# NVIDIA/tacotron2

Hardware: AMD Instinct MI355X
Metric: mel-frames/sec (train fwd+bwd) LJSpeech hparams (higher is better)
Workload: dtype bf16; 1 GPU; BASELINE configs[1]: LJSpeech default hparams, batch_size=64/GPU, synthetic LJSpeech-shaped batches, full train step (fwd+loss+bwd+clip+Adam); global_batch=64, parallelism=dp1, optimizer=FusedAdam, compute=bf16 MFMA operands, f32 accumulate/state/master weights

## Files before the change

### include/tacotron2_amd.h

```cpp
#ifndef TACOTRON2_AMD_H
#define TACOTRON2_AMD_H

#include <stdint.h>

#ifdef __cplusplus
extern "C" {
#endif

#define T2AMD_ABI_VERSION 1
#define T2AMD_OK 0
#define T2AMD_ERR_ARG 1
#define T2AMD_ERR_LAUNCH 2

#define T2AMD_ATT_DIM 128
#define T2AMD_LOC_FILTERS 32
#define T2AMD_LOC_KERNEL 31
#define T2AMD_LOC_TAPS (2 * T2AMD_LOC_KERNEL)
#define T2AMD_ATT_SLICES 4

int t2amd_abi_version(void);
const char* t2amd_source_sha1(void);
const char* t2amd_last_error(void);
int t2amd_struct_sizes(int* out, int max_n);
int t2amd_set_validate_only(int on);
int t2amd_profile_enable(int tag, int max_launches);
int t2amd_profile_read(float* total_ms, int* count);
int t2amd_profile_event_overhead(float* ms);

typedef struct t2amd_gemm_desc {
    const float* A;
    const float* B;
    float* C;
    int M, N, K;
    long long lda, ldb, ldc;
    int a_kcontig;
    int b_kcontig;
    int batch;
    long long strideA, strideB, strideC;
    int splitk;
    long long strideSplitC;
    int accumulate;
    const float* bias;
    int act;
    const uint8_t* keep;
    long long ldkeep;
    float keep_scale;
    int convA_T, convA_C, convA_pad, convA_sign;
    int convB_T, convB_C, convB_pad;
    int precision;
} t2amd_gemm_desc;

int t2amd_gemm_tile_size(int M, int N, int precision, int nz, int a_kcontig, int b_kcontig);
int t2amd_gemm_f32(const t2amd_gemm_desc* d, void* stream);

int t2amd_splitk_reduce_f32(const float* partials, int nsplit, long long stride, float* out,
                            long long n, int accumulate, int perm_taps, int perm_ci, void* stream);
int t2amd_splitk_reduce2d_f32(const float* partials, int nsplit, long long stride, float* out, int rows, int cols,
                              long long ldo, int accumulate, void* stream);

typedef struct t2amd_gemm16_desc {
    const void* A;
    const void* B;
    float* C;
    int M, N, K;
    long long lda, ldb, ldc;
    int splitk;
    long long strideSplitC;
    int accumulate;
    const float* bias;
    int win_T, win_Tp;
} t2amd_gemm16_desc;
int t2amd_gemm16_tn(const t2amd_gemm16_desc* d, void* stream);
int t2amd_gemm16_kk(const t2amd_gemm16_desc* d, void* stream);
int t2amd_gemm16_kk_group(const t2amd_gemm16_desc* d, int count, void* stream);

int t2amd_cast_halo_bf16(const float* src, long long lds, void* dst, long long rows, int C, int T, int pad, void* stream);

int t2amd_pack_conv_bf16(const float* W, void* out, int Co, int Ci, int k, int Kp, int reversed, void* stream);

int t2amd_transpose_cast_bf16(const void* src, int src_is_bf16, long long lds, void* dst, long long ldd, int rows, int cols,
                              int rows_padded, void* stream);

int t2amd_bn_stats_f32(const float* x, long long ldx, int M, int N, double* ws, float* mean,
                       float* invstd, float* running_mean, float* running_var, float momentum,
                       float eps, void* stream);
int t2amd_bn_eval_invstd_f32(const float* running_var, float* invstd, int N, float eps, void* stream);
int t2amd_bn_act_fwd_f32(const float* x, long long ldx, float* y, long long ldy, int M, int N,
                         const float* mean, const float* invstd, const float* gamma,
                         const float* beta, int act, const uint8_t* keep, long long ldkeep,
                         float keep_scale, const int* lens, int row_valid_T, void* stream);
int t2amd_bn_act_fwd_img_f32(const float* x, long long ldx, float* y, long long ldy, int M, int N, const float* mean,
                             const float* invstd, const float* gamma, const float* beta, int act, const uint8_t* keep,
                             long long ldkeep, float keep_scale, void* y_img16, int T, int pad, void* stream);
int t2amd_bn_act_bwd_f32(float* dy, long long lddy, const float* y, long long ldy, const float* x,
                         long long ldx, int M, int N, const float* mean, const float* invstd,
                         const float* gamma, int act, const uint8_t* keep, long long ldkeep,
                         float keep_scale, double* ws, float* dgamma, float* dbeta, void* stream);
int t2amd_bn_act_bwd_img_f32(float* dy, long long lddy, const float* y, long long ldy, const float* x, long long ldx, int M, int N,
                             const float* mean, const float* invstd, const float* gamma, int act, const uint8_t* keep,
                             long long ldkeep, float keep_scale, double* ws, float* dgamma, float* dbeta, void* dx_img16, int T,
                             int pad, float* dbias, int keep_f32, void* stream);
int t2amd_colsum_f32(const float* x, long long ldx, int M, int N, double* ws, float* out,
                     int accumulate, void* stream);
int t2amd_colsum_bf16(const void* x16, long long ldx, int M, int N, double* ws, float* out, int accumulate, void* stream);

int t2amd_embedding_fwd_f32(const long long* ids, const float* table, float* out, long long rows,
                            int dim, int n_symbols, void* stream);
int t2amd_embedding_bwd_f32(const long long* ids, const float* dout, float* dtable, float* ws, long long rows,
                            int dim, int n_symbols, void* stream);
int t2amd_philox_keep_mask(uint8_t* out, long long n, float p, unsigned long long seed,
                           unsigned long long offset, void* stream);
int t2amd_fill_f32(float* p, long long n, float v, void* stream);
int t2amd_cast_bf16_f32(const float* src, void* dst, long long n, void* stream);
int t2amd_split_bf16x3_f32(const float* src, long long lds, void* dst, long long ldd, long long rows, int K, void* stream);
int t2amd_copy2d_f32(const float* src, long long lds, const float* src2, long long lds2, float* dst,
                     long long ldd, int rows, int cols, void* stream);
int t2amd_transpose_f32(const float* src, long long lds, float* dst, long long ldd, int rows,
                        int cols, int batch, long long sstride, long long dstride, void* stream);
int t2amd_frames_to_time_major_f32(const float* mels, float* x0, int B, int C, int To, void* stream);
int t2amd_split_projection_f32(const float* pg, float* mel_cl, float* gate, const int* out_lens,
                               int B, int C, int To, void* stream);
int t2amd_finalize_outputs_f32(float* mel_cl, const float* post_cl, float* mel, float* mel_post,
                               const int* out_lens, int B, int C, int To, void* stream);
int t2amd_grads_to_channel_last_f32(const float* dmel, const float* dmel_post, float* dmel_cl,
                                    float* dpost_cl, int B, int C, int To, void* stream);
int t2amd_gather_dout_f32(const float* dmel_cl, const float* dgate, float* dout, int B, int C,
                          int To, void* stream);
int t2amd_relu_dropout_bwd_f32(float* dy, const float* y, float scale, long long n, void* stream);

typedef struct t2amd_seg {
    const float* p;
    long long ld;
    int width;
} t2amd_seg;

typedef struct t2amd_lstm_step {
    t2amd_seg x[3];
    int nseg;
    const float* W;
    int Ktot, H, B;
    const float* gin;
    long long ld_gin;
    const float* bias;
    const float* c_prev;
    long long ld_cprev;
    float* gates_out;
    long long ld_gates;
    float* c_out;
    long long ld_c;
    float* h_out;
    long long ld_h;
    const uint8_t* keep;
    long long ld_keep;
    float keep_scale;
    const int* lens;
    int t;
    int tag;
    int bf16;
    void* h16_out;
    long long ld_h16;
} t2amd_lstm_step;

int t2amd_lstm_step_fwd_f32(const t2amd_lstm_step* a, void* stream);
int t2amd_lstm_step_fwd2_f32(const t2amd_lstm_step* a, const t2amd_lstm_step* b, void* stream);

int t2amd_lstm_step_small_f32(const t2amd_lstm_step* a, void* stream);
typedef struct t2amd_small_linear {
    const float* X;
    long long ldx;
    const float* W;
    long long ldw;
    const float* bias;
    float* Y;
    long long ldy;
    int B, N, K;
    int act;
    const uint8_t* keep;
    long long ldkeep;
    float keep_scale;
} t2amd_small_linear;
int t2amd_linear_small_f32(const t2amd_small_linear* a, void* stream);

typedef struct t2amd_skinny_gemm {
    t2amd_seg x[3];
    int nseg;
    const float* W;
    int Ktot, N, B;
    float* Y;
    long long ldy;
    int nsplit;
    long long split_stride;
    int tag;
    int bf16;
    const float* bias;
    int act;
    const uint8_t* keep;
    long long ld_keep;
    float keep_scale;
    void* Y16;
    long long ldy16;
    uint8_t* stop_active;
    int* stop_lengths;
    int* stop_done;
    int stop_col, stop_t, stop_max_steps;
    float stop_threshold;
} t2amd_skinny_gemm;

int t2amd_skinny_gemm_f32(const t2amd_skinny_gemm* a, void* stream);
int t2amd_skinny_gemm2_f32(const t2amd_skinny_gemm* a, const t2amd_skinny_gemm* b, void* stream);

typedef struct t2amd_addend {
    const float* p;
    long long ld;
    int nsplit;
    long long split_stride;
} t2amd_addend;

typedef struct t2amd_lstm_bwd {
    int B, H;
    t2amd_addend dh[3];
    const float* gates;
    long long ld_gates;
    const float* c_prev;
    long long ld_cprev;
    const float* c;
    long long ld_c;
    const uint8_t* keep;
    long long ld_keep;
    float keep_scale;
    float* dc;
    long long ld_dc;
    float* dgates;
    long long ld_dgates;
    const int* lens;
    int t;
    void* dgates16;
    long long ld_dgates16;
    int dgates16_x3;
} t2amd_lstm_bwd;

int t2amd_lstm_pointwise_bwd_f32(const t2amd_lstm_bwd* a, void* stream);
int t2amd_lstm_pointwise_bwd2_f32(const t2amd_lstm_bwd* a, const t2amd_lstm_bwd* b, void* stream);

int t2amd_fold_location_f32(const float* wdense, const float* wconv, float* U, void* stream);
int t2amd_unfold_location_grads_f32(const float* dU_acc, const float* dv_acc, int nb,
                                    const float* wdense, const float* wconv, float* dwdense,
                                    float* dwconv, float* dv, void* stream);

typedef struct t2amd_attn_fwd {
    int B, Ti, E, Hq;
    const float* h;
    long long ld_h;
    const float* Wq;
    const float* U;
    const float* v;
    const float* pm;
    const float* memory;
    const int* lens;
    const float* w_prev;
    long long ld_wprev;
    float* cum;
    float* cum_save;
    float* w_out;
    long long ld_wout;
    float* ctx_out;
    long long ld_ctx;
    float* q_out;
    long long ld_q;
    const uint8_t* active;
    float* ws;
    void* ctx16_out;
    long long ld_ctx16;
    int loc_split_bf16;
    const void* memory16;
    const void* Wq16;
    long long ws_floats;
    int ctx16_x3;
} t2amd_attn_fwd;

int t2amd_attention_step_fwd_f32(const t2amd_attn_fwd* a, void* stream);
// ... 370 lines not shown
```

### tacotron2_amd/csrc/elementwise.hip

```cpp
#include "common.h"

#define RB 64

template <int MODE>
__global__ void colreduce_partial_kernel(const float* __restrict__ x, long long ldx, int M, int N,
                                         double* __restrict__ ws) {
    const int col = blockIdx.x * 64 + (threadIdx.x & 63);
    const int rsub = threadIdx.x >> 6;
    const int rb = blockIdx.y;
    __shared__ double s1[4][64], s2[4][64];
    double a = 0.0, q = 0.0;
    if (col < N) {
        const long long step = (long long)RB * 4;
        long long r = (long long)rb * 4 + rsub;
        for (; r + 3 * step < M; r += 4 * step) {
            const float v0 = x[r * ldx + col], v1 = x[(r + step) * ldx + col];
            const float v2 = x[(r + 2 * step) * ldx + col], v3 = x[(r + 3 * step) * ldx + col];
            a += (double)v0; a += (double)v1; a += (double)v2; a += (double)v3;
            if (MODE == 0) {
                q += (double)v0 * (double)v0; q += (double)v1 * (double)v1;
                q += (double)v2 * (double)v2; q += (double)v3 * (double)v3;
            }
        }
        for (; r < M; r += step) {
// ... 769 lines not shown
            }
        }
    }
}

extern "C" int t2amd_philox_keep_mask(uint8_t* out, long long n, float p, unsigned long long seed,
                                      unsigned long long offset, void* stream) {
    T2_REQUIRE(out && n > 0 && p >= 0.f && p < 1.f, "philox: bad args");
    T2_REQUIRE(offset % 4 == 0, "philox: offset must be a multiple of 4");
    int blocks = t2_cdiv((n + 3) / 4, 256);
    if (blocks > 8192) blocks = 8192;
    T2_LAUNCH(philox_keep_kernel, dim3(blocks), dim3(256), 0, (hipStream_t)stream, out, n, p, seed, offset);
    T2_LAUNCH_CHECK();
    return T2AMD_OK;
}

__global__ void fill_kernel(float* p, long long n, float v) {
    for (long long i = blockIdx.x * (long long)blockDim.x + threadIdx.x; i < n; i += (long long)gridDim.x * blockDim.x)
        p[i] = v;
}
__global__ void cast_bf16_kernel(const float4* __restrict__ src, uint2* __restrict__ dst, long long n4) {
    for (long long i = blockIdx.x * (long long)blockDim.x + threadIdx.x; i < n4; i += (long long)gridDim.x * blockDim.x) {
        const float4 v = src[i];
        uint2 o;
        o.x = (unsigned)t2_f32_to_bf16(v.x) | ((unsigned)t2_f32_to_bf16(v.y) << 16);
        o.y = (unsigned)t2_f32_to_bf16(v.z) | ((unsigned)t2_f32_to_bf16(v.w) << 16);
        dst[i] = o;
    }
}

extern "C" int t2amd_cast_bf16_f32(const float* src, void* dst, long long n, void* stream) {
    T2_REQUIRE(src && dst && n > 0 && n % 4 == 0, "cast_bf16: n must be a positive multiple of 4");
    T2_REQUIRE(t2_aligned16(src) && (reinterpret_cast<uintptr_t>(dst) & 7u) == 0, "cast_bf16: alignment");
    int blocks = t2_cdiv(n / 4, 256);
    if (blocks > 4096) blocks = 4096;
    T2_LAUNCH(cast_bf16_kernel, dim3(blocks), dim3(256), 0, (hipStream_t)stream, reinterpret_cast<const float4*>(src),
              reinterpret_cast<uint2*>(dst), n / 4);
    T2_LAUNCH_CHECK();
    return T2AMD_OK;
}

__global__ void split_bf16x3_kernel(const float* __restrict__ src, long long lds_, unsigned short* __restrict__ dst, long long ldd,
                                    long long rows, int K4) {
    const long long total = rows * K4;
    for (long long i = blockIdx.x * (long long)blockDim.x + threadIdx.x; i < total; i += (long long)gridDim.x * blockDim.x) {
        const long long r = i / K4;
        const int k = (int)(i - r * K4) * 4;
        const float4 v = *reinterpret_cast<const float4*>(src + r * lds_ + k);
        unsigned short h[4], l[4];
        t2_split_bf16(v.x, h[0], l[0]); t2_split_bf16(v.y, h[1], l[1]);
        t2_split_bf16(v.z, h[2], l[2]); t2_split_bf16(v.w, h[3], l[3]);
        unsigned short* const d = dst + r * ldd * 2 + t2_x3_pos(k);
        *reinterpret_cast<uint2*>(d) = make_uint2((unsigned)h[0] | ((unsigned)h[1] << 16), (unsigned)h[2] | ((unsigned)h[3] << 16));
        *reinterpret_cast<uint2*>(d + 16) = make_uint2((unsigned)l[0] | ((unsigned)l[1] << 16), (unsigned)l[2] | ((unsigned)l[3] << 16));
    }
}
extern "C" int t2amd_split_bf16x3_f32(const float* src, long long lds, void* dst, long long ldd, long long rows, int K, void* stream) {
    T2_REQUIRE(src && dst && rows > 0 && K > 0 && K % 16 == 0, "split_bf16x3: K must be a positive multiple of 16");
    T2_REQUIRE(lds >= K && lds % 4 == 0 && ldd >= K && ldd % 16 == 0, "split_bf16x3: row strides (lds % 4 == 0, ldd % 16 == 0, both >= K)");
    T2_REQUIRE(t2_aligned16(src) && t2_aligned16(dst), "split_bf16x3: alignment");
    int blocks = t2_cdiv(rows * (K / 4), 256);
    if (blocks > 8192) blocks = 8192;
    T2_LAUNCH(split_bf16x3_kernel, dim3(blocks), dim3(256), 0, (hipStream_t)stream, src, lds, reinterpret_cast<unsigned short*>(dst), ldd,
              rows, K / 4);
    T2_LAUNCH_CHECK();
    return T2AMD_OK;
}

extern "C" int t2amd_fill_f32(float* p, long long n, float v, void* stream) {
    T2_REQUIRE(p && n > 0, "fill: bad args");
    int blocks = t2_cdiv(n, 256);
    if (blocks > 4096) blocks = 4096;
    T2_LAUNCH(fill_kernel, dim3(blocks), dim3(256), 0, (hipStream_t)stream, p, n, v);
    T2_LAUNCH_CHECK();
    return T2AMD_OK;
}

__global__ void copy2d_kernel(const float* __restrict__ src, long long lds_, const float* __restrict__ src2,
                              long long lds2, float* __restrict__ dst, long long ldd, int rows, int cols) {
    const long long total = (long long)rows * cols;
    for (long long i = blockIdx.x * (long long)blockDim.x + threadIdx.x; i < total;
         i += (long long)gridDim.x * blockDim.x) {
        const long long r = i / cols;
        const int c = (int)(i - r * cols);
        float v = src[r * lds_ + c];
        if (src2) v += src2[r * lds2 + c];
        dst[r * ldd + c] = v;
    }
}
extern "C" int t2amd_copy2d_f32(const float* src, long long lds_, const float* src2, long long lds2, float* dst,
                                long long ldd, int rows, int cols, void* stream) {
    T2_REQUIRE(src && dst && rows > 0 && cols > 0, "copy2d: bad args");
    int blocks = t2_cdiv((long long)rows * cols, 256);
    if (blocks > 4096) blocks = 4096;
    T2_LAUNCH(copy2d_kernel, dim3(blocks), dim3(256), 0, (hipStream_t)stream, src, lds_, src2, lds2, dst, ldd,
                       rows, cols);
    T2_LAUNCH_CHECK();
    return T2AMD_OK;
}

__global__ void transpose_kernel(const float* __restrict__ src, long long lds_, float* __restrict__ dst, long long ldd,
                                 int rows, int cols, long long sstride, long long dstride) {
    __shared__ float tile[32][33];
    const float* s = src + (long long)blockIdx.z * sstride;
    float* d = dst + (long long)blockIdx.z * dstride;
    const int c0 = blockIdx.x * 32, r0 = blockIdx.y * 32;
    const int tx = threadIdx.x & 31, ty = threadIdx.x >> 5;
    for (int j = ty; j < 32; j += 8) {
        const int r = r0 + j, c = c0 + tx;
        tile[j][tx] = (r < rows && c < cols) ? s[(long long)r * lds_ + c] : 0.f;
    }
    __syncthreads();
    for (int j = ty; j < 32; j += 8) {
        const int c = c0 + j, r = r0 + tx;
        if (c < cols && r < rows) d[(long long)c * ldd + r] = tile[tx][j];
    }
}
extern "C" int t2amd_transpose_f32(const float* src, long long lds_, float* dst, long long ldd, int rows, int cols,
                                   int batch, long long sstride, long long dstride, void* stream) {
    T2_REQUIRE(src && dst && rows > 0 && cols > 0 && batch > 0, "transpose: bad args");
    dim3 grid(t2_cdiv(cols, 32), t2_cdiv(rows, 32), batch);
    T2_REQUIRE(grid.y <= 65535 && grid.z <= 65535, "transpose: grid too large");
    T2_LAUNCH(transpose_kernel, grid, dim3(256), 0, (hipStream_t)stream, src, lds_, dst, ldd, rows, cols, sstride,
                       dstride);
    T2_LAUNCH_CHECK();
    return T2AMD_OK;
}

__global__ void frames_to_tm_kernel(const float* __restrict__ mels, float* __restrict__ x0, int B, int C, int To) {
    __shared__ float tile[32][33];
    const int b = blockIdx.z;
    const int t0 = blockIdx.x * 32, c0 = blockIdx.y * 32;
    const int tx = threadIdx.x & 31, ty = threadIdx.x >> 5;
    for (int j = ty; j < 32; j += 8) {
        const int c = c0 + j, t = t0 + tx;
        float v = 0.f;
        if (c < C && t < To && t >= 1) v = mels[((long long)b * C + c) * To + (t - 1)];
        tile[j][tx] = v;
    }
    __syncthreads();
    for (int j = ty; j < 32; j += 8) {
        const int t = t0 + j, c = c0 + tx;
        if (t < To && c < C) x0[((long long)t * B + b) * C + c] = tile[tx][j];
    }
}
extern "C" int t2amd_frames_to_time_major_f32(const float* mels, float* x0, int B, int C, int To, void* stream) {
    T2_REQUIRE(mels && x0 && B > 0 && C > 0 && To > 0, "frames_to_tm: bad args");
    dim3 grid(t2_cdiv(To, 32), t2_cdiv(C, 32), B);
    T2_LAUNCH(frames_to_tm_kernel, grid, dim3(256), 0, (hipStream_t)stream, mels, x0, B, C, To);
    T2_LAUNCH_CHECK();
    return T2AMD_OK;
}

__global__ void split_projection_kernel(const float* __restrict__ pg, float* __restrict__ mel_cl,
                                        float* __restrict__ gate, const int* __restrict__ out_lens, int B, int C,
                                        int To) {
    const long long total = (long long)To * B * (C + 1);
    for (long long i = blockIdx.x * (long long)blockDim.x + threadIdx.x; i < total;
         i += (long long)gridDim.x * blockDim.x) {
        const long long row = i / (C + 1);
        const int c = (int)(i - row * (C + 1));
        const int t = (int)(row / B), b = (int)(row - (long long)t * B);
        const float v = pg[i];
        if (c < C) {
            mel_cl[((long long)b * To + t) * C + c] = v;
        } else {
            const bool pad = out_lens && t >= out_lens[b];
            gate[(long long)b * To + t] = pad ? 1e3f : v;
        }
    }
}
extern "C" int t2amd_split_projection_f32(const float* pg, float* mel_cl, float* gate, const int* out_lens, int B,
                                          int C, int To, void* stream) {
    T2_REQUIRE(pg && mel_cl && gate && B > 0 && C > 0 && To > 0, "split_projection: bad args");
    int blocks = t2_cdiv((long long)To * B * (C + 1), 256);
    if (blocks > 8192) blocks = 8192;
    T2_LAUNCH(split_projection_kernel, dim3(blocks), dim3(256), 0, (hipStream_t)stream, pg, mel_cl, gate,
                       out_lens, B, C, To);
    T2_LAUNCH_CHECK();
    return T2AMD_OK;
}

__global__ void finalize_outputs_kernel(float* __restrict__ mel_cl, const float* __restrict__ post_cl,
                                        float* __restrict__ mel, float* __restrict__ mel_post,
                                        const int* __restrict__ out_lens, int B, int C, int To) {
    __shared__ float t1[32][33], t2[32][33];
    const int b = blockIdx.z;
    const int c0 = blockIdx.x * 32, t0 = blockIdx.y * 32;
    const int tx = threadIdx.x & 31, ty = threadIdx.x >> 5;
    const int len = out_lens ? out_lens[b] : To;
    for (int j = ty; j < 32; j += 8) {
        const int t = t0 + j, c = c0 + tx;
        float m = 0.f, q = 0.f;
        if (t < To && c < C) {
            const long long idx = ((long long)b * To + t) * C + c;
            if (t < len) {
                m = mel_cl[idx];
                q = post_cl ? m + post_cl[idx] : 0.f;
            } else {
                mel_cl[idx] = 0.f;
            }
        }
        t1[j][tx] = m;
        t2[j][tx] = q;
    }
    __syncthreads();
    for (int j = ty; j < 32; j += 8) {
        const int c = c0 + j, t = t0 + tx;
        if (c < C && t < To) {
            const long long o = ((long long)b * C + c) * To + t;
            mel[o] = t1[tx][j];
            if (mel_post) mel_post[o] = t2[tx][j];
        }
    }
}
extern "C" int t2amd_finalize_outputs_f32(float* mel_cl, const float* post_cl, float* mel, float* mel_post,
                                          const int* out_lens, int B, int C, int To, void* stream) {
    T2_REQUIRE(mel_cl && mel && B > 0 && C > 0 && To > 0, "finalize_outputs: bad args");
    T2_REQUIRE((post_cl != nullptr) == (mel_post != nullptr), "finalize_outputs: post_cl and mel_post go together");
    dim3 grid(t2_cdiv(C, 32), t2_cdiv(To, 32), B);
    T2_REQUIRE(grid.y <= 65535, "finalize_outputs: To too large");
    T2_LAUNCH(finalize_outputs_kernel, grid, dim3(256), 0, (hipStream_t)stream, mel_cl, post_cl, mel, mel_post,
                       out_lens, B, C, To);
    T2_LAUNCH_CHECK();
    return T2AMD_OK;
}

__global__ void grads_to_cl_kernel(const float* __restrict__ dmel, const float* __restrict__ dmel_post,
                                   float* __restrict__ dmel_cl, float* __restrict__ dpost_cl, int B, int C, int To) {
    __shared__ float t1[32][33], t2[32][33];
    const int b = blockIdx.z;
    const int t0 = blockIdx.x * 32, c0 = blockIdx.y * 32;
    const int tx = threadIdx.x & 31, ty = threadIdx.x >> 5;
    for (int j = ty; j < 32; j += 8) {
        const int c = c0 + j, t = t0 + tx;
        float a = 0.f, q = 0.f;
        if (c < C && t < To) {
            const long long idx = ((long long)b * C + c) * To + t;
            if (dmel) a = dmel[idx];
            if (dmel_post) q = dmel_post[idx];
        }
        t1[j][tx] = a;
        t2[j][tx] = q;
    }
    __syncthreads();
    for (int j = ty; j < 32; j += 8) {
        const int t = t0 + j, c = c0 + tx;
        if (t < To && c < C) {
            const long long o = ((long long)b * To + t) * C + c;
            dmel_cl[o] = t1[tx][j] + t2[tx][j];
            dpost_cl[o] = t2[tx][j];
        }
    }
}
extern "C" int t2amd_grads_to_channel_last_f32(const float* dmel, const float* dmel_post, float* dmel_cl,
                                               float* dpost_cl, int B, int C, int To, void* stream) {
    T2_REQUIRE(dmel_cl && dpost_cl && B > 0 && C > 0 && To > 0, "grads_to_cl: bad args");
    dim3 grid(t2_cdiv(To, 32), t2_cdiv(C, 32), B);
    T2_LAUNCH(grads_to_cl_kernel, grid, dim3(256), 0, (hipStream_t)stream, dmel, dmel_post, dmel_cl, dpost_cl, B,
                       C, To);
    T2_LAUNCH_CHECK();
    return T2AMD_OK;
}

__global__ void gather_dout_kernel(const float* __restrict__ dmel_cl, const float* __restrict__ dgate,
                                   float* __restrict__ dout, int B, int C, int To) {
    const long long total = (long long)To * B * (C + 1);
    for (long long i = blockIdx.x * (long long)blockDim.x + threadIdx.x; i < total;
         i += (long long)gridDim.x * blockDim.x) {
        const long long row = i / (C + 1);
        const int c = (int)(i - row * (C + 1));
        const int t = (int)(row / B), b = (int)(row - (long long)t * B);
        float v;
        if (c < C) v = dmel_cl[((long long)b * To + t) * C + c];
        else v = dgate ? dgate[(long long)b * To + t] : 0.f;
        dout[i] = v;
    }
}
extern "C" int t2amd_gather_dout_f32(const float* dmel_cl, const float* dgate, float* dout, int B, int C, int To,
                                     void* stream) {
    T2_REQUIRE(dmel_cl && dout && B > 0 && C > 0 && To > 0, "gather_dout: bad args");
    int blocks = t2_cdiv((long long)To * B * (C + 1), 256);
    if (blocks > 8192) blocks = 8192;
    T2_LAUNCH(gather_dout_kernel, dim3(blocks), dim3(256), 0, (hipStream_t)stream, dmel_cl, dgate, dout, B, C,
                       To);
    T2_LAUNCH_CHECK();
    return T2AMD_OK;
}

__global__ void relu_dropout_bwd_kernel(float* __restrict__ dy, const float* __restrict__ y, float scale, long long n) {
    for (long long i = blockIdx.x * (long long)blockDim.x + threadIdx.x; i < n; i += (long long)gridDim.x * blockDim.x)
        dy[i] = (y[i] > 0.f) ? dy[i] * scale : 0.f;
}
__global__ void relu_dropout_bwd_vec_kernel(float4* __restrict__ dy, const float4* __restrict__ y, float scale, long long n4) {
    for (long long i = blockIdx.x * (long long)blockDim.x + threadIdx.x; i < n4; i += (long long)gridDim.x * blockDim.x) {
        const float4 g = dy[i], v = y[i];
        dy[i] = make_float4((v.x > 0.f) ? g.x * scale : 0.f, (v.y > 0.f) ? g.y * scale : 0.f, (v.z > 0.f) ? g.z * scale : 0.f,
                            (v.w > 0.f) ? g.w * scale : 0.f);
    }
}
extern "C" int t2amd_relu_dropout_bwd_f32(float* dy, const float* y, float scale, long long n, void* stream) {
    T2_REQUIRE(dy && y && n > 0, "relu_dropout_bwd: bad args");
    if (!g_ew_scalar && n % 4 == 0 && t2_aligned16(dy) && t2_aligned16(y)) {
        int b4 = t2_cdiv(n / 4, 256);
        if (b4 > 8192) b4 = 8192;
        T2_LAUNCH(relu_dropout_bwd_vec_kernel, dim3(b4), dim3(256), 0, (hipStream_t)stream, reinterpret_cast<float4*>(dy),
                  reinterpret_cast<const float4*>(y), scale, n / 4);
        T2_LAUNCH_CHECK();
        return T2AMD_OK;
    }
    int blocks = t2_cdiv(n, 256);
    if (blocks > 8192) blocks = 8192;
    T2_LAUNCH(relu_dropout_bwd_kernel, dim3(blocks), dim3(256), 0, (hipStream_t)stream, dy, y, scale, n);
    T2_LAUNCH_CHECK();
    return T2AMD_OK;
}
```

### tacotron2_amd/csrc/gemm16.hip

```cpp
#include "common.h"
#include <stdlib.h>

typedef __bf16 g16_bf16x8 __attribute__((ext_vector_type(8)));
typedef __attribute__((address_space(3))) void* g16_lptr;
typedef __attribute__((address_space(1))) const void* g16_gptr;

#define G16_T 256
#define G16_BK 64
#define G16_IMG (G16_T * 128)
#define G16_NT 512

struct Gemm16Params {
    t2amd_gemm16_desc d;
    int ktiles_per_split;
};

struct G16Tile { int bx, by, bz; };
__device__ __forceinline__ G16Tile g16_tile_id() {
    const int nbx = gridDim.x, nby = gridDim.y;
    const int total = nbx * nby * (int)gridDim.z;
    const int L = blockIdx.x + nbx * (blockIdx.y + nby * blockIdx.z);
    const int xcd = L & 7, q = L >> 3;
    const int base = total >> 3, rem = total & 7;
    const int id = xcd * base + (xcd < rem ? xcd : rem) + q;
    const int per_z = nbx * nby;
    G16Tile t;
    t.bz = id / per_z;
    const int r = id - t.bz * per_z;
    const int G = 8;
    const int group = r / (G * nbx);
    const int first = group * G;
    const int gsz = (nby - first) < G ? (nby - first) : G;
    const int w = r - group * (G * nbx);
    t.by = first + w % gsz;
    t.bx = w / gsz;
    return t;
}

__global__ __launch_bounds__(G16_NT) void gemm16_tn_kernel(Gemm16Params p) {
    __shared__ __attribute__((aligned(16))) char smem[4 * G16_IMG];
    const t2amd_gemm16_desc& d = p.d;
    const int tid = threadIdx.x, lane = tid & 63;
    const int wave = __builtin_amdgcn_readfirstlane(tid >> 6);
    const int wm = wave >> 2, wn = wave & 3;
    const int l31 = lane & 31, lhi = lane >> 5;

    const G16Tile tile = g16_tile_id();
    const int split = tile.bz;
    const int row0 = tile.by * G16_T, col0 = tile.bx * G16_T;
    const int M = d.M, N = d.N;
    const int nkt_all = d.K / G16_BK;
    const int kt_beg = split * p.ktiles_per_split;
    int kt_end = kt_beg + p.ktiles_per_split;
    if (kt_end > nkt_all) kt_end = nkt_all;
    const int nk = kt_end > kt_beg ? kt_end - kt_beg : 0;

    const char* asrc[4];
    const char* bsrc[4];
    {
        const int rin = 8 * wave + (lane >> 3);
        const int chunk = (lane & 7) ^ ((rin >> 1) & 7);
#pragma unroll
        for (int i = 0; i < 4; ++i) {
            int ga = row0 + 64 * i + rin, gb = col0 + 64 * i + rin;
            ga = ga < M ? ga : M - 1;
            gb = gb < N ? gb : N - 1;
            asrc[i] = reinterpret_cast<const char*>(d.A) + ((long long)ga * d.lda + (long long)kt_beg * G16_BK) * 2 + chunk * 16;
            bsrc[i] = reinterpret_cast<const char*>(d.B) + ((long long)gb * d.ldb + (long long)kt_beg * G16_BK) * 2 + chunk * 16;
        }
    }
#define G16_ISSUE(STAGE)                                                                                         \
    {                                                                                                            \
        char* ad_ = smem + (STAGE) * G16_IMG + wave * 1024;                                                      \
        char* bd_ = smem + (2 + (STAGE)) * G16_IMG + wave * 1024;                                                \
        _Pragma("unroll") for (int i = 0; i < 4; ++i) {                                                          \
            __builtin_amdgcn_global_load_lds((g16_gptr)(asrc[i]), (g16_lptr)(ad_ + i * 8192), 16, 0, 0);         \
            __builtin_amdgcn_global_load_lds((g16_gptr)(bsrc[i]), (g16_lptr)(bd_ + i * 8192), 16, 0, 0);         \
            asrc[i] += 128; bsrc[i] += 128;                                                                      \
        }                                                                                                        \
    }

    unsigned aaddr[4][4], baddr[2][4];
    {
        const unsigned base = (unsigned)reinterpret_cast<size_t>((g16_lptr)(smem));
#pragma unroll
        for (int t = 0; t < 4; ++t) {
            const int r = wm * 128 + t * 32 + l31;
#pragma unroll
            for (int ks = 0; ks < 4; ++ks) aaddr[t][ks] = base + (unsigned)(r * 128 + (((2 * ks + lhi) ^ ((r >> 1) & 7)) << 4));
        }
#pragma unroll
        for (int t = 0; t < 2; ++t) {
            const int r = wn * 64 + t * 32 + l31;
#pragma unroll
            for (int ks = 0; ks < 4; ++ks)
                baddr[t][ks] = base + 2 * G16_IMG + (unsigned)(r * 128 + (((2 * ks + lhi) ^ ((r >> 1) & 7)) << 4));
        }
    }

    f32x16 acc[4][2];
#pragma unroll
    for (int i = 0; i < 4; ++i)
#pragma unroll
        for (int j = 0; j < 2; ++j)
#pragma unroll
            for (int r = 0; r < 16; ++r) acc[i][j][r] = 0.f;

    f32x4 fa[4], fb[2], ga[4], gb[2];
#define G16_READ(STAGE, KS, A_, B_)                                                                              \
    asm volatile(                                                                                                \
        "ds_read_b128 %0, %6 offset:%12\n\t"                                                                     \
        "ds_read_b128 %4, %10 offset:%12\n\t"                                                                    \
        "ds_read_b128 %1, %7 offset:%12\n\t"                                                                     \
        "ds_read_b128 %5, %11 offset:%12\n\t"                                                                    \
        "ds_read_b128 %2, %8 offset:%12\n\t"                                                                     \
        "ds_read_b128 %3, %9 offset:%12"                                                                         \
        : "=&v"(A_[0]), "=&v"(A_[1]), "=&v"(A_[2]), "=&v"(A_[3]), "=&v"(B_[0]), "=&v"(B_[1])                     \
        : "v"(aaddr[0][KS]), "v"(aaddr[1][KS]), "v"(aaddr[2][KS]), "v"(aaddr[3][KS]), "v"(baddr[0][KS]),          \
          "v"(baddr[1][KS]), "i"((STAGE) * G16_IMG)                                                              \
        : "memory");
#define G16_WAIT(A_, B_)                                                                                         \
    asm volatile("s_waitcnt lgkmcnt(0)"                                                                          \
                 : "+v"(A_[0]), "+v"(A_[1]), "+v"(A_[2]), "+v"(A_[3]), "+v"(B_[0]), "+v"(B_[1]) : : "memory");
#define G16_MFMA(A_, B_)                                                                                         \
    _Pragma("unroll") for (int i = 0; i < 4; ++i)                                                                \
        _Pragma("unroll") for (int j = 0; j < 2; ++j)                                                            \
            acc[i][j] = __builtin_amdgcn_mfma_f32_32x32x16_bf16(__builtin_bit_cast(g16_bf16x8, A_[i]),           \
                                                                __builtin_bit_cast(g16_bf16x8, B_[j]), acc[i][j], 0, 0, 0);
#define G16_TILE(STAGE)                                                                                          \
    {                                                                                                            \
        G16_READ(STAGE, 0, fa, fb) G16_WAIT(fa, fb)                                                              \
        G16_READ(STAGE, 1, ga, gb) __builtin_amdgcn_sched_barrier(0); G16_MFMA(fa, fb) __builtin_amdgcn_sched_barrier(0); G16_WAIT(ga, gb) \
        G16_READ(STAGE, 2, fa, fb) __builtin_amdgcn_sched_barrier(0); G16_MFMA(ga, gb) __builtin_amdgcn_sched_barrier(0); G16_WAIT(fa, fb) \
        G16_READ(STAGE, 3, ga, gb) __builtin_amdgcn_sched_barrier(0); G16_MFMA(fa, fb) __builtin_amdgcn_sched_barrier(0); G16_WAIT(ga, gb) \
        G16_MFMA(ga, gb)                                                                                         \
    }

    if (nk > 0) {
        G16_ISSUE(0)
        asm volatile("s_waitcnt vmcnt(0)" ::: "memory");
        __builtin_amdgcn_s_barrier();
        for (int kt = 0; kt + 1 < nk; kt += 2) {
            G16_ISSUE(1)
            G16_TILE(0)
            asm volatile("s_waitcnt vmcnt(0)" ::: "memory");
            __builtin_amdgcn_s_barrier();
            if (kt + 2 < nk) G16_ISSUE(0)
            G16_TILE(1)
            asm volatile("s_waitcnt vmcnt(0)" ::: "memory");
            __builtin_amdgcn_s_barrier();
        }
        if (nk & 1) G16_TILE(0)
    }
#undef G16_ISSUE
#undef G16_READ
#undef G16_WAIT
#undef G16_MFMA
#undef G16_TILE

    float* __restrict__ C = d.C + (long long)split * d.strideSplitC;
#pragma unroll
    for (int tm = 0; tm < 4; ++tm) {
#pragma unroll
        for (int tn = 0; tn < 2; ++tn) {
            const int gn = col0 + wn * 64 + tn * 32 + l31;
#pragma unroll
            for (int r = 0; r < 16; ++r) {
                const int gm = row0 + wm * 128 + tm * 32 + (r & 3) + 8 * (r >> 2) + 4 * lhi;
                long long crow = gm;
                bool live = gm < M;
                if (d.win_Tp > 0) {
                    const int b_ = gm / d.win_Tp, t_ = gm - b_ * d.win_Tp;
                    live = live && t_ < d.win_T;
                    crow = (long long)b_ * d.win_T + t_;
                }
                if (live && gn < N) {
                    float* cp = C + crow * d.ldc + gn;
                    float val = acc[tm][tn][r];
                    if (d.bias) val += d.bias[gn];
                    if (d.accumulate) val += *cp;
                    *cp = val;
                }
            }
        }
    }
}

extern "C" int t2amd_gemm16_tn(const t2amd_gemm16_desc* dp, void* stream) {
    T2_REQUIRE(dp != nullptr, "gemm16: null descriptor");
    Gemm16Params p;
    p.d = *dp;
    t2amd_gemm16_desc& d = p.d;
    T2_REQUIRE(d.A && d.B && d.C, "gemm16: null operand");
    T2_REQUIRE(d.M > 0 && d.N > 0 && d.K > 0 && d.K % G16_BK == 0, "gemm16: K must be a positive multiple of 64");
    T2_REQUIRE(t2_aligned16(d.A) && t2_aligned16(d.B) && d.lda % 8 == 0 && d.ldb % 8 == 0 && d.ldb >= d.K,
               "gemm16: operands must be 16-byte aligned with row strides that are multiples of 8 elements (B's >= K)");
    T2_REQUIRE(d.win_Tp == 0 || (d.win_T > 0 && d.win_T <= d.win_Tp && d.splitk == 1), "gemm16: bad window geometry");
    T2_REQUIRE(d.win_Tp > 0 || d.lda >= d.K, "gemm16: lda must be >= K unless the rows are windows");
    if (d.splitk < 1) d.splitk = 1;
    T2_REQUIRE(d.splitk == 1 || (!d.bias && !d.accumulate), "gemm16: split-K needs a plain epilogue");
    const int nkt = d.K / G16_BK;
    p.ktiles_per_split = t2_cdiv(nkt, d.splitk);
    dim3 grid(t2_cdiv(d.N, G16_T), t2_cdiv(d.M, G16_T), d.splitk);
    T2_REQUIRE(grid.y <= 65535 && grid.z <= 65535, "gemm16: grid too large");
    T2_LAUNCH(gemm16_tn_kernel, grid, dim3(G16_NT), 0, (hipStream_t)stream, p);
    T2_LAUNCH_CHECK();
    return T2AMD_OK;
}

typedef float g16_f32x2 __attribute__((ext_vector_type(2)));

#define G16_GROUP 4
struct Gemm16GroupParams {
    t2amd_gemm16_desc d[G16_GROUP];
    int coltile_end[G16_GROUP];
    int count;
};

__global__ __launch_bounds__(G16_NT) void gemm16_kk_kernel(Gemm16GroupParams p) {
    __shared__ __attribute__((aligned(16))) char smem[4 * G16_IMG];
    const int tid = threadIdx.x, lane = tid & 63;
    const int wave = __builtin_amdgcn_readfirstlane(tid >> 6);
    const int wm = wave >> 2, wn = wave & 3;
    const int l31 = lane & 31, lhi = lane >> 5;

    const G16Tile tile = g16_tile_id();
    const int split = tile.bz;
    int prob = 0;
#pragma unroll
    for (int j = 0; j + 1 < G16_GROUP; ++j)
        if (j + 1 < p.count && tile.bx >= p.coltile_end[j]) prob = j + 1;
    const int bx = tile.bx - (prob > 0 ? p.coltile_end[prob - 1] : 0);
    struct { const void* A; const void* B; float* C; int M, N, K; long long lda, ldb, ldc; long long strideSplitC; int accumulate;
             const float* bias; int splitk; } d;
    d.A = p.d[prob].A; d.B = p.d[prob].B; d.C = p.d[prob].C; d.M = p.d[prob].M; d.N = p.d[prob].N; d.K = p.d[prob].K;
    d.lda = p.d[prob].lda; d.ldb = p.d[prob].ldb; d.ldc = p.d[prob].ldc; d.strideSplitC = p.d[prob].strideSplitC;
    d.accumulate = p.d[prob].accumulate; d.bias = p.d[prob].bias; d.splitk = p.d[prob].splitk;
    const int row0 = tile.by * G16_T, col0 = bx * G16_T;
    const int M = d.M, N = d.N;
    const int nkt_all = (d.K + G16_BK - 1) / G16_BK;
    const int per_split = (nkt_all + d.splitk - 1) / d.splitk;
    const int kt_beg = split * per_split;
    int kt_end = kt_beg + per_split;
    if (kt_end > nkt_all) kt_end = nkt_all;
    const int nk = kt_end > kt_beg ? kt_end - kt_beg : 0;
    const int rem = d.K - (nkt_all - 1) * G16_BK;
    const int ztile = (kt_end == nkt_all && rem < G16_BK) ? nk - 1 : -1;

    const int rsub = 2 * wave + lhi;
    const long long arow = d.lda * 2, brow = d.ldb * 2;
    const char* asrc[4];
    const char* bsrc[4];
    {
        const int cl = l31 ^ ((rsub & 3) << 2);
        int ma = row0 + 8 * cl, nb = col0 + 8 * cl;
        ma = ma + 8 <= M ? ma : M - 8;
        nb = nb + 8 <= N ? nb : N - 8;
#pragma unroll
        for (int i = 0; i < 4; ++i) {
            const long long k = (long long)kt_beg * G16_BK + 16 * i + rsub;
            asrc[i] = reinterpret_cast<const char*>(d.A) + k * arow + (long long)ma * 2;
            bsrc[i] = reinterpret_cast<const char*>(d.B) + k * brow + (long long)nb * 2;
        }
    }
#define KK_ISSUE(STAGE, KT)                                                                                      \
    {                                                                                                            \
        char* ad_ = smem + (STAGE) * G16_IMG + wave * 1024;                                                      \
        char* bd_ = smem + (2 + (STAGE)) * G16_IMG + wave * 1024;                                                \
        if ((KT) != ztile) {                                                                                     \
            _Pragma("unroll") for (int i = 0; i < 4; ++i) {                                                      \
                __builtin_amdgcn_global_load_lds((g16_gptr)(asrc[i]), (g16_lptr)(ad_ + i * 8192), 16, 0, 0);     \
                __builtin_amdgcn_global_load_lds((g16_gptr)(bsrc[i]), (g16_lptr)(bd_ + i * 8192), 16, 0, 0);     \
                asrc[i] += 64 * arow; bsrc[i] += 64 * brow;                                                      \
            }                                                                                                    \
        } else {                                                                                                 \
            _Pragma("unroll") for (int i = 0; i < 4; ++i) {                                                      \
                const int over = 16 * i + rsub - (rem - 1);           \
                const char* a_ = over > 0 ? asrc[i] - over * arow : asrc[i];                                     \
                const char* b_ = over > 0 ? bsrc[i] - over * brow : bsrc[i];                                     \
                __builtin_amdgcn_global_load_lds((g16_gptr)(a_), (g16_lptr)(ad_ + i * 8192), 16, 0, 0);          \
                __builtin_amdgcn_global_load_lds((g16_gptr)(b_), (g16_lptr)(bd_ + i * 8192), 16, 0, 0);          \
            }                                                                                                    \
        }                                                                                                        \
    }
#define KK_LANDED(STAGE, KT)                                                                                     \
    asm volatile("s_waitcnt vmcnt(0)" ::: "memory");                                                             \
    if ((KT) == ztile) {                                                                                         \
        _Pragma("unroll") for (int i = 0; i < 4; ++i)                                                            \
            if (16 * i + rsub >= rem)                                                                            \
                *reinterpret_cast<f32x4*>(smem + (STAGE) * G16_IMG + i * 8192 + wave * 1024 + lane * 16) = f32x4{0.f, 0.f, 0.f, 0.f}; \
        asm volatile("s_waitcnt lgkmcnt(0)" ::: "memory");                                                       \
    }                                                                                                            \
    __builtin_amdgcn_s_barrier();

    unsigned aaddr[4], baddr[2];
    {
        const unsigned base = (unsigned)reinterpret_cast<size_t>((g16_lptr)(smem));
        const int g = lane >> 4, i = lane & 15;
        const int r = 8 * (g >> 1) + (i >> 2);
        const int sw = (i >> 2) << 2;
        const int sub = 2 * (g & 1) + ((i & 3) >> 1);
        const unsigned in = (unsigned)(r * 512 + (i & 1) * 8);
#pragma unroll
        for (int t = 0; t < 4; ++t) aaddr[t] = base + in + (unsigned)((((wm * 16 + 4 * t + sub) ^ sw)) << 4);
#pragma unroll
        for (int t = 0; t < 2; ++t) baddr[t] = base + 2 * G16_IMG + in + (unsigned)((((wn * 8 + 4 * t + sub) ^ sw)) << 4);
    }

    f32x16 acc[4][2];
#pragma unroll
    for (int i = 0; i < 4; ++i)
#pragma unroll
        for (int j = 0; j < 2; ++j)
#pragma unroll
            for (int r = 0; r < 16; ++r) acc[i][j][r] = 0.f;

    g16_f32x2 fa[4][2], fb[2][2], ga[4][2], gb[2][2];
#define KK_READ(STAGE, KS, A_, B_)                                                                               \
    asm volatile(                                                                                                \
        "ds_read_b64_tr_b16 %0, %12 offset:%18\n\t"                                                              \
        "ds_read_b64_tr_b16 %1, %12 offset:%19\n\t"                                                              \
        "ds_read_b64_tr_b16 %8, %16 offset:%18\n\t"                                                              \
        "ds_read_b64_tr_b16 %9, %16 offset:%19\n\t"                                                              \
        "ds_read_b64_tr_b16 %2, %13 offset:%18\n\t"                                                              \
        "ds_read_b64_tr_b16 %3, %13 offset:%19\n\t"                                                              \
        "ds_read_b64_tr_b16 %10, %17 offset:%18\n\t"                                                             \
        "ds_read_b64_tr_b16 %11, %17 offset:%19\n\t"                                                             \
        "ds_read_b64_tr_b16 %4, %14 offset:%18\n\t"                                                              \
        "ds_read_b64_tr_b16 %5, %14 offset:%19\n\t"                                                              \
        "ds_read_b64_tr_b16 %6, %15 offset:%18\n\t"                                                              \
        "ds_read_b64_tr_b16 %7, %15 offset:%19"                                                                  \
        : "=&v"(A_[0][0]), "=&v"(A_[0][1]), "=&v"(A_[1][0]), "=&v"(A_[1][1]), "=&v"(A_[2][0]), "=&v"(A_[2][1]),  \
          "=&v"(A_[3][0]), "=&v"(A_[3][1]), "=&v"(B_[0][0]), "=&v"(B_[0][1]), "=&v"(B_[1][0]), "=&v"(B_[1][1])   \
        : "v"(aaddr[0]), "v"(aaddr[1]), "v"(aaddr[2]), "v"(aaddr[3]), "v"(baddr[0]), "v"(baddr[1]),              \
          "i"((STAGE) * G16_IMG + (KS) * 8192), "i"((STAGE) * G16_IMG + (KS) * 8192 + 2048)                      \
        : "memory");
#define KK_WAIT(A_, B_)                                                                                          \
    asm volatile("s_waitcnt lgkmcnt(0)"                                                                          \
                 : "+v"(A_[0][0]), "+v"(A_[0][1]), "+v"(A_[1][0]), "+v"(A_[1][1]), "+v"(A_[2][0]), "+v"(A_[2][1]), \
                   "+v"(A_[3][0]), "+v"(A_[3][1]), "+v"(B_[0][0]), "+v"(B_[0][1]), "+v"(B_[1][0]), "+v"(B_[1][1]) : : "memory");
#define KK_OP(X_) __builtin_bit_cast(g16_bf16x8, __builtin_shufflevector(X_[0], X_[1], 0, 1, 2, 3))
#define KK_MFMA(A_, B_)                                                                                          \
    _Pragma("unroll") for (int i = 0; i < 4; ++i)                                                                \
        _Pragma("unroll") for (int j = 0; j < 2; ++j)                                                            \
            acc[i][j] = __builtin_amdgcn_mfma_f32_32x32x16_bf16(KK_OP(A_[i]), KK_OP(B_[j]), acc[i][j], 0, 0, 0);
#define KK_TILE(STAGE)                                                                                           \
    {                                                                                                            \
        KK_READ(STAGE, 0, fa, fb) KK_WAIT(fa, fb)                                                                \
        KK_READ(STAGE, 1, ga, gb) __builtin_amdgcn_sched_barrier(0); KK_MFMA(fa, fb) __builtin_amdgcn_sched_barrier(0); KK_WAIT(ga, gb) \
        KK_READ(STAGE, 2, fa, fb) __builtin_amdgcn_sched_barrier(0); KK_MFMA(ga, gb) __builtin_amdgcn_sched_barrier(0); KK_WAIT(fa, fb) \
        KK_READ(STAGE, 3, ga, gb) __builtin_amdgcn_sched_barrier(0); KK_MFMA(fa, fb) __builtin_amdgcn_sched_barrier(0); KK_WAIT(ga, gb) \
        KK_MFMA(ga, gb)                                                                                          \
    }

    if (nk > 0) {
        KK_ISSUE(0, 0)
        KK_LANDED(0, 0)
        for (int kt = 0; kt + 1 < nk; kt += 2) {
            KK_ISSUE(1, kt + 1)
            KK_TILE(0)
            KK_LANDED(1, kt + 1)
            if (kt + 2 < nk) KK_ISSUE(0, kt + 2)
            KK_TILE(1)
            KK_LANDED(0, kt + 2)
        }
        if (nk & 1) KK_TILE(0)
    }
#undef KK_ISSUE
#undef KK_LANDED
#undef KK_READ
#undef KK_WAIT
#undef KK_OP
#undef KK_MFMA
#undef KK_TILE

    float* __restrict__ C = d.C + (long long)split * d.strideSplitC;
#pragma unroll
    for (int tm = 0; tm < 4; ++tm) {
#pragma unroll
        for (int tn = 0; tn < 2; ++tn) {
            const int gn = col0 + wn * 64 + tn * 32 + l31;
#pragma unroll
            for (int r = 0; r < 16; ++r) {
                const int gm = row0 + wm * 128 + tm * 32 + (r & 3) + 8 * (r >> 2) + 4 * lhi;
                if (gm < M && gn < N) {
                    float* cp = C + (long long)gm * d.ldc + gn;
                    float val = acc[tm][tn][r];
                    if (d.bias) val += d.bias[gn];
                    if (d.accumulate) val += *cp;
                    *cp = val;
                }
            }
        }
    }
}

extern "C" int t2amd_gemm16_kk_group(const t2amd_gemm16_desc* dp, int count, void* stream) {
    T2_REQUIRE(dp != nullptr && count >= 1 && count <= G16_GROUP, "gemm16_kk: 1..4 descriptors");
    Gemm16GroupParams p;
    p.count = count;
    int coltiles = 0;
    for (int j = 0; j < G16_GROUP; ++j) {
        p.d[j] = dp[j < count ? j : count - 1];
        if (j >= count) { p.coltile_end[j] = coltiles; continue; }
        t2amd_gemm16_desc& d = p.d[j];
        T2_REQUIRE(d.A && d.B && d.C, "gemm16_kk: null operand");
        T2_REQUIRE(d.M >= 8 && d.N >= 8 && d.K > 0 && d.M % 8 == 0 && d.N % 8 == 0, "gemm16_kk: M and N must be positive multiples of 8, K positive");
        T2_REQUIRE(t2_aligned16(d.A) && t2_aligned16(d.B) && d.lda > 0 && d.ldb > 0 && d.lda % 8 == 0 && d.ldb % 8 == 0,
                   "gemm16_kk: operands must be 16-byte aligned with row strides that are multiples of 8 elements");
        T2_REQUIRE(d.win_Tp == 0 && d.win_T == 0, "gemm16_kk: no window epilogue (overlapping rows are expressed by lda / ldb < M / N)");
        if (d.splitk < 1) d.splitk = 1;
        T2_REQUIRE(d.splitk == 1 || (!d.bias && !d.accumulate), "gemm16_kk: split-K needs a plain epilogue");
        T2_REQUIRE(d.M == p.d[0].M && d.splitk == p.d[0].splitk, "gemm16_kk: the products of one launch share M and the split count");
        coltiles += t2_cdiv(d.N, G16_T);
        p.coltile_end[j] = coltiles;
    }
    dim3 grid(coltiles, t2_cdiv(p.d[0].M, G16_T), p.d[0].splitk);
    T2_REQUIRE(grid.y <= 65535 && grid.z <= 65535, "gemm16_kk: grid too large");
    T2_LAUNCH(gemm16_kk_kernel, grid, dim3(G16_NT), 0, (hipStream_t)stream, p);
    T2_LAUNCH_CHECK();
    return T2AMD_OK;
}

extern "C" int t2amd_gemm16_kk(const t2amd_gemm16_desc* dp, void* stream) { return t2amd_gemm16_kk_group(dp, 1, stream); }

template <bool SRC16>
__global__ __launch_bounds__(256) void transpose_cast16_kernel(const void* __restrict__ src, long long lds_, unsigned short* __restrict__ dst,
                                                               long long ldd, int rows, int cols, int rpad) {
    __shared__ unsigned short tile[64][66];
    const int r0 = blockIdx.x * 64, c0 = blockIdx.y * 64;
    const int tid = threadIdx.x;
    const bool vec_in = SRC16 ? (lds_ % 4 == 0 && (reinterpret_cast<size_t>(src) & 7) == 0) : (lds_ % 4 == 0 && (reinterpret_cast<size_t>(src) & 15) == 0);
#pragma unroll
    for (int pass = 0; pass < 4; ++pass) {
        const int i = pass * 16 + (tid >> 4), j = 4 * (tid & 15);
        const int r = r0 + i, c = c0 + j;
        unsigned short v[4] = {0, 0, 0, 0};
        if (r < rows) {
            if (vec_in && c + 3 < cols) {
                if (SRC16) {
                    const uint2 u = *reinterpret_cast<const uint2*>(reinterpret_cast<const unsigned short*>(src) + (long long)r * lds_ + c);
                    v[0] = (unsigned short)(u.x & 0xffffu); v[1] = (unsigned short)(u.x >> 16);
                    v[2] = (unsigned short)(u.y & 0xffffu); v[3] = (unsigned short)(u.y >> 16);
                } else {
                    const float4 f = *reinterpret_cast<const float4*>(reinterpret_cast<const float*>(src) + (long long)r * lds_ + c);
                    v[0] = t2_f32_to_bf16(f.x); v[1] = t2_f32_to_bf16(f.y); v[2] = t2_f32_to_bf16(f.z); v[3] = t2_f32_to_bf16(f.w);
                }
            } else {
#pragma unroll
                for (int e = 0; e < 4; ++e)
                    if (c + e < cols)
                        v[e] = SRC16 ? reinterpret_cast<const unsigned short*>(src)[(long long)r * lds_ + c + e]
                                     : t2_f32_to_bf16(reinterpret_cast<const float*>(src)[(long long)r * lds_ + c + e]);
            }
        }
#pragma unroll
        for (int e = 0; e < 4; ++e) tile[i][j + e] = v[e];
    }
    __syncthreads();
    const bool vec_out = ldd % 4 == 0 && (reinterpret_cast<size_t>(dst) & 7) == 0;
#pragma unroll
    for (int pass = 0; pass < 4; ++pass) {
        const int i = pass * 16 + (tid >> 4), j = 4 * (tid & 15);
        const int c = c0 + i, r = r0 + j;
        if (c >= cols || r >= rpad) continue;
        unsigned short* o = dst + (long long)c * ldd + r;
        if (vec_out && r + 3 < rpad) {
            uint2 u;
            u.x = (unsigned)tile[j][i] | ((unsigned)tile[j + 1][i] << 16);
            u.y = (unsigned)tile[j + 2][i] | ((unsigned)tile[j + 3][i] << 16);
            *reinterpret_cast<uint2*>(o) = u;
        } else {
#pragma unroll
            for (int e = 0; e < 4; ++e)
                if (r + e < rpad) o[e] = tile[j + e][i];
        }
    }
}

__global__ __launch_bounds__(256) void cast_halo16_kernel(const float* __restrict__ src, long long lds_, unsigned short* __restrict__ dst,
                                                          long long img_rows, long long nb, int C4, int T, int Tp, int pad) {
    const long long i = (long long)blockIdx.x * 256 + threadIdx.x;
    if (i >= img_rows * C4) return;
    const long long R = i / C4;
    const int c4 = (int)(i - R * C4);
    const long long b = R / Tp;
    const int t = (int)(R - b * Tp) - pad;
    uint2 o = make_uint2(0u, 0u);
    if (b < nb && t >= 0 && t < T) {
        const float4 v = *reinterpret_cast<const float4*>(src + (b * T + t) * lds_ + c4 * 4);
        o.x = (unsigned)t2_f32_to_bf16(v.x) | ((unsigned)t2_f32_to_bf16(v.y) << 16);
        o.y = (unsigned)t2_f32_to_bf16(v.z) | ((unsigned)t2_f32_to_bf16(v.w) << 16);
    }
    *reinterpret_cast<uint2*>(dst + (R * (long long)(C4 * 4)) + c4 * 4) = o;
}

__global__ __launch_bounds__(256) void pack_conv16_kernel(const float* __restrict__ W, unsigned short* __restrict__ out, int Co, int Ci,
                                                          int k, int Kp, int reversed) {
    const int rows = reversed ? Ci : Co, inner = reversed ? Co : Ci;
    const long long n = (long long)rows * Kp;
    for (long long i = (long long)blockIdx.x * 256 + threadIdx.x; i < n; i += (long long)gridDim.x * 256) {
        const int r = (int)(i / Kp), c = (int)(i - (long long)r * Kp);
        unsigned short v = 0;
        if (c < k * inner) {
            const int tap = c / inner, j = c - tap * inner;
            const int co = reversed ? j : r, ci = reversed ? r : j, t = reversed ? k - 1 - tap : tap;
            v = t2_f32_to_bf16(W[((long long)co * Ci + ci) * k + t]);
        }
        out[i] = v;
    }
}

extern "C" int t2amd_pack_conv_bf16(const float* W, void* out, int Co, int Ci, int k, int Kp, int reversed, void* stream) {
    T2_REQUIRE(W && out && Co > 0 && Ci > 0 && k > 0 && Kp >= k * (reversed ? Co : Ci), "pack_conv: bad arguments");
    const long long n = (long long)(reversed ? Ci : Co) * Kp;
    int blocks = t2_cdiv(n, 256);
    if (blocks > 8192) blocks = 8192;
    T2_LAUNCH(pack_conv16_kernel, dim3(blocks), dim3(256), 0, (hipStream_t)stream, W, (unsigned short*)out, Co, Ci, k, Kp, reversed);
    T2_LAUNCH_CHECK();
    return T2AMD_OK;
}

extern "C" int t2amd_cast_halo_bf16(const float* src, long long lds_, void* dst, long long rows, int C, int T, int pad, void* stream) {
    T2_REQUIRE(src && dst && rows > 0 && C > 0 && C % 4 == 0 && T > 0 && rows % T == 0 && pad >= 0 && lds_ % 4 == 0 &&
                   t2_aligned16(src) && t2_aligned16(dst),
               "cast_halo: rows must be whole utterances of T, C a multiple of 4, 16-byte aligned operands");
    const long long nb = rows / T, img_rows = nb * (T + 2 * pad) + 2 * pad;
    const long long n = img_rows * (C / 4);
    T2_REQUIRE((n + 255) / 256 < (1ll << 31), "cast_halo: too large");
    T2_LAUNCH(cast_halo16_kernel, dim3((unsigned)((n + 255) / 256)), dim3(256), 0, (hipStream_t)stream, src, lds_, (unsigned short*)dst,
              img_rows, nb, C / 4, T, T + 2 * pad, pad);
    T2_LAUNCH_CHECK();
    return T2AMD_OK;
}

extern "C" int t2amd_transpose_cast_bf16(const void* src, int src_is_bf16, long long lds_, void* dst, long long ldd, int rows, int cols,
                                         int rows_padded, void* stream) {
    T2_REQUIRE(src && dst && rows > 0 && cols > 0 && rows_padded >= rows && ldd >= rows_padded, "transpose_cast: bad arguments");
    dim3 grid(t2_cdiv(rows_padded, 64), t2_cdiv(cols, 64));
    T2_REQUIRE(grid.y <= 65535, "transpose_cast: too many columns");
    if (src_is_bf16)
        T2_LAUNCH((transpose_cast16_kernel<true>), grid, dim3(256), 0, (hipStream_t)stream, src, lds_, (unsigned short*)dst, ldd, rows, cols, rows_padded);
    else
        T2_LAUNCH((transpose_cast16_kernel<false>), grid, dim3(256), 0, (hipStream_t)stream, src, lds_, (unsigned short*)dst, ldd, rows, cols, rows_padded);
    T2_LAUNCH_CHECK();
    return T2AMD_OK;
}
```

### tacotron2_amd/engine.py

```python
import os

import math
import torch

from . import native as nv
from .native import NativeError

BN_EPS = 1e-5
BN_MOMENTUM = 0.1


def check_hparams(hp):
    if hp.n_frames_per_step != 1:
        raise ValueError("n_frames_per_step != 1 is not supported (nor by the reference, hparams.py:56)")
    K = hp.attention_location_kernel_size
    if not (1 <= hp.attention_dim <= nv.ATT_DIM and 1 <= hp.attention_location_n_filters <= nv.LOC_FILTERS
            and 1 <= K <= nv.LOC_KERNEL and K % 2 == 1):
        raise ValueError("the attention kernels hold attention_dim <= %d, <= %d location filters and an odd location "
                         "kernel <= %d (smaller geometries run zero-embedded in the compiled one; an even kernel size "
                         "does not run in the reference either: ConvNorm pads (k-1)//2, model.py:18-20)"
                         % (nv.ATT_DIM, nv.LOC_FILTERS, nv.LOC_KERNEL))
    for name in ('encoder_embedding_dim', 'attention_rnn_dim', 'decoder_rnn_dim', 'prenet_dim'):
        if getattr(hp, name) % 64 != 0:
            raise ValueError("%s must be a multiple of 64 for the MFMA recurrent kernels" % name)
    if (hp.encoder_embedding_dim // 2) % 64 != 0:
        raise ValueError("encoder_embedding_dim/2 must be a multiple of 64")
    if hp.symbols_embedding_dim != hp.encoder_embedding_dim:
        raise ValueError("symbols_embedding_dim must equal encoder_embedding_dim")
    for name in ('encoder_embedding_dim', 'postnet_embedding_dim', 'n_mel_channels'):
        if getattr(hp, name) % 16 != 0:
            raise ValueError("%s must be a multiple of 16 (implicit-GEMM convolution tiles)" % name)
    if hp.encoder_kernel_size % 2 != 1 or hp.postnet_kernel_size % 2 != 1:
        raise ValueError("convolution kernel sizes must be odd")


class MaskSource(object):

    def __init__(self, injected, device, run=None):
        self.injected = injected or {}
        self.device = device
        self.run = run
        self.seed = None
        self.offset = 0

    def get(self, name, index, shape, p):
        src = self.injected.get(name)
        if src is not None:
            m = src[index] if index is not None else src
            if tuple(m.shape) != tuple(shape) or m.dtype != torch.uint8 or not m.is_contiguous():
                raise NativeError("injected mask %s[%s] must be contiguous uint8 of shape %s, got %s %s"
                                  % (name, index, tuple(shape), tuple(m.shape), m.dtype))
            return m
        if self.seed is None:
            self.seed = int(torch.randint(0, 2 ** 62, (1,)).item())
        out = self.run.empty8(*shape) if self.run is not None else torch.empty(shape, dtype=torch.uint8, device=self.device)
        nv.philox_keep_mask(out, p, self.seed, self.offset)
        self.offset += (out.numel() + 3) // 4 * 4
        return out


def _choose_splitk(M, N, K, batch=1, precision=0, a_km=False, b_kn=False):
    t256 = ((M + 255) // 256) * ((N + 255) // 256) * batch
    if precision >= 1 and M >= 512 and N >= 512 and nv.gemm_tile_size(M, N, precision, 1 << 20, a_km, b_kn) == 256:
        if t256 >= 192:
            return 1
        best, best_score = 0, -1.0
        for s in range(1, 33):
            if s > 1 and K // s < 512:
                break
            if t256 * s < 192:
                continue
            w = t256 * s / 256.0
            score = w / math.ceil(w) * min(1.0, w / 0.85) - 0.02 * (s - 1)
            if score > best_score:
                best, best_score = s, score
        if best:
            return best
    tiles = ((M + 127) // 128) * ((N + 127) // 128) * batch
    if tiles >= 512:
        return 1
    s = (768 + tiles - 1) // tiles
    s = min(s, 64, max(1, K // 256))
    return max(1, s)


def _choose_splitk16(M, N, K):
    t256 = ((M + 255) // 256) * ((N + 255) // 256)
    nkt = (K + 63) // 64
    best, best_t = 1, None
    for s in range(1, 65):
        if s > 1 and nkt // s < 8:
            break
        rounds = math.ceil(t256 * s / 256.0)
        t = rounds * (math.ceil(nkt / s) * 1.9 + 4.0)
        if s > 1:
            t += (s + 1) * M * N * 4 / 5.0e6 + 3.0
        if best_t is None or t < best_t - 1e-9:
            best, best_t = s, t
    return best


WGRAD16 = os.environ.get('T2AMD_WGRAD16', '1') != '0'


WGRAD_KK = os.environ.get('T2AMD_WGRAD_KK', '1') != '0'


def _kk_to(run, out, A16, B16, K, M, N, lda=None, ldb=None, perm=None):
    sk = _choose_splitk16(M, N, K)
    if sk == 1 and perm is None:
        nv.gemm16_kk(out, A16, B16, K, M=M, N=N, lda=lda, ldb=ldb)
        return
    part = run.empty(sk, M * N)
    nv.gemm16_kk(part[0].view(M, N), A16, B16, K, M=M, N=N, lda=lda, ldb=ldb, splitk=sk, partials=part)
    if perm is not None:
        nv.splitk_reduce(part, sk, out, perm_taps=perm[0], perm_ci=perm[1])
    else:
        nv.splitk_reduce2d(part, sk, out)


def _lstm_wgrad_kk(run, dG2, B, parts, outs):
    rowsD, G4 = dG2.shape
    widths = [src.shape[1] for src, _ in parts]
    offs = [0]
    for w in widths:
        offs.append(offs[-1] + w)
    jobs = []
    for dW, i0, i1 in outs:
        base = offs[i0]
        for i in range(i0, i1):
            src, shifted = parts[i]
            if src.dtype != torch.bfloat16:
                src = run.cast16(src)
            blk = dW[:, offs[i] - base:offs[i + 1] - base]
            if shifted and rowsD <= B:
                blk.zero_()
            elif shifted:
                jobs.append((blk, dG2[B:], src, rowsD - B, widths[i]))
            else:
                jobs.append((blk, dG2, src, rowsD, widths[i]))
    if not jobs:
        return
    sk = _choose_splitk16(G4, sum((j[4] + 255) // 256 * 256 for j in jobs), rowsD)
    if sk == 1:
        nv.gemm16_kk_group([dict(Cm=blk, A16=A, B16=Bm, K=K, M=G4, N=w) for blk, A, Bm, K, w in jobs])
        return
    parts_ = [run.empty(sk, G4 * w) for _, _, _, _, w in jobs]
    nv.gemm16_kk_group([dict(Cm=pt[0].view(G4, w), A16=A, B16=Bm, K=K, M=G4, N=w, splitk=sk, partials=pt)
                        for (blk, A, Bm, K, w), pt in zip(jobs, parts_)])
    for (blk, _, _, _, _), pt in zip(jobs, parts_):
        nv.splitk_reduce2d(pt, sk, blk)


def _lstm_wgrad16(run, dG2, B, parts, outs):
    rowsD, G4 = dG2.shape
    if WGRAD_KK and G4 % 8 == 0 and all(src.shape[1] % 8 == 0 for src, _ in parts):
        return _lstm_wgrad_kk(run, dG2, B, parts, outs)
    Kp = ((rowsD + B + 63) // 64) * 64
    GT = run.empty16(G4, Kp)
    nv.transpose_cast_bf16(dG2, GT)
    widths = [src.shape[1] for src, _ in parts]
    XT = run.empty16(sum(widths), Kp)
    n0, offs = 0, []
    for (src, shifted), w in zip(parts, widths):
        blk = XT[n0:n0 + w]
        if shifted:
            blk[:, :B].zero_()
            if rowsD > B:
                nv.transpose_cast_bf16(src[:rowsD - B], blk[:, B:])
            else:
                blk[:, B:].zero_()
        else:
            nv.transpose_cast_bf16(src, blk)
        offs.append(n0)
        n0 += w
    offs.append(n0)
    for dW, i0, i1 in outs:
        Bop = XT[offs[i0]:offs[i1]]
        M, N = dW.shape
        sk = _choose_splitk16(M, N, Kp)
        if sk == 1:
            nv.gemm16_tn(dW, GT, Bop)
        else:
            part = run.empty(sk, M * N)
            nv.gemm16_tn(dW, GT, Bop, splitk=sk, partials=part)
            nv.splitk_reduce(part, sk, dW)


class _Ctx(object):
    arena = None

    def release(self):
        a, self.arena = self.arena, None
        _arena_release(a)

    def __del__(self):
        try:
            self.release()
        except Exception:
            pass


class _EvalCtx(object):
    training = False


FAST_GRAD_GEMM = True


def _dgrad_split():
    raw = os.environ.get('T2AMD_DGRAD_SPLIT', '2')
    try:
        ns = int(raw)
    except ValueError:
        ns = -1
    if not 1 <= ns <= 8:
        raise NativeError("T2AMD_DGRAD_SPLIT must be an integer in 1..8, got %r" % (raw,))
    return ns


DGRAD_SPLIT = _dgrad_split()


def _enc_dgrad_split():
    raw = os.environ.get('T2AMD_ENC_DGRAD_SPLIT', '4')
    if raw not in ('1', '2', '4'):
        raise NativeError("T2AMD_ENC_DGRAD_SPLIT must be 1, 2 or 4, got %r" % (raw,))
    return int(raw)


ENC_DGRAD_SPLIT = _enc_dgrad_split()

BN_BWD_IMAGE = os.environ.get('T2AMD_BN_BWD_IMAGE', '1') != '0'
BN_FWD_IMAGE = os.environ.get('T2AMD_BN_FWD_IMAGE', '1') != '0'
BIAS_GRAD16 = os.environ.get('T2AMD_BIAS_GRAD16', '1') != '0'
GATE_GRADS_BF16_ONLY = os.environ.get('T2AMD_GATE_GRADS_BF16_ONLY', '1') != '0'
DXD_RING = int(os.environ.get('T2AMD_DXD_RING', '3'))


def _rg(run, *a, **k):
    return run.gemm(*a, fast=run.gradp, **k)


def _ng(run, *a, **k):
    return nv.gemm(*a, fast=run.gradp, **k)


def _fg(run, *a, exact=False, **k):
    return nv.gemm(*a, fast=(0 if (exact and run.x3) else run.fwdp), **k)


_PACK_GEN = [0]


def bump_weight_generation():
    _PACK_GEN[0] += 1


# ... 597 lines not shown
               "runs on the launch chain from here on" % ne)
        if log is not None:
            log(msg)
        else:
            import sys
            print(msg, file=sys.stderr, flush=True)
    if n > 0:
        TRAIN_FWD_PERSISTENT = False
        nv.set_attn_fwd_fused(0)
        nv.set_attn_bwd_fused(0)
        nv.set_bptt_cell_fold(0)
        msg = ("tacotron2_amd: %d in-launch attention hand-off(s) timed out (the workgroups of an utterance were not "
               "co-resident within 50 ms -- is the GPU shared or partitioned?); that step was poisoned with NaN and is "
               "skipped; the separate-launch forms are selected from here on" % n)
        if TRAIN_FWD_REPROMOTE_AFTER > 0:
            msg += " (and re-selected after %d clean steps)" % _DEMOTION['need']
        if log is not None:
            log(msg)
        else:
            import sys
            print(msg, file=sys.stderr, flush=True)
    return n + ne


def _cached_bias_sum(run, tag, b1, b2):
    return run.cached(tag, [b1, b2], lambda: _bias_sum(run, b1, b2))


_ATT_Q = 'decoder.attention_layer.query_layer.linear_layer.weight'
_ATT_M = 'decoder.attention_layer.memory_layer.linear_layer.weight'
_ATT_V = 'decoder.attention_layer.v.linear_layer.weight'
_ATT_D = 'decoder.attention_layer.location_layer.location_dense.linear_layer.weight'
_ATT_C = 'decoder.attention_layer.location_layer.location_conv.conv.weight'


def _embed_attention(run, P):
    Wq, Wm, Wv, Wd, Wc = (P[n] for n in (_ATT_Q, _ATT_M, _ATT_V, _ATT_D, _ATT_C))
    A, F, K = Wq.shape[0], Wc.shape[0], Wc.shape[2]
    AD, FD, KD = nv.ATT_DIM, nv.LOC_FILTERS, nv.LOC_KERNEL
    if (A, F, K) == (AD, FD, KD):
        return P, ()

    def embed():
        o = (KD - K) // 2
        q = run.zeros(AD, Wq.shape[1]); q[:A] = Wq
        m = run.zeros(AD, Wm.shape[1]); m[:A] = Wm
        v = run.zeros(1, AD); v[:, :A] = Wv
        d = run.zeros(AD, FD); d[:A, :F] = Wd
        c = run.zeros(FD, 2, KD); c[:F, :, o:o + K] = Wc
        return q, m, v, d, c
    emb = run.cached('attention.embedded', [Wq, Wm, Wv, Wd, Wc], embed)
    P = dict(P)
    P.update(zip((_ATT_Q, _ATT_M, _ATT_V, _ATT_D, _ATT_C), emb))
    return P, (_ATT_Q, _ATT_M, _ATT_V, _ATT_D, _ATT_C)


def _crop_attention_grad(name, grad, shape):
    if name == _ATT_C:
        o = (nv.LOC_KERNEL - shape[2]) // 2
        return grad[:shape[0], :, o:o + shape[2]]
    return grad[:shape[0], :shape[1]]


def _fold_U(run, Wdense, Wconv):
    U = run.empty(nv.ATT_DIM * nv.LOC_TAPS)
    nv.fold_location(Wdense, Wconv, U)
    return U


def _packed_projection(run, P, Cm, Hd, E):
    Wp = P['decoder.linear_projection.linear_layer.weight']
    Wg = P['decoder.gate_layer.linear_layer.weight']
    bp = P['decoder.linear_projection.linear_layer.bias']
    bg = P['decoder.gate_layer.linear_layer.bias']

    def pack():
        Wpg = run.empty(Cm + 1, Hd + E)
        nv.copy2d(Wpg[:Cm], Wp)
        nv.copy2d(Wpg[Cm:], Wg)
        bpg = run.empty(Cm + 1)
        nv.copy2d(bpg[:Cm].view(1, Cm), bp.view(1, Cm))
        nv.copy2d(bpg[Cm:].view(1, 1), bg.view(1, 1))
        return Wpg, bpg
    return run.cached('Wpg', [Wp, Wg, bp, bg], pack)


def _forward(model, P, bufs, text, in_lens, mels, max_len, out_lens, training):
    hp = model.hparams
    dev = text.device
    if not text.is_cuda and not nv.validate_only():
        raise NativeError("tacotron2_amd: the engine runs on the MI355X only (got %s tensors). "
                          "There is no CPU path; the CPU oracle lives in oracle/ for tests." % dev)
    nv.load()
    c = _Ctx()
    c.arena = _arena_acquire(dev)
    run = _Run(dev, getattr(model, 'precision', 'fp32'), _weight_cache(model), c.arena)
    _guard_weights(model, run, P)
    P, _ = _embed_attention(run, P)
    ms = MaskSource(model.dropout_masks, dev, run)
    B = text.shape[0]
    Ti = int(max_len)
    To = mels.shape[2]
    E = hp.encoder_embedding_dim
    Ha, Hd, Pd = hp.attention_rnn_dim, hp.decoder_rnn_dim, hp.prenet_dim
    Cm = hp.n_mel_channels
    He = E // 2
    A = nv.ATT_DIM
    if text.shape[1] != Ti:
        text = text[:, :Ti]
    text = text.contiguous()
    mels = mels.contiguous().float()
    lens32 = in_lens.to(torch.int32).contiguous()
    olens32 = out_lens.to(torch.int32).contiguous() if (model.mask_padding and out_lens is not None) else None
    c.B, c.Ti, c.To, c.text, c.lens32, c.olens32 = B, Ti, To, text, lens32, olens32
    c.training = training

    rowsE = B * Ti
    emb = run.empty(rowsE, E)
    nv.embedding_fwd(text, P['embedding.weight'], emb)
    nconv = hp.encoder_n_convolutions
    enc_masks = [ms.get('enc', i, (B, Ti, E), 0.5) for i in range(nconv)] if training else None
    x3, c.enc_saved = _conv_stack_fwd(run, P, bufs, 'encoder.convolutions', nconv, emb, Ti,
                                      [1] * nconv, enc_masks, training, exact=True)
    memory = run.empty(B, Ti, E)
    c.enc_lstm = []
    for d, sfx in enumerate(('', '_reverse')):
        Wih = P['encoder.lstm.weight_ih_l0' + sfx]
        Whh = P['encoder.lstm.weight_hh_l0' + sfx]
        bsum = _cached_bias_sum(run, 'enc_bias' + sfx, P['encoder.lstm.bias_ih_l0' + sfx], P['encoder.lstm.bias_hh_l0' + sfx])
        GX = run.empty(rowsE, 4 * He)
        _fg(run, GX, x3, Wih, bias=bsum)
        Cst = run.empty(Ti, B, He)
        desc = nv.LstmSeq()
        desc.B, desc.T, desc.H, desc.reverse = B, Ti, He, d
        desc.Whh = nv.ptr(Whh)
        desc.GX = nv.ptr(GX)
        out_view = memory.view(rowsE, E)[:, d * He:(d + 1) * He]
        desc.out, desc.ld_out = nv.ptr(out_view), E
        desc.C = nv.ptr(Cst)
        desc.lens = nv.ptr(lens32, torch.int32)
        c.enc_lstm.append(dict(GX=GX, C=Cst, Whh=Whh, Wih=Wih, desc=desc, bsum=bsum))

    def regen_gx():
        for L_ in c.enc_lstm:
            _fg(run, L_['GX'], x3, L_['Wih'], bias=L_['bsum'])
    model.last_encoder_path = _encoder_lstm_fwd(
        model, text.device, c.enc_lstm[0]['desc'], c.enc_lstm[1]['desc'], regen_gx,
        reads=[L_[k_] for L_ in c.enc_lstm for k_ in ('Whh', 'GX')] + [lens32],
        writes=[memory] + [L_['C'] for L_ in c.enc_lstm], poison=memory if training else None, run=run)
    c.x3, c.memory = x3, memory

    rowsD = To * B
    x0 = run.empty(To, B, Cm)
    nv.frames_to_time_major(mels, x0)
    W1 = P['decoder.prenet.layers.0.linear_layer.weight']
    W2 = P['decoder.prenet.layers.1.linear_layer.weight']
    k0 = ms.get('prenet', 0, (To, B, Pd), 0.5)
    k1 = ms.get('prenet', 1, (To, B, Pd), 0.5)
    p1 = run.empty(rowsD, Pd)
    p2 = run.empty(rowsD, Pd)
    _fg(run, p1, x0.view(rowsD, Cm), W1, act=1, keep=k0.view(rowsD, Pd), keep_scale=2.0, exact=True)
    _fg(run, p2, p1, W2, act=1, keep=k1.view(rowsD, Pd), keep_scale=2.0, exact=True)
    Wmem = P['decoder.attention_layer.memory_layer.linear_layer.weight']
    pm = run.empty(B, Ti, A)
    _fg(run, pm.view(rowsE, A), memory.view(rowsE, E), Wmem)

    Wih_a, Whh_a = P['decoder.attention_rnn.weight_ih'], P['decoder.attention_rnn.weight_hh']
    Wih_d, Whh_d = P['decoder.decoder_rnn.weight_ih'], P['decoder.decoder_rnn.weight_hh']
    bias_a = _cached_bias_sum(run, 'bias_a', P['decoder.attention_rnn.bias_ih'], P['decoder.attention_rnn.bias_hh'])
    bias_d = _cached_bias_sum(run, 'bias_d', P['decoder.decoder_rnn.bias_ih'], P['decoder.decoder_rnn.bias_hh'])

    def pack_a_rec():
        W = run.empty(4 * Ha, E + Ha)
        nv.copy2d(W[:, :E], Wih_a[:, Pd:Pd + E])
        nv.copy2d(W[:, E:], Whh_a)
        return W

    def pack_d_cat():
        W = run.empty(4 * Hd, Ha + E + Hd)
        nv.copy2d(W[:, :Ha + E], Wih_d)
        nv.copy2d(W[:, Ha + E:], Whh_d)
        return W

    Wa_rec = run.cached('Wa_rec', [Wih_a, Whh_a], pack_a_rec)
    Wd_cat = run.cached('Wd_cat', [Wih_d, Whh_d], pack_d_cat)
    Wq = P['decoder.attention_layer.query_layer.linear_layer.weight'].contiguous()
    Wdense = P['decoder.attention_layer.location_layer.location_dense.linear_layer.weight']
    Wconv = P['decoder.attention_layer.location_layer.location_conv.conv.weight']
    U = run.cached('U', [Wdense, Wconv], lambda: _fold_U(run, Wdense, Wconv))
    vvec = P['decoder.attention_layer.v.linear_layer.weight'].view(-1)

    GA = run.empty(To, B, 4 * Ha)

    def project_ga():
        if run.bf16 and WGRAD16 and Pd % 64 == 0 and (Pd + E) % 8 == 0 and not nv.validate_only():
            Wih_a16 = run.cached('Wih_a16', [Wih_a], lambda: run.cast16(Wih_a))
            nv.gemm16_tn(GA.view(rowsD, 4 * Ha), run.cast16(p2), Wih_a16[:, :Pd], bias=bias_a)
        else:
            _fg(run, GA.view(rowsD, 4 * Ha), p2, Wih_a[:, :Pd], bias=bias_a)
    project_ga()

    att_p, dec_p = hp.p_attention_dropout, hp.p_decoder_dropout
    keep_att = ms.get('att', None, (To, B, Ha), att_p) if training else None
    keep_dec = ms.get('dec', None, (To, B, Hd), dec_p) if training else None

    d = nv.DecTrain()
    d.B, d.Ti, d.To, d.E, d.Ha, d.Hd = B, Ti, To, E, Ha, Hd
    slabs = dict(HA=run.empty(To, B, Ha), CA=run.empty(To, B, Ha), GD=run.empty(To, B, 4 * Hd),
                 HD=run.empty(To, B, Hd), CD=run.empty(To, B, Hd), CTX=run.empty(To, B, E),
                 Q=run.empty(To, B, A), ALIGN=run.out_empty(B, To, Ti), CUM=run.empty(To, B, Ti),
                 cum_work=run.empty(B, Ti),
                 attn_ws=run.empty(nv.attn_fwd_ws_floats(B, Ti) + nv.attn_bwd_ws_floats(B, Ti)))
    d.Wa_rec, d.Wd_cat, d.bias_d = nv.ptr(Wa_rec), nv.ptr(Wd_cat), nv.ptr(bias_d)
    d.Wq, d.U, d.v = nv.ptr(Wq), nv.ptr(U), nv.ptr(vvec)
    d.GA, d.memory, d.pm = nv.ptr(GA), nv.ptr(memory), nv.ptr(pm)
    d.lens = nv.ptr(lens32, torch.int32)
    d.keep_att = nv.ptr(keep_att, torch.uint8)
    d.keep_dec = nv.ptr(keep_dec, torch.uint8)
    d.scale_att, d.scale_dec = nv.scale_for(att_p), nv.scale_for(dec_p)
    for k_, v_ in slabs.items():
        setattr(d, k_, nv.ptr(v_))
    if run.bf16:
        c.bf16 = dict(Wa_rec16=run.cached('Wa_rec16', [Wih_a, Whh_a], lambda: run.cast16(Wa_rec)),
                      Wd_cat16=run.cached('Wd_cat16', [Wih_d, Whh_d], lambda: run.cast16(Wd_cat)),
                      HA16=run.empty16(To, B, Ha),
                      HD16=run.empty16(To, B, Hd), CTX16=run.empty16(To, B, E), memory16=run.cast16(memory),
                      Wq16=run.cached('Wq16', [Wq], lambda: run.cast16(Wq)))
        d.bf16 = 1
        for k_, v_ in c.bf16.items():
            setattr(d, k_, nv.ptr(v_, torch.bfloat16))
    elif run.x3:
        c.bf16 = dict(Wa_rec16=run.cached('Wa_rec16x3', [Wih_a, Whh_a], lambda: run.split16(Wa_rec)),
                      Wd_cat16=run.cached('Wd_cat16x3', [Wih_d, Whh_d], lambda: run.split16(Wd_cat)),
                      HA16=run.empty16(To, B, 2 * Ha), HD16=run.empty16(To, B, 2 * Hd), CTX16=run.empty16(To, B, 2 * E))
        d.bf16 = 3
        for k_, v_ in c.bf16.items():
            setattr(d, k_, nv.ptr(v_, torch.bfloat16))
    op16 = run.bf16 or run.x3
    model.last_train_decoder_path = _decoder_train_fwd(
        model, run, d, poison=slabs['CTX'] if training else None,
        reads=[Wa_rec, Wd_cat, bias_d, Wq, U, vvec, memory, pm, lens32, keep_att, keep_dec]
        + ([c.bf16[k_] for k_ in ('Wa_rec16', 'Wd_cat16')] if op16 else []) + ([c.bf16[k_] for k_ in ('memory16', 'Wq16')] if run.bf16 else []),
        writes=[GA] + list(slabs.values()) + ([c.bf16[k_] for k_ in ('HA16', 'HD16', 'CTX16')] if op16 else []),
        regen_ga=project_ga)

    Wpg, bpg = _packed_projection(run, P, Cm, Hd, E)
    PG = run.empty(rowsD, Cm + 1)
    _fg(run, PG, slabs['HD'].view(rowsD, Hd), Wpg[:, :Hd])
    _fg(run, PG, slabs['CTX'].view(rowsD, E), Wpg[:, Hd:], accumulate=True, bias=bpg)
    mel_cl = run.empty(B, To, Cm)
    gate = run.out_empty(B, To)
    nv.split_projection(PG, mel_cl, gate, olens32)

    npost = hp.postnet_n_convolutions
    rowsP = B * To
    post_chans = [hp.postnet_embedding_dim] * (npost - 1) + [Cm]
    post_masks = [ms.get('post', i, (B, To, post_chans[i]), 0.5) for i in range(npost)] if training else None
    post_cl, c.post_saved = _conv_stack_fwd(run, P, bufs, 'postnet.convolutions', npost,
                                            mel_cl.view(rowsP, Cm), To, [2] * (npost - 1) + [0],
                                            post_masks, training)
    mel = run.out_empty(B, Cm, To)
    mel_post = run.out_empty(B, Cm, To)
    nv.finalize_outputs(mel_cl, post_cl.view(B, To, Cm), mel, mel_post, olens32)

    c.run = run
    c.dec = d
    c.keep = dict(att=keep_att, dec=keep_dec, k0=k0, k1=k1)
    c.slabs = slabs
    c.tensors = dict(x0=x0, p1=p1, p2=p2, pm=pm, GA=GA, Wa_rec=Wa_rec, Wd_cat=Wd_cat, bias_d=bias_d,
                     Wq=Wq, U=U, Wpg=Wpg, mel_cl=mel_cl, vvec=vvec, lens32=lens32)
    return (mel, mel_post, gate, slabs['ALIGN']), c


def _backward(model, P, c, d_mel, d_post, d_gate, d_align):
    hp = model.hparams
    run = c.run
    g = {}
    B, Ti, To = c.B, c.Ti, c.To
    E = hp.encoder_embedding_dim
    Ha, Hd, Pd = hp.attention_rnn_dim, hp.decoder_rnn_dim, hp.prenet_dim
    Cm = hp.n_mel_channels
    He = E // 2
    A = nv.ATT_DIM
    rowsD, rowsE, rowsP = To * B, B * Ti, B * To
    S, T = c.slabs, c.tensors

    def cont(t):
        return t.contiguous() if t is not None else None

    sync = getattr(model, '_grad_sync', None)
    if sync is not None:
        sync.start(run.dev)

    def G(name, *shape):
        return sync.out(name, shape) if sync is not None else run.out_empty(*shape)

    own_shape = {n: tuple(P[n].shape) for n in (_ATT_Q, _ATT_M, _ATT_V, _ATT_D, _ATT_C)}
    P, embedded = _embed_attention(run, P)
    if embedded:
        G_own, staged = G, {}

        def G(name, *shape):
            if name in embedded:
                staged[name] = run.empty(*shape)
                return staged[name]
            return G_own(name, *shape)

    dmel_cl = run.empty(B, To, Cm)
    dpost_cl = run.empty(B, To, Cm)
    nv.grads_to_channel_last(cont(d_mel), cont(d_post), dmel_cl, dpost_cl)
    _conv_stack_bwd(run, P, g, 'postnet.convolutions', c.post_saved, dpost_cl.view(rowsP, Cm), To,
                    first_dx=dmel_cl.view(rowsP, Cm), first_dx_accumulate=True, G=G)
    if sync is not None:
        sync.bucket_ready('postnet')
    dout = run.empty(rowsD, Cm + 1)
    nv.gather_dout(dmel_cl, cont(d_gate), dout)

    Wpg = T['Wpg']
    DHC = run.empty(rowsD, Hd + E)
    _ng(run, DHC, dout, Wpg, b_kn=True)
    dWpg_h = run.empty(Cm + 1, Hd)
    dWpg_c = run.empty(Cm + 1, E)
    _rg(run, dWpg_h, dout, S['HD'].view(rowsD, Hd), a_km=True, b_kn=True)
    _rg(run, dWpg_c, dout, S['CTX'].view(rowsD, E), a_km=True, b_kn=True)
    dWp = G('decoder.linear_projection.linear_layer.weight', Cm, Hd + E)
    dWg = G('decoder.gate_layer.linear_layer.weight', 1, Hd + E)
    nv.copy2d(dWp[:, :Hd], dWpg_h[:Cm]); nv.copy2d(dWp[:, Hd:], dWpg_c[:Cm])
    nv.copy2d(dWg[:, :Hd], dWpg_h[Cm:]); nv.copy2d(dWg[:, Hd:], dWpg_c[Cm:])
    dbpg = run.empty(Cm + 1)
    run.colsum(dout, dbpg)
    dbp = G('decoder.linear_projection.linear_layer.bias', Cm)
    dbg = G('decoder.gate_layer.linear_layer.bias', 1)
    nv.copy2d(dbp.view(1, Cm), dbpg[:Cm].view(1, Cm))
    nv.copy2d(dbg.view(1, 1), dbpg[Cm:].view(1, 1))
    g['decoder.linear_projection.linear_layer.weight'] = dWp
    g['decoder.gate_layer.linear_layer.weight'] = dWg
    g['decoder.linear_projection.linear_layer.bias'] = dbp
    g['decoder.gate_layer.linear_layer.bias'] = dbg

    Wq = P['decoder.attention_layer.query_layer.linear_layer.weight']
    Wih_a, Whh_a = P['decoder.attention_rnn.weight_ih'], P['decoder.attention_rnn.weight_hh']
    Wih_d, Whh_d = P['decoder.decoder_rnn.weight_ih'], P['decoder.decoder_rnn.weight_hh']

    def transposed(src, rows, cols):
        Wt = run.empty(rows, cols)
        nv.transpose(Wt, src)
        return Wt

    Wa_recT = run.cached('Wa_recT', [Wih_a, Whh_a], lambda: transposed(T['Wa_rec'], E + Ha, 4 * Ha))
    Wd_catT = run.cached('Wd_catT', [Wih_d, Whh_d], lambda: transposed(T['Wd_cat'], Ha + E + Hd, 4 * Hd))
    ns = DGRAD_SPLIT
    bw = nv.DecTrainBwd()
    bw.f = c.dec
    bw.Wa_recT, bw.Wd_catT = nv.ptr(Wa_recT), nv.ptr(Wd_catT)
    bw.DHC = nv.ptr(DHC)
    bw.d_align = nv.ptr(cont(d_align))
    bw.nsplit = ns
    ring = DXD_RING if (DXD_RING >= 3 and nv.decoder_streams() == 1) else 0
    drop32 = GATE_GRADS_BF16_ONLY and BIAS_GRAD16 and run.bf16 and WGRAD16 and B % 8 == 0 and not nv.validate_only()
    out = dict(DGA=None if drop32 else run.empty(To, B, 4 * Ha), DGD=None if drop32 else run.empty(To, B, 4 * Hd), DCTX=run.empty(To, B, E),
               DQ=run.empty(To, B, A), d_pm=run.empty(B, Ti, A), dU_acc=run.empty(B, A, nv.LOC_TAPS),
               dv_acc=run.empty(B, A), dXd=run.empty(ring or To, ns, B, Ha + E + Hd), dXa=run.empty(ns, B, E + Ha),
               dc_a=run.empty(B, Ha), dc_d=run.empty(B, Hd), dwin_part=run.empty(nv.ATT_SLICES, B, 2, Ti),
               dcum_acc=run.empty(B, Ti), dq_h=run.empty(nv.ATT_SLICES, B, Ha))
    for k_, v_ in out.items():
        setattr(bw, k_, nv.ptr(v_))
    bw.dXd_ring = ring
    if run.bf16:
        slab16 = WGRAD16 and B % 8 == 0 and not nv.validate_only()
        nst = To if slab16 else 1
        b16 = dict(Wa_recT16=run.cached('Wa_recT16', [Wih_a, Whh_a], lambda: run.cast16(Wa_recT)),
                   Wd_catT16=run.cached('Wd_catT16', [Wih_d, Whh_d], lambda: run.cast16(Wd_catT)),
                   DGA16=run.empty16(nst, B, 4 * Ha), DGD16=run.empty16(nst, B, 4 * Hd))
        for k_, v_ in b16.items():
            setattr(bw, k_, nv.ptr(v_, torch.bfloat16))
        if slab16:
            bw.dg16_step_a, bw.dg16_step_d = B * 4 * Ha, B * 4 * Hd
    elif run.x3:
        b16 = dict(Wa_recT16=run.cached('Wa_recT16x3', [Wih_a, Whh_a], lambda: run.split16(Wa_recT)),
                   Wd_catT16=run.cached('Wd_catT16x3', [Wih_d, Whh_d], lambda: run.split16(Wd_catT)),
                   DGA16=run.empty16(1, B, 8 * Ha), DGD16=run.empty16(1, B, 8 * Hd))
        for k_, v_ in b16.items():
            setattr(bw, k_, nv.ptr(v_, torch.bfloat16))
    op16 = run.bf16 or run.x3
    model.last_train_decoder_bwd_path = _decoder_train_bwd(model, run, bw, out['dv_acc'],
                              reads=[Wa_recT, Wd_catT, DHC, cont(d_align), T['Wq'], T['U'], T['vvec'], T['pm'], c.memory,
                                     T['lens32'], T['GA'], c.keep['att'], c.keep['dec']]
                              + [S[k_] for k_ in ('HA', 'CA', 'GD', 'HD', 'CD', 'CTX', 'Q', 'ALIGN', 'CUM')]
                              + ([b16['Wa_recT16'], b16['Wd_catT16']] if op16 else [])
                              + ([c.bf16['memory16'], c.bf16['Wq16']] if run.bf16 else []),
                              writes=[v_ for v_ in out.values() if v_ is not None] + [S['attn_ws']] + ([b16['DGA16'], b16['DGD16']] if op16 else []))
    DGA, DGD, DCTX, DQ, d_pm = (out[k_] for k_ in ('DGA', 'DGD', 'DCTX', 'DQ', 'd_pm'))
    DGA2, DGD2 = (None, None) if drop32 else (DGA.view(rowsD, 4 * Ha), DGD.view(rowsD, 4 * Hd))

    Wdense = P['decoder.attention_layer.location_layer.location_dense.linear_layer.weight']
    Wconv = P['decoder.attention_layer.location_layer.location_conv.conv.weight']
    dWdense = G('decoder.attention_layer.location_layer.location_dense.linear_layer.weight', A, nv.LOC_FILTERS)
    dWconv = G('decoder.attention_layer.location_layer.location_conv.conv.weight', nv.LOC_FILTERS, 2, nv.LOC_KERNEL)
    dv = G('decoder.attention_layer.v.linear_layer.weight', 1, A)
    nv.unfold_location_grads(out['dU_acc'], out['dv_acc'], B, Wdense, Wconv, dWdense, dWconv, dv)
    g['decoder.attention_layer.location_layer.location_dense.linear_layer.weight'] = dWdense
    g['decoder.attention_layer.location_layer.location_conv.conv.weight'] = dWconv
    g['decoder.attention_layer.v.linear_layer.weight'] = dv
    dWq = G('decoder.attention_layer.query_layer.linear_layer.weight', A, Ha)
    _rg(run, dWq, DQ.view(rowsD, A), S['HA'].view(rowsD, Ha), a_km=True, b_kn=True)
    g['decoder.attention_layer.query_layer.linear_layer.weight'] = dWq

    dWih_a = G('decoder.attention_rnn.weight_ih', 4 * Ha, Pd + E)
    dWhh_a = G('decoder.attention_rnn.weight_hh', 4 * Ha, Ha)
    use16 = run.bf16 and WGRAD16 and B % 8 == 0 and not nv.validate_only()
    Z = c.bf16 if use16 else None
    if use16:
        _lstm_wgrad16(run, b16['DGA16'].view(rowsD, 4 * Ha), B, [(T['p2'], False), (Z['CTX16'].view(rowsD, E), True), (Z['HA16'].view(rowsD, Ha), True)],
                      [(dWih_a, 0, 2), (dWhh_a, 2, 3)])
    elif To > 1:
        tmp = run.empty(4 * Ha, Pd)
        _rg(run, tmp, DGA2, T['p2'], a_km=True, b_kn=True)
        nv.copy2d(dWih_a[:, :Pd], tmp)
        sh = (To - 1) * B
        tmp2 = run.empty(4 * Ha, E)
        _rg(run, tmp2, DGA2[B:], S['CTX'].view(rowsD, E)[:sh], a_km=True, b_kn=True)
        nv.copy2d(dWih_a[:, Pd:], tmp2)
        _rg(run, dWhh_a, DGA2[B:], S['HA'].view(rowsD, Ha)[:sh], a_km=True, b_kn=True)
    else:
        tmp = run.empty(4 * Ha, Pd)
        _rg(run, tmp, DGA2, T['p2'], a_km=True, b_kn=True)
        nv.copy2d(dWih_a[:, :Pd], tmp)
        nv.fill(dWhh_a, 0.0)
        z = run.zeros(4 * Ha, E)
        nv.copy2d(dWih_a[:, Pd:], z)
    db_a = G('decoder.attention_rnn.bias_ih', 4 * Ha)
    bias16 = use16 and BIAS_GRAD16
    if bias16:
        nv.colsum16(b16['DGA16'].view(rowsD, 4 * Ha), run.ws(4 * Ha), db_a)
    else:
        run.colsum(DGA2, db_a)
    db_a2 = G('decoder.attention_rnn.bias_hh', 4 * Ha)
    nv.copy2d(db_a2.view(1, -1), db_a.view(1, -1))
    g['decoder.attention_rnn.weight_ih'] = dWih_a
    g['decoder.attention_rnn.weight_hh'] = dWhh_a
    g['decoder.attention_rnn.bias_ih'] = db_a
    g['decoder.attention_rnn.bias_hh'] = db_a2

    dWih_d = G('decoder.decoder_rnn.weight_ih', 4 * Hd, Ha + E)
    dWhh_d = G('decoder.decoder_rnn.weight_hh', 4 * Hd, Hd)
    if use16:
        _lstm_wgrad16(run, b16['DGD16'].view(rowsD, 4 * Hd), B, [(Z['HA16'].view(rowsD, Ha), False), (Z['CTX16'].view(rowsD, E), False),
                                     (Z['HD16'].view(rowsD, Hd), True)], [(dWih_d, 0, 2), (dWhh_d, 2, 3)])
    else:
        tmp3 = run.empty(4 * Hd, Ha)
        _rg(run, tmp3, DGD2, S['HA'].view(rowsD, Ha), a_km=True, b_kn=True)
        nv.copy2d(dWih_d[:, :Ha], tmp3)
        tmp4 = run.empty(4 * Hd, E)
        _rg(run, tmp4, DGD2, S['CTX'].view(rowsD, E), a_km=True, b_kn=True)
        nv.copy2d(dWih_d[:, Ha:], tmp4)
        if To > 1:
            sh = (To - 1) * B
            _rg(run, dWhh_d, DGD2[B:], S['HD'].view(rowsD, Hd)[:sh], a_km=True, b_kn=True)
        else:
            nv.fill(dWhh_d, 0.0)
    db_d = G('decoder.decoder_rnn.bias_ih', 4 * Hd)
    if bias16:
        nv.colsum16(b16['DGD16'].view(rowsD, 4 * Hd), run.ws(4 * Hd), db_d)
    else:
        run.colsum(DGD2, db_d)
    db_d2 = G('decoder.decoder_rnn.bias_hh', 4 * Hd)
    nv.copy2d(db_d2.view(1, -1), db_d.view(1, -1))
    g['decoder.decoder_rnn.weight_ih'] = dWih_d
    g['decoder.decoder_rnn.weight_hh'] = dWhh_d
    g['decoder.decoder_rnn.bias_ih'] = db_d
    g['decoder.decoder_rnn.bias_hh'] = db_d2

    W2 = P['decoder.prenet.layers.1.linear_layer.weight']
    dp2 = run.empty(rowsD, Pd)
    if use16 and b16['DGA16'].shape[0] == To and (4 * Ha) % 64 == 0:
        WpT16 = run.cached('Wih_a_pT16', [Wih_a], lambda: Wih_a[:, :Pd].t().contiguous().to(torch.bfloat16))
        nv.gemm16_tn(dp2, b16['DGA16'].view(rowsD, 4 * Ha), WpT16)
    else:
        _ng(run, dp2, DGA2, Wih_a[:, :Pd], b_kn=True)
    nv.relu_dropout_bwd(dp2, T['p2'], 2.0)
    dW2 = G('decoder.prenet.layers.1.linear_layer.weight', Pd, Pd)
    _rg(run, dW2, dp2, T['p1'], a_km=True, b_kn=True)
    dp1 = run.empty(rowsD, Pd)
    _ng(run, dp1, dp2, W2, b_kn=True)
    nv.relu_dropout_bwd(dp1, T['p1'], 2.0)
    dW1 = G('decoder.prenet.layers.0.linear_layer.weight', Pd, Cm)
    _rg(run, dW1, dp1, T['x0'].view(rowsD, Cm), a_km=True, b_kn=True)
    g['decoder.prenet.layers.0.linear_layer.weight'] = dW1
    g['decoder.prenet.layers.1.linear_layer.weight'] = dW2

    Wmem = P['decoder.attention_layer.memory_layer.linear_layer.weight']
    dmem = run.empty(B, Ti, E)
    _ng(run, dmem[0], S['ALIGN'][0], DCTX[:, 0, :], a_km=True, b_kn=True, batch=B,
            strides=(To * Ti, E, Ti * E))
    _ng(run, dmem.view(rowsE, E), d_pm.view(rowsE, A), Wmem, b_kn=True, accumulate=True)
    dWmem = G('decoder.attention_layer.memory_layer.linear_layer.weight', A, E)
    _rg(run, dWmem, d_pm.view(rowsE, A), c.memory.view(rowsE, E), a_km=True, b_kn=True)
    g['decoder.attention_layer.memory_layer.linear_layer.weight'] = dWmem

    if embedded:
        for name, big in staged.items():
            g[name] = G_own(name, *own_shape[name])
            g[name].copy_(_crop_attention_grad(name, big, own_shape[name]))
    if sync is not None:
        sync.bucket_ready('decoder')
    dx3 = run.empty(rowsE, E)
    bdesc, DGs, keepalive = [], [], []
    for d, sfx in enumerate(('', '_reverse')):
        L = c.enc_lstm[d]
        WhhT = run.cached('enc_WhhT' + sfx, [L['Whh']], lambda L=L: transposed(L['Whh'], He, 4 * He))
        DG = run.empty(rowsE, 4 * He)
        desc = nv.LstmSeq()
        desc.B, desc.T, desc.H, desc.reverse = B, Ti, He, d
        desc.WhhT = nv.ptr(WhhT)
        desc.GX = nv.ptr(L['GX'])
        desc.C = nv.ptr(L['C'])
        desc.lens = nv.ptr(c.lens32, torch.int32)
        dout_view = dmem.view(rowsE, E)[:, d * He:(d + 1) * He]
        desc.dout, desc.ld_dout = nv.ptr(dout_view), E
        desc.DG = nv.ptr(DG)
        dX = run.empty(ENC_DGRAD_SPLIT, B, He)
        dc = run.empty(B, He)
        desc.dX, desc.dc, desc.dx_splits = nv.ptr(dX), nv.ptr(dc), ENC_DGRAD_SPLIT
        bdesc.append(desc)
        DGs.append(DG)
        keepalive.append((WhhT, dX, dc))
    model.last_encoder_bwd_path = _encoder_lstm_bwd(
        model, run, bdesc[0], bdesc[1], poison=DGs[0],
        reads=[k_[0] for k_ in keepalive] + [L_[k_] for L_ in c.enc_lstm for k_ in ('GX', 'C')] + [c.lens32, dmem],
        writes=DGs + [k_[i_] for k_ in keepalive for i_ in (1, 2)])
    for d, sfx in enumerate(('', '_reverse')):
        L, DG = c.enc_lstm[d], DGs[d]
        dWih = G('encoder.lstm.weight_ih_l0' + sfx, 4 * He, E)
        _rg(run, dWih, DG, c.x3, a_km=True, b_kn=True)
        dWhh = G('encoder.lstm.weight_hh_l0' + sfx, 4 * He, He)
        hview = c.memory.view(rowsE, E)[:, d * He:(d + 1) * He]
        _rg(run, dWhh, DG, hview, a_km=True, b_kn=True, convB=(Ti, He, 1 if d == 0 else -1))
        db = G('encoder.lstm.bias_ih_l0' + sfx, 4 * He)
        run.colsum(DG, db)
        db2 = G('encoder.lstm.bias_hh_l0' + sfx, 4 * He)
        nv.copy2d(db2.view(1, -1), db.view(1, -1))
        g['encoder.lstm.weight_ih_l0' + sfx] = dWih
        g['encoder.lstm.weight_hh_l0' + sfx] = dWhh
        g['encoder.lstm.bias_ih_l0' + sfx] = db
        g['encoder.lstm.bias_hh_l0' + sfx] = db2
        _ng(run, dx3, DG, L['Wih'], b_kn=True, accumulate=(d == 1))
    demb = run.empty(rowsE, E)
    _conv_stack_bwd(run, P, g, 'encoder.convolutions', c.enc_saved, dx3, Ti, first_dx=demb, G=G)
    dtable = G('embedding.weight', *P['embedding.weight'].shape)
    nv.embedding_bwd(c.text, demb, dtable)
    g['embedding.weight'] = dtable
    if sync is not None:
        sync.bucket_ready('encoder')
        sync.finish()
    return g


GC_FREEZE = os.environ.get('T2AMD_GC_FREEZE', '0') == '1'
_gc_state = {'train_forwards': 0, 'frozen': False}


def settle_gc(force=False, quiet=False):
    if _gc_state['frozen'] and not force:
        return False
    import gc
    gc.collect()
# ... 481 lines not shown
```

### tacotron2_amd/native.py

```python
import ctypes as C
import os

import torch

_HERE = os.path.dirname(os.path.abspath(__file__))
LIB_PATH = os.environ.get("T2AMD_LIB", os.path.join(_HERE, "lib", "libtacotron2_amd.so"))

TORCH_OPS_PATH = os.path.join(_HERE, "lib", "libtacotron2_amd_torch.so")

ATT_DIM = 128
LOC_FILTERS = 32
LOC_KERNEL = 31
LOC_TAPS = 62
ATT_SLICES = 4

_f32p = C.c_void_p
_i64 = C.c_longlong


class GemmDesc(C.Structure):
    _fields_ = [
        ("A", _f32p), ("B", _f32p), ("C", _f32p),
        ("M", C.c_int), ("N", C.c_int), ("K", C.c_int),
        ("lda", _i64), ("ldb", _i64), ("ldc", _i64),
        ("a_kcontig", C.c_int), ("b_kcontig", C.c_int),
        ("batch", C.c_int),
        ("strideA", _i64), ("strideB", _i64), ("strideC", _i64),
        ("splitk", C.c_int), ("strideSplitC", _i64),
        ("accumulate", C.c_int),
        ("bias", _f32p), ("act", C.c_int),
        ("keep", C.c_void_p), ("ldkeep", _i64), ("keep_scale", C.c_float),
        ("convA_T", C.c_int), ("convA_C", C.c_int), ("convA_pad", C.c_int), ("convA_sign", C.c_int),
        ("convB_T", C.c_int), ("convB_C", C.c_int), ("convB_pad", C.c_int),
        ("precision", C.c_int),
    ]


class Gemm16Desc(C.Structure):
    _fields_ = [
        ("A", C.c_void_p), ("B", C.c_void_p), ("C", _f32p),
        ("M", C.c_int), ("N", C.c_int), ("K", C.c_int),
        ("lda", _i64), ("ldb", _i64), ("ldc", _i64),
        ("splitk", C.c_int), ("strideSplitC", _i64), ("accumulate", C.c_int), ("bias", _f32p),
        ("win_T", C.c_int), ("win_Tp", C.c_int),
    ]


class Seg(C.Structure):
    _fields_ = [("p", _f32p), ("ld", _i64), ("width", C.c_int)]


class LstmStep(C.Structure):
    _fields_ = [
        ("x", Seg * 3), ("nseg", C.c_int),
        ("W", _f32p), ("Ktot", C.c_int), ("H", C.c_int), ("B", C.c_int),
        ("gin", _f32p), ("ld_gin", _i64),
        ("bias", _f32p),
        ("c_prev", _f32p), ("ld_cprev", _i64),
        ("gates_out", _f32p), ("ld_gates", _i64),
        ("c_out", _f32p), ("ld_c", _i64),
        ("h_out", _f32p), ("ld_h", _i64),
        ("keep", C.c_void_p), ("ld_keep", _i64), ("keep_scale", C.c_float),
        ("lens", C.c_void_p), ("t", C.c_int), ("tag", C.c_int),
        ("bf16", C.c_int), ("h16_out", C.c_void_p), ("ld_h16", _i64),
    ]


class SkinnyGemm(C.Structure):
    _fields_ = [
        ("x", Seg * 3), ("nseg", C.c_int),
        ("W", _f32p), ("Ktot", C.c_int), ("N", C.c_int), ("B", C.c_int),
        ("Y", _f32p), ("ldy", _i64), ("nsplit", C.c_int), ("split_stride", _i64), ("tag", C.c_int),
        ("bf16", C.c_int),
        ("bias", _f32p), ("act", C.c_int), ("keep", C.c_void_p), ("ld_keep", _i64), ("keep_scale", C.c_float),
        ("Y16", C.c_void_p), ("ldy16", _i64),
        ("stop_active", C.c_void_p), ("stop_lengths", C.c_void_p), ("stop_done", C.c_void_p),
        ("stop_col", C.c_int), ("stop_t", C.c_int), ("stop_max_steps", C.c_int), ("stop_threshold", C.c_float),
    ]


class Addend(C.Structure):
    _fields_ = [("p", _f32p), ("ld", _i64), ("nsplit", C.c_int), ("split_stride", _i64)]


class LstmBwd(C.Structure):
    _fields_ = [
        ("B", C.c_int), ("H", C.c_int),
        ("dh", Addend * 3),
        ("gates", _f32p), ("ld_gates", _i64),
        ("c_prev", _f32p), ("ld_cprev", _i64),
        ("c", _f32p), ("ld_c", _i64),
        ("keep", C.c_void_p), ("ld_keep", _i64), ("keep_scale", C.c_float),
        ("dc", _f32p), ("ld_dc", _i64),
        ("dgates", _f32p), ("ld_dgates", _i64),
        ("lens", C.c_void_p), ("t", C.c_int),
        ("dgates16", C.c_void_p), ("ld_dgates16", _i64),
        ("dgates16_x3", C.c_int),
    ]


class AttnFwd(C.Structure):
    _fields_ = [
        ("B", C.c_int), ("Ti", C.c_int), ("E", C.c_int), ("Hq", C.c_int),
        ("h", _f32p), ("ld_h", _i64),
        ("Wq", _f32p), ("U", _f32p), ("v", _f32p), ("pm", _f32p), ("memory", _f32p),
        ("lens", C.c_void_p),
        ("w_prev", _f32p), ("ld_wprev", _i64),
        ("cum", _f32p), ("cum_save", _f32p),
        ("w_out", _f32p), ("ld_wout", _i64),
        ("ctx_out", _f32p), ("ld_ctx", _i64),
        ("q_out", _f32p), ("ld_q", _i64),
        ("active", C.c_void_p),
        ("ws", _f32p),
        ("ctx16_out", C.c_void_p), ("ld_ctx16", _i64),
        ("loc_split_bf16", C.c_int),
        ("memory16", C.c_void_p),
        ("Wq16", C.c_void_p),
        ("ws_floats", _i64),
        ("ctx16_x3", C.c_int),
    ]


class AttnBwd(C.Structure):
    _fields_ = [
        ("B", C.c_int), ("Ti", C.c_int), ("E", C.c_int), ("Hq", C.c_int),
        ("dctx", Addend * 3),
        ("dctx_total", _f32p), ("ld_dctx_total", _i64),
        ("d_w_extra", _f32p), ("ld_dwextra", _i64),
        ("q", _f32p), ("ld_q", _i64),
        ("Wq", _f32p), ("U", _f32p), ("v", _f32p), ("pm", _f32p), ("memory", _f32p),
        ("lens", C.c_void_p),
        ("w", _f32p), ("ld_w", _i64),
        ("w_prev", _f32p), ("ld_wprev", _i64),
        ("cum_before", _f32p),
        ("dwin_part", _f32p), ("dcum_acc", _f32p),
        ("d_pm", _f32p), ("dU_acc", _f32p), ("dv_acc", _f32p),
        ("dq_out", _f32p), ("ld_dq", _i64),
        ("dh_out", _f32p), ("ld_dh", _i64), ("dh_split_stride", _i64),
        ("ws", _f32p),
        ("bf16", C.c_int),
        ("memory16", C.c_void_p),
        ("cell_q", C.POINTER(LstmBwd)), ("cell_x", C.POINTER(LstmBwd)),
        ("ws_floats", _i64),
        ("Wq16", C.c_void_p),
    ]


class DecTrain(C.Structure):
    _fields_ = [
        ("B", C.c_int), ("Ti", C.c_int), ("To", C.c_int), ("E", C.c_int), ("Ha", C.c_int), ("Hd", C.c_int),
        ("Wa_rec", _f32p), ("Wd_cat", _f32p), ("bias_d", _f32p), ("Wq", _f32p), ("U", _f32p), ("v", _f32p),
        ("GA", _f32p), ("memory", _f32p), ("pm", _f32p), ("lens", C.c_void_p),
        ("keep_att", C.c_void_p), ("keep_dec", C.c_void_p),
        ("scale_att", C.c_float), ("scale_dec", C.c_float),
        ("HA", _f32p), ("CA", _f32p), ("GD", _f32p), ("HD", _f32p), ("CD", _f32p), ("CTX", _f32p),
        ("Q", _f32p), ("ALIGN", _f32p), ("CUM", _f32p), ("cum_work", _f32p), ("attn_ws", _f32p),
        ("bf16", C.c_int), ("Wa_rec16", C.c_void_p), ("Wd_cat16", C.c_void_p),
        ("HA16", C.c_void_p), ("HD16", C.c_void_p), ("CTX16", C.c_void_p),
        ("memory16", C.c_void_p), ("Wq16", C.c_void_p),
    ]


class DecTrainBwd(C.Structure):
    _fields_ = [
        ("f", DecTrain),
        ("Wa_recT", _f32p), ("Wd_catT", _f32p), ("DHC", _f32p), ("d_align", _f32p),
        ("nsplit", C.c_int),
        ("DGA", _f32p), ("DGD", _f32p), ("DCTX", _f32p), ("DQ", _f32p), ("d_pm", _f32p),
        ("dU_acc", _f32p), ("dv_acc", _f32p),
        ("dXd", _f32p), ("dXa", _f32p), ("dc_a", _f32p), ("dc_d", _f32p),
        ("dwin_part", _f32p), ("dcum_acc", _f32p), ("dq_h", _f32p),
        ("Wa_recT16", C.c_void_p), ("Wd_catT16", C.c_void_p), ("DGA16", C.c_void_p), ("DGD16", C.c_void_p),
        ("dg16_step_a", _i64), ("dg16_step_d", _i64),
        ("dXd_ring", C.c_int),
    ]


class LstmSeq(C.Structure):
    _fields_ = [
        ("B", C.c_int), ("T", C.c_int), ("H", C.c_int), ("reverse", C.c_int),
        ("Whh", _f32p), ("WhhT", _f32p), ("GX", _f32p),
        ("out", _f32p), ("ld_out", _i64),
        ("C", _f32p), ("lens", C.c_void_p),
        ("dout", _f32p), ("ld_dout", _i64),
        ("DG", _f32p), ("dX", _f32p), ("dc", _f32p),
        ("dx_splits", C.c_int),
    ]


class SmallLinear(C.Structure):
    _fields_ = [
        ("X", _f32p), ("ldx", _i64), ("W", _f32p), ("ldw", _i64), ("bias", _f32p),
        ("Y", _f32p), ("ldy", _i64),
        ("B", C.c_int), ("N", C.c_int), ("K", C.c_int), ("act", C.c_int),
        ("keep", C.c_void_p), ("ldkeep", _i64), ("keep_scale", C.c_float),
    ]


class DecInfer(C.Structure):
    _fields_ = [
        ("B", C.c_int), ("Ti", C.c_int), ("E", C.c_int), ("Ha", C.c_int), ("Hd", C.c_int),
        ("P", C.c_int), ("C", C.c_int),
        ("t0", C.c_int), ("n_steps", C.c_int), ("max_steps", C.c_int),
        ("gate_threshold", C.c_float),
        ("W1", _f32p), ("W2", _f32p), ("Wa_cat", _f32p), ("bias_a", _f32p), ("Wd_cat", _f32p),
        ("bias_d", _f32p), ("Wq", _f32p), ("U", _f32p), ("v", _f32p), ("Wpg", _f32p), ("bias_pg", _f32p),
        ("memory", _f32p), ("pm", _f32p), ("lens", C.c_void_p), ("keep_prenet", C.c_void_p),
        ("h_a", _f32p), ("c_a", _f32p), ("c_d", _f32p), ("hc", _f32p), ("cum", _f32p),
        ("x_prenet", _f32p), ("gates", _f32p), ("zero_frame", _f32p), ("attn_ws", _f32p),
        ("PG", _f32p), ("ALIGN", _f32p), ("out_lengths", C.c_void_p), ("active", C.c_void_p),
        ("done_count", C.c_void_p),
        ("bf16", C.c_int), ("Wa_cat16", C.c_void_p), ("Wd_cat16", C.c_void_p),
        ("x_prenet16", C.c_void_p), ("h_a16", C.c_void_p), ("hc16", C.c_void_p),
        ("Wf", _f32p), ("bias_f", _f32p), ("memory16", C.c_void_p), ("Wq16", C.c_void_p),
        ("Wf16", C.c_void_p), ("Wpg16", C.c_void_p), ("W2_16", C.c_void_p), ("x_prenet1_16", C.c_void_p),
        ("attn_ws_floats", _i64),
    ]


class DecPersist(C.Structure):
    _fields_ = [
        ("Ti", C.c_int), ("E", C.c_int), ("H", C.c_int), ("P", C.c_int), ("C", C.c_int),
        ("max_steps", C.c_int), ("gate_threshold", C.c_float),
        ("Wa16", C.c_void_p), ("Wd16", C.c_void_p), ("bias_a", _f32p), ("bias_d", _f32p),
        ("Wq", _f32p), ("U", _f32p), ("v", _f32p), ("Wf", _f32p), ("bias_f", _f32p), ("W2", _f32p),
        ("memory", _f32p), ("pm", _f32p), ("keep_prenet", C.c_void_p),
        ("PG", _f32p), ("ALIGN", _f32p), ("out_length", C.c_void_p), ("status", C.c_void_p),
        ("steps_done", C.c_void_p), ("mailbox", C.c_void_p), ("trace", _f32p), ("timing", C.c_void_p),
        ("weights_f32", C.c_int),
    ]


PERSIST_TIMEOUT = 7
MAX_TENSORS = 64


class TensorList(C.Structure):
    _fields_ = [("param", C.c_void_p * MAX_TENSORS), ("grad", C.c_void_p * MAX_TENSORS),
                ("exp_avg", C.c_void_p * MAX_TENSORS), ("exp_avg_sq", C.c_void_p * MAX_TENSORS),
                ("numel", C.c_longlong * MAX_TENSORS), ("first_block", C.c_int * MAX_TENSORS), ("count", C.c_int)]


class AdamHyper(C.Structure):
    _fields_ = [("step_size", C.c_float), ("bc2_sqrt", C.c_float), ("one_minus_beta1", C.c_float),
                ("beta2", C.c_float), ("one_minus_beta2", C.c_float), ("eps", C.c_float), ("weight_decay", C.c_float)]


_STRUCTS = [GemmDesc, Seg, LstmStep, SkinnyGemm, Addend, LstmBwd, AttnFwd, AttnBwd, DecTrain,
            DecTrainBwd, LstmSeq, DecInfer, SmallLinear, TensorList, AdamHyper, DecPersist, Gemm16Desc]

SYMBOLS = [
    "t2amd_abi_version", "t2amd_source_sha1", "t2amd_last_error", "t2amd_struct_sizes", "t2amd_set_validate_only", "t2amd_profile_enable", "t2amd_profile_read", "t2amd_profile_event_overhead",
    "t2amd_gemm_f32", "t2amd_gemm_tile_size", "t2amd_splitk_reduce_f32", "t2amd_splitk_reduce2d_f32", "t2amd_gemm16_tn", "t2amd_gemm16_kk", "t2amd_gemm16_kk_group", "t2amd_transpose_cast_bf16", "t2amd_cast_halo_bf16", "t2amd_pack_conv_bf16",
    "t2amd_bn_stats_f32", "t2amd_bn_eval_invstd_f32", "t2amd_bn_act_fwd_f32", "t2amd_bn_act_bwd_f32", "t2amd_bn_act_bwd_img_f32", "t2amd_colsum_bf16", "t2amd_bn_act_fwd_img_f32",
    "t2amd_colsum_f32",
    "t2amd_embedding_fwd_f32", "t2amd_embedding_bwd_f32", "t2amd_philox_keep_mask", "t2amd_fill_f32",
    "t2amd_copy2d_f32", "t2amd_cast_bf16_f32", "t2amd_split_bf16x3_f32", "t2amd_transpose_f32", "t2amd_frames_to_time_major_f32",
    "t2amd_split_projection_f32", "t2amd_finalize_outputs_f32", "t2amd_grads_to_channel_last_f32",
    "t2amd_gather_dout_f32", "t2amd_relu_dropout_bwd_f32",
    "t2amd_lstm_step_fwd_f32", "t2amd_skinny_gemm_f32", "t2amd_lstm_pointwise_bwd_f32",
    "t2amd_lstm_step_fwd2_f32", "t2amd_skinny_gemm2_f32", "t2amd_lstm_pointwise_bwd2_f32",
    "t2amd_fold_location_f32", "t2amd_unfold_location_grads_f32",
    "t2amd_attention_step_fwd_f32", "t2amd_attention_step_bwd_f32",
    "t2amd_decoder_train_fwd_loop_f32", "t2amd_decoder_train_bwd_loop_f32",
    "t2amd_decoder_train_fwd_persistent_flag_bytes", "t2amd_decoder_train_fwd_persistent_supported", "t2amd_decoder_train_fwd_persistent_f32",
    "t2amd_lstm_seq_fwd_f32", "t2amd_lstm_seq_bwd_f32", "t2amd_decoder_infer_steps_f32",
    "t2amd_set_decoder_streams", "t2amd_set_bptt_cell_fold", "t2amd_get_bptt_cell_fold", "t2amd_attn_bwd_ws_floats",
    "t2amd_set_small_batch_max", "t2amd_get_small_batch_max", "t2amd_dec_infer_uses_tiles",
    "t2amd_set_attn_bwd_granules", "t2amd_attn_handoff_timeouts", "t2amd_set_attn_bwd_fused", "t2amd_attn_fwd_ws_floats", "t2amd_set_attn_fwd_fused", "t2amd_lstm_step_small_f32", "t2amd_linear_small_f32",
    "t2amd_lstm_seq_fwd2_f32", "t2amd_lstm_seq_bwd2_f32",
    "t2amd_lstm_seq_persistent_mailbox_bytes", "t2amd_lstm_seq_persistent_supported", "t2amd_lstm_seq_fwd2_persistent_f32",
    "t2amd_lstm_seq_batch_persistent_flag_bytes", "t2amd_lstm_seq_batch_persistent_supported", "t2amd_lstm_seq_fwd2_batch_persistent_f32", "t2amd_encoder_handoff_timeouts",
    "t2amd_lstm_seq_bwd2_batch_persistent_supported", "t2amd_lstm_seq_bwd2_batch_persistent_f32",
    "t2amd_reflect_pad_f32", "t2amd_reflect_index", "t2amd_stft_magnitude_f32", "t2amd_mel_log_compress_f32",
    "t2amd_gl_packed_rows", "t2amd_gl_overlap_add_f32", "t2amd_gl_project_f32", "t2amd_gl_rect_f32", "t2amd_stft_polar_f32",
    "t2amd_mel_decompress_f32",
    "t2amd_wg_layer_f32", "t2amd_wg_tail_f32", "t2amd_wg_denoise_f32", "t2amd_wg_head_f32", "t2amd_wg_nll_chunk", "t2amd_wg_nll_f32",
    "t2amd_wg_layer_train_f32", "t2amd_wg_head_save_f32", "t2amd_wg_head_bwd_rows", "t2amd_wg_head_bwd_f32",
    "t2amd_wg_partial_sum_f32", "t2amd_wg_gate_bwd_f32",
    "t2amd_wg_weight_norm_short", "t2amd_wg_weight_norm_f32", "t2amd_wg_weight_norm_bwd_f32",
    "t2amd_optim_chunk", "t2amd_grad_norm_f32", "t2amd_adam_step_f32",
    "t2amd_decoder_persist_mailbox_bytes", "t2amd_decoder_persist_supported", "t2amd_decoder_infer_persistent_f32",
    "t2amd_loss_workspace_doubles", "t2amd_tacotron2_loss_fwd_f32", "t2amd_tacotron2_loss_bwd_f32",
    "t2amd_hg_conv_f32", "t2amd_hg_upsample_f32", "t2amd_hg_post_f32", "t2amd_hg_pack_mel_f32",
]

_P, _I, _L, _F, _UL = C.c_void_p, C.c_int, C.c_longlong, C.c_float, C.c_ulonglong


def _argtypes():
    pt = C.POINTER
    return {
        "t2amd_gemm_f32": [pt(GemmDesc), _P],
        "t2amd_gemm_tile_size": [_I, _I, _I, _I, _I, _I],
        "t2amd_splitk_reduce_f32": [_P, _I, _L, _P, _L, _I, _I, _I, _P],
        "t2amd_splitk_reduce2d_f32": [_P, _I, _L, _P, _I, _I, _L, _I, _P],
        "t2amd_gemm16_tn": [pt(Gemm16Desc), _P],
        "t2amd_gemm16_kk": [pt(Gemm16Desc), _P],
        "t2amd_gemm16_kk_group": [pt(Gemm16Desc), _I, _P],
        "t2amd_transpose_cast_bf16": [_P, _I, _L, _P, _L, _I, _I, _I, _P],
        "t2amd_cast_halo_bf16": [_P, _L, _P, _L, _I, _I, _I, _P],
        "t2amd_pack_conv_bf16": [_P, _P, _I, _I, _I, _I, _I, _P],
        "t2amd_bn_stats_f32": [_P, _L, _I, _I, _P, _P, _P, _P, _P, _F, _F, _P],
        "t2amd_bn_eval_invstd_f32": [_P, _P, _I, _F, _P],
        "t2amd_bn_act_fwd_f32": [_P, _L, _P, _L, _I, _I, _P, _P, _P, _P, _I, _P, _L, _F, _P, _I, _P],
        "t2amd_bn_act_fwd_img_f32": [_P, _L, _P, _L, _I, _I, _P, _P, _P, _P, _I, _P, _L, _F, _P, _I, _I, _P],
        "t2amd_bn_act_bwd_f32": [_P, _L, _P, _L, _P, _L, _I, _I, _P, _P, _P, _I, _P, _L, _F, _P, _P, _P, _P],
        "t2amd_bn_act_bwd_img_f32": [_P, _L, _P, _L, _P, _L, _I, _I, _P, _P, _P, _I, _P, _L, _F, _P, _P, _P, _P, _I, _I, _P, _I, _P],
        "t2amd_colsum_f32": [_P, _L, _I, _I, _P, _P, _I, _P],
        "t2amd_colsum_bf16": [_P, _L, _I, _I, _P, _P, _I, _P],
        "t2amd_embedding_fwd_f32": [_P, _P, _P, _L, _I, _I, _P],
        "t2amd_embedding_bwd_f32": [_P, _P, _P, _P, _L, _I, _I, _P],
        "t2amd_philox_keep_mask": [_P, _L, _F, _UL, _UL, _P],
        "t2amd_fill_f32": [_P, _L, _F, _P],
        "t2amd_cast_bf16_f32": [_P, _P, _L, _P],
        "t2amd_split_bf16x3_f32": [_P, _L, _P, _L, _L, _I, _P],
        "t2amd_copy2d_f32": [_P, _L, _P, _L, _P, _L, _I, _I, _P],
        "t2amd_transpose_f32": [_P, _L, _P, _L, _I, _I, _I, _L, _L, _P],
        "t2amd_frames_to_time_major_f32": [_P, _P, _I, _I, _I, _P],
        "t2amd_split_projection_f32": [_P, _P, _P, _P, _I, _I, _I, _P],
        "t2amd_finalize_outputs_f32": [_P, _P, _P, _P, _P, _I, _I, _I, _P],
        "t2amd_grads_to_channel_last_f32": [_P, _P, _P, _P, _I, _I, _I, _P],
        "t2amd_gather_dout_f32": [_P, _P, _P, _I, _I, _I, _P],
        "t2amd_relu_dropout_bwd_f32": [_P, _P, _F, _L, _P],
        "t2amd_lstm_step_fwd_f32": [pt(LstmStep), _P],
        "t2amd_skinny_gemm_f32": [pt(SkinnyGemm), _P],
        "t2amd_lstm_pointwise_bwd_f32": [pt(LstmBwd), _P],
        "t2amd_lstm_step_fwd2_f32": [pt(LstmStep), pt(LstmStep), _P],
        "t2amd_skinny_gemm2_f32": [pt(SkinnyGemm), pt(SkinnyGemm), _P],
        "t2amd_lstm_pointwise_bwd2_f32": [pt(LstmBwd), pt(LstmBwd), _P],
        "t2amd_fold_location_f32": [_P, _P, _P, _P],
        "t2amd_unfold_location_grads_f32": [_P, _P, _I, _P, _P, _P, _P, _P, _P],
        "t2amd_attention_step_fwd_f32": [pt(AttnFwd), _P],
        "t2amd_attention_step_bwd_f32": [pt(AttnBwd), _P],
        "t2amd_decoder_train_fwd_loop_f32": [pt(DecTrain), _P],
        "t2amd_decoder_train_fwd_persistent_flag_bytes": [_I, _I],
        "t2amd_decoder_train_fwd_persistent_supported": [pt(DecTrain), _I],
        "t2amd_decoder_train_fwd_persistent_f32": [pt(DecTrain), _P, _P, _P, _P],
        "t2amd_decoder_train_bwd_loop_f32": [pt(DecTrainBwd), _P],
        "t2amd_lstm_seq_fwd_f32": [pt(LstmSeq), _P],
        "t2amd_lstm_seq_bwd_f32": [pt(LstmSeq), _P],
        "t2amd_lstm_seq_fwd2_f32": [pt(LstmSeq), pt(LstmSeq), _P],
        "t2amd_lstm_seq_bwd2_f32": [pt(LstmSeq), pt(LstmSeq), _P],
        "t2amd_lstm_seq_persistent_mailbox_bytes": [_I, _I],
        "t2amd_lstm_seq_persistent_supported": [pt(LstmSeq)],
        "t2amd_lstm_seq_fwd2_persistent_f32": [pt(LstmSeq), pt(LstmSeq), _P, _P, _P],
        "t2amd_lstm_seq_batch_persistent_flag_bytes": [_I, _I, _I],
        "t2amd_lstm_seq_batch_persistent_supported": [pt(LstmSeq), _I, _I],
        "t2amd_lstm_seq_fwd2_batch_persistent_f32": [pt(LstmSeq), pt(LstmSeq), _P, _P, _P, _P],
        "t2amd_lstm_seq_bwd2_batch_persistent_supported": [pt(LstmSeq), _I, _I],
        "t2amd_lstm_seq_bwd2_batch_persistent_f32": [pt(LstmSeq), pt(LstmSeq), _P, _P, _P, _P],
        "t2amd_encoder_handoff_timeouts": [_I],
        "t2amd_decoder_infer_steps_f32": [pt(DecInfer), _P],
        "t2amd_struct_sizes": [pt(C.c_int), _I],
        "t2amd_set_validate_only": [_I],
        "t2amd_set_decoder_streams": [_I],
        "t2amd_set_bptt_cell_fold": [_I],
        "t2amd_get_bptt_cell_fold": [],
        "t2amd_set_small_batch_max": [_I],
        "t2amd_get_small_batch_max": [_I],
        "t2amd_dec_infer_uses_tiles": [_I, _I, _I, _I, _I, _I],
        "t2amd_attn_bwd_ws_floats": [_I, _I],
        "t2amd_set_attn_bwd_granules": [_I],
        "t2amd_attn_handoff_timeouts": [_I],
        "t2amd_set_attn_bwd_fused": [_I],
        "t2amd_attn_fwd_ws_floats": [_I, _I],
        "t2amd_set_attn_fwd_fused": [_I],
        "t2amd_lstm_step_small_f32": [pt(LstmStep), _P],
        "t2amd_linear_small_f32": [pt(SmallLinear), _P],
        "t2amd_profile_enable": [_I, _I],
        "t2amd_profile_read": [pt(C.c_float), pt(C.c_int)],
        "t2amd_profile_event_overhead": [pt(C.c_float)],
        "t2amd_reflect_pad_f32": [_P, _L, _P, _L, _I, _I, _I, _I, _P],
        "t2amd_stft_magnitude_f32": [_P, _L, _P, _L, _L, _I, _I, _P],
        "t2amd_mel_log_compress_f32": [_P, _L, _P, _I, _I, _I, _F, _P],
        "t2amd_gl_overlap_add_f32": [_P, _L, _P, _P, _P, _I, _L, _I, _I, _F, _P, _L, _L, _I, _P],
        "t2amd_gl_project_f32": [_P, _L, _P, _L, _P, _P, _I, _L, _I, _I, _I, _I, _P, _L, _P],
        "t2amd_gl_rect_f32": [_P, _P, _L, _P, _P, _I, _L, _I, _I, _I, _I, _P, _L, _P, _L, _P],
        "t2amd_stft_polar_f32": [_P, _L, _I, _I, _I, _P, _P, _P],
        "t2amd_mel_decompress_f32": [_P, _I, _I, _I, _P, _P, _P, _L, _P],
        "t2amd_wg_layer_f32": [_P, _L, _P, _P, _I, _I, _I, _I, _I, _I, _P, _L, _P, _L, _P, _L, _I, _P, _L, _I, _P, _I, _P],
        "t2amd_wg_tail_f32": [_P, _L, _I, _P, _P, _I, _P, _P, _L, _P, _L, _L, _I, _F, _P, _P, _P, _L, _P, _L, _P, _P, _L,
                              _I, _P],
        "t2amd_wg_denoise_f32": [_P, _P, _I, _I, _L, _F, _P],
        "t2amd_wg_head_f32": [_P, _L, _I, _P, _P, _I, _P, _L, _L, _P, _L, _P, _L, _P, _L, _L, _I, _I, _P, _P, _P, _P, _L, _P,
                              _P, _L, _I, _I, _L, _P],
        "t2amd_wg_nll_chunk": [],
        "t2amd_wg_nll_f32": [_P, _L, _L, _I, _P, _L, _L, _I, _P, _I, _L, _P, _L, _P, _P],
        "t2amd_wg_layer_train_f32": [_P, _L, _P, _P, _I, _I, _I, _I, _I, _I, _P, _L, _P, _L, _P, _L, _I, _P, _L, _I, _P, _P, _L,
                                     _P, _L, _I, _P],
        "t2amd_wg_head_save_f32": [_P, _L, _I, _P, _P, _I, _P, _L, _L, _P, _L, _P, _L, _P, _L, _L, _I, _I, _P, _P, _P, _P, _L,
                                   _P, _P, _L, _I, _I, _L, _P, _L, _P],
        "t2amd_wg_head_bwd_rows": [],
        "t2amd_wg_head_bwd_f32": [_P, _L, _I, _P, _I, _P, _L, _L, _P, _L, _P, _L, _P, _L, _P, _L, _P, _L, _P, _P, _I, _P, _L,
                                  _P, _L, _P, _P, _L, _I, _I, _L, _F, _F, _P],
        "t2amd_wg_partial_sum_f32": [_P, _L, _L, _P, _P],
        "t2amd_wg_gate_bwd_f32": [_P, _L, _P, _L, _P, _L, _I, _P, _L, _P, _L, _P],
        "t2amd_wg_weight_norm_short": [],
        "t2amd_wg_weight_norm_f32": [_P, _I, _L, _P, _P, _P, _P, _P],
        "t2amd_wg_weight_norm_bwd_f32": [_P, _I, _L, _P, _P, _P, _P, _P, _P, _F, _P],
        "t2amd_optim_chunk": [],
        "t2amd_grad_norm_f32": [pt(TensorList), _F, _P, _P, _P],
        "t2amd_adam_step_f32": [pt(TensorList), pt(AdamHyper), _P, _P],
        "t2amd_decoder_persist_mailbox_bytes": [_I, _I, _I, _I],
        "t2amd_decoder_persist_supported": [pt(DecPersist)],
        "t2amd_decoder_infer_persistent_f32": [pt(DecPersist), _P],
        "t2amd_loss_workspace_doubles": [],
        "t2amd_tacotron2_loss_fwd_f32": [_P, _P, _P, _L, _P, _P, _L, _P, _P, _P],
        "t2amd_tacotron2_loss_bwd_f32": [_P, _P, _P, _L, _P, _P, _L, _P, _P, _P, _P, _P],
        "t2amd_hg_conv_f32": [_P, _L, _L, _L, _I, _P, _L, _P, _I, _I, _I, _I, _F, _P, _L, _L, _P, _L, _L, _F, _I, _P, _L, _I,
                              _I, _P],
        "t2amd_hg_upsample_f32": [_P, _L, _L, _L, _I, _P, _L, _P, _I, _I, _I, _I, _F, _P, _L, _L, _P, _L, _I, _I, _P],
        "t2amd_hg_post_f32": [_P, _L, _L, _L, _I, _P, _L, _P, _F, _P, _P, _L, _I, _P, _L, _L, _P],
        "t2amd_hg_pack_mel_f32": [_P, _L, _I, _I, _L, _P, _P, _L, _P, _I, _L, _P],
    }


_lib = None


class NativeError(RuntimeError):
    pass


def load():
    global _lib
    if _lib is not None:
        return _lib
    if not os.path.exists(LIB_PATH):
        raise NativeError(
            "tacotron2_amd: %s not found. The MI355X engine has no fallback path; build it with "
            "`python -m tacotron2_amd.build` (needs hipcc)." % LIB_PATH)
    lib = C.CDLL(LIB_PATH)
    for name in SYMBOLS:
        if not hasattr(lib, name):
            raise NativeError("tacotron2_amd: symbol %s missing from %s" % (name, LIB_PATH))
    for name, at in _argtypes().items():
        fn = getattr(lib, name)
        fn.argtypes = at
        fn.restype = C.c_int
    lib.t2amd_last_error.restype = C.c_char_p
    lib.t2amd_reflect_index.argtypes = [_L, _L]
    lib.t2amd_reflect_index.restype = C.c_longlong
    lib.t2amd_gl_packed_rows.argtypes = [_P, _I, _I, _I]
    lib.t2amd_gl_packed_rows.restype = C.c_longlong
    lib.t2amd_abi_version.restype = C.c_int
    lib.t2amd_attn_bwd_ws_floats.restype = C.c_longlong
    lib.t2amd_attn_fwd_ws_floats.restype = C.c_longlong
    lib.t2amd_decoder_persist_mailbox_bytes.restype = C.c_longlong
    lib.t2amd_lstm_seq_persistent_mailbox_bytes.restype = C.c_longlong
    lib.t2amd_lstm_seq_batch_persistent_flag_bytes.restype = C.c_longlong
    lib.t2amd_decoder_train_fwd_persistent_flag_bytes.restype = C.c_longlong
    if lib.t2amd_abi_version() != 1:
        raise NativeError("tacotron2_amd: ABI version mismatch")
    lib.t2amd_source_sha1.restype = C.c_char_p
    lib.t2amd_source_sha1.argtypes = []
    built = (lib.t2amd_source_sha1() or b"").decode()
    if os.path.isdir(os.path.join(_HERE, "csrc")) and os.environ.get("T2AMD_ALLOW_STALE_LIB", "0") != "1":
        from . import build as _build
        try:
            want = _build.source_sha1()
        except OSError as e:
            want = None
            if os.environ.get("T2AMD_REQUIRE_SOURCE_HASH", "0") == "1":
                raise NativeError("tacotron2_amd: cannot hash the kernel sources beside %s (%s)" % (LIB_PATH, e))
            import sys
            print("tacotron2_amd: warning: the kernel sources beside %s could not be hashed (%s); the library (built from %s) "
                  "is loaded WITHOUT the stale-library check (T2AMD_REQUIRE_SOURCE_HASH=1 makes this an error)"
                  % (LIB_PATH, e, built or "<unstamped sources>"), file=sys.stderr, flush=True)
        if want is not None and built != want:
            raise NativeError("tacotron2_amd: %s was built from other sources (binary %s, sources %s): run "
                              "`python -m tacotron2_amd.build` (or set T2AMD_ALLOW_STALE_LIB=1 to use it anyway)"
                              % (LIB_PATH, built or "<unstamped>", want))
    sizes = (C.c_int * 32)()
    n = lib.t2amd_struct_sizes(sizes, 32)
    if n != len(_STRUCTS):
# ... 80 lines not shown

def decoder_streams():
    return _decoder_streams


def set_bptt_cell_fold(on):
    _check(load().t2amd_set_bptt_cell_fold(1 if on else 0), "t2amd_set_bptt_cell_fold")


def get_bptt_cell_fold():
    return int(load().t2amd_get_bptt_cell_fold())


def set_small_batch_max(n):
    _check(load().t2amd_set_small_batch_max(int(n)), "t2amd_set_small_batch_max")


def small_batch_max(bf16=0):
    return int(load().t2amd_get_small_batch_max(int(bf16)))


def dec_infer_uses_tiles(B, bf16, E, Ha, Hd, P):
    return bool(load().t2amd_dec_infer_uses_tiles(int(B), int(bf16), int(E), int(Ha), int(Hd), int(P)))


def small_batch_max_setting():
    a, b = small_batch_max(0), small_batch_max(1)
    return -1 if a != b else a


def set_validate_only(on):
    global _validate_only
    load().t2amd_set_validate_only(1 if on else 0)
    _validate_only = bool(on)


def validate_only():
    return _validate_only


def profile_enable(tag, max_launches):
    _check(load().t2amd_profile_enable(tag, max_launches), "t2amd_profile_enable")


def profile_event_overhead():
    ms = C.c_float(0)
    _check(load().t2amd_profile_event_overhead(C.byref(ms)), "t2amd_profile_event_overhead")
    return ms.value


def profile_read():
    ms, n = C.c_float(0), C.c_int(0)
    _check(load().t2amd_profile_read(C.byref(ms), C.byref(n)), "t2amd_profile_read")
    return ms.value, n.value


def _check(rc, what):
    if rc != 0:
        msg = _lib.t2amd_last_error()
        raise NativeError("%s failed (code %d): %s" % (what, rc, msg.decode() if msg else "?"))


def _stream():
    if _validate_only:
        return None
    return C.c_void_p(torch.cuda.current_stream().cuda_stream)


def ptr(t, dtype=torch.float32):
    if t is None:
        return None
    if not t.is_cuda and not _validate_only:
        raise NativeError("tacotron2_amd: expected a device (HIP) tensor, got a %s tensor; the engine "
                          "has no CPU path" % t.device)
    if dtype is not None and t.dtype != dtype:
        raise NativeError("tacotron2_amd: expected %s, got %s" % (dtype, t.dtype))
    return C.c_void_p(t.data_ptr())


def _mat(t, dtype=torch.float32):
    if t.dim() != 2 or (t.shape[1] > 1 and t.stride(1) != 1):
        raise NativeError("expected a 2-D tensor with contiguous rows, got shape %s stride %s"
                          % (tuple(t.shape), t.stride()))
    ld = t.stride(0) if t.shape[0] > 1 else max(t.stride(0), t.shape[1])
    return ptr(t, dtype), ld, t.shape[0], t.shape[1]


def _fullc(t):
    if not t.is_contiguous():
        raise NativeError("expected a contiguous tensor, got shape %s stride %s" % (tuple(t.shape), t.stride()))
    return t


def scale_for(p):
    return float(torch.tensor(1.0, dtype=torch.float32) / torch.tensor(1.0 - p, dtype=torch.float32))


def gemm_tile_size(M, N, precision, nz=1, a_km=False, b_kn=False):
    return int(load().t2amd_gemm_tile_size(int(M), int(N), int(precision), int(nz), 0 if a_km else 1, 0 if b_kn else 1))


def gemm(Cm, A, B, a_km=False, b_kn=False, accumulate=False, bias=None, act=0, keep=None,
         keep_scale=1.0, convA=None, convB=None, batch=1, strides=(0, 0, 0), splitk=1, partials=None,
         fast=False):
    lib = load()
    d = GemmDesc()
    pa, lda, r0, c0 = _mat(A)
    pb, ldb, r1, c1 = _mat(B)
    pc, ldc, M, N = _mat(Cm)
    Ka, Ma = (r0, c0) if a_km else (c0, r0)
    Kb, Nb = (r1, c1) if b_kn else (c1, r1)
    if convA is not None:
        if a_km or Ka != convA[1] or Kb % convA[1] != 0:
            raise NativeError("gemm: convA needs A=[rows,C] and K(B) a multiple of C")
        K = Kb
    else:
        K = Ka
    if convB is not None:
        if not b_kn or Nb != convB[1] or N % convB[1] != 0:
            raise NativeError("gemm: convB needs B=[rows,C] (b_kn) and N(C) a multiple of C")
        Nb = N
    if Ma != M or Nb != N or Kb != K:
        raise NativeError("gemm: shape mismatch C=%s A=%s B=%s (a_km=%s b_kn=%s K=%d)"
                          % (tuple(Cm.shape), tuple(A.shape), tuple(B.shape), a_km, b_kn, K))
    d.A, d.B, d.C = pa, pb, pc
    d.M, d.N, d.K = M, N, K
    d.lda, d.ldb, d.ldc = lda, ldb, ldc
    d.a_kcontig = 0 if a_km else 1
    d.b_kcontig = 0 if b_kn else 1
    d.batch = batch
    d.strideA, d.strideB, d.strideC = strides
    d.splitk = splitk
    d.precision = int(fast)
    d.accumulate = 1 if accumulate else 0
    d.bias = ptr(bias)
    d.act = act
    if keep is not None:
        if keep.dim() != 2 or tuple(keep.shape) != (M, N) or keep.stride(1) != 1:
            raise NativeError("gemm: keep mask must be a [M,N] uint8 view, got %s" % (tuple(keep.shape),))
        d.keep, d.ldkeep, d.keep_scale = ptr(keep, torch.uint8), keep.stride(0), keep_scale
    if convA is not None:
        d.convA_T, d.convA_C, d.convA_pad, d.convA_sign = convA
    if convB is not None:
        d.convB_T, d.convB_C, d.convB_pad = convB
    if splitk > 1:
        if partials is None or partials.numel() < splitk * M * N or not partials.is_contiguous():
            raise NativeError("gemm: split-K needs a contiguous partials buffer")
        d.C = ptr(partials)
        d.ldc = N
        d.strideSplitC = M * N
    _check(lib.t2amd_gemm_f32(C.byref(d), _stream()), "t2amd_gemm_f32")


def gemm16_tn(Cm, A16, B16, K=None, splitk=1, partials=None, accumulate=False, bias=None):
    lib = load()
    d = Gemm16Desc()
    pa, lda, M, Ka = _mat(A16, torch.bfloat16)
    pb, ldb, N, Kb = _mat(B16, torch.bfloat16)
    K = Ka if K is None else K
    if K > Ka or K > Kb or Cm.shape[0] != M or Cm.shape[1] != N:
        raise NativeError("gemm16_tn: shape mismatch A=%s B=%s C=%s K=%d" % (tuple(A16.shape), tuple(B16.shape), tuple(Cm.shape), K))
    d.A, d.B, d.M, d.N, d.K, d.lda, d.ldb = pa, pb, M, N, K, lda, ldb
    d.splitk = splitk
    if splitk > 1:
        if partials is None or partials.numel() < splitk * M * N:
            raise NativeError("gemm16_tn: split-K needs a (splitk, M*N) partials buffer")
        d.C, d.ldc, d.strideSplitC = ptr(partials), N, M * N
    else:
        d.C, d.ldc = _mat(Cm)[:2]
    d.accumulate = 1 if accumulate else 0
    d.bias = ptr(bias)
    _check(lib.t2amd_gemm16_tn(C.byref(d), _stream()), "t2amd_gemm16_tn")


def conv16(Cm, img16, W16, B, T, pad, bias=None, accumulate=False):
    lib = load()
    d = Gemm16Desc()
    Ci = img16.shape[1]
    Tp = T + 2 * pad
    pw, ldw, Co, K = _mat(W16, torch.bfloat16)
    klen = (2 * pad + 1) * Ci
    if img16.shape[0] < B * Tp + 2 * pad or K < klen or K - klen > 2 * pad * Ci or Cm.shape[0] != B * T or Cm.shape[1] != Co:
        raise NativeError("conv16: shape mismatch img=%s W=%s C=%s" % (tuple(img16.shape), tuple(W16.shape), tuple(Cm.shape)))
    d.A, d.lda = ptr(_fullc(img16), torch.bfloat16), Ci
    d.B, d.ldb = pw, ldw
    d.C, d.ldc = _mat(Cm)[:2]
    d.M, d.N, d.K = (B - 1) * Tp + T, Co, K
    d.splitk, d.accumulate, d.bias = 1, 1 if accumulate else 0, ptr(bias)
    d.win_T, d.win_Tp = T, Tp
    _check(lib.t2amd_gemm16_tn(C.byref(d), _stream()), "t2amd_gemm16_tn")


def _kk_desc(Cm, A16, B16, K, M=None, N=None, lda=None, ldb=None, splitk=1, partials=None, accumulate=False, bias=None):
    d = Gemm16Desc()
    pa, lda0, ra, wa = _mat(A16, torch.bfloat16)
    pb, ldb0, rb, wb = _mat(B16, torch.bfloat16)
    M = wa if M is None else M
    N = wb if N is None else N
    lda = lda0 if lda is None else lda
    ldb = ldb0 if ldb is None else ldb
    span_a = (ra - 1) * lda0 + wa
    span_b = (rb - 1) * ldb0 + wb
    if K < 1 or (K - 1) * lda + M > span_a or (K - 1) * ldb + N > span_b or Cm.shape[0] != M or Cm.shape[1] != N:
        raise NativeError("gemm16_kk: shape mismatch A=%s B=%s C=%s M=%d N=%d K=%d lda=%d ldb=%d"
                          % (tuple(A16.shape), tuple(B16.shape), tuple(Cm.shape), M, N, K, lda, ldb))
    d.A, d.B, d.M, d.N, d.K, d.lda, d.ldb = pa, pb, M, N, K, lda, ldb
    d.splitk = splitk
    if splitk > 1:
        if partials is None or partials.numel() < splitk * M * N:
            raise NativeError("gemm16_kk: split-K needs a (splitk, M*N) partials buffer")
        d.C, d.ldc, d.strideSplitC = ptr(partials), N, M * N
    else:
        d.C, d.ldc = _mat(Cm)[:2]
    d.accumulate = 1 if accumulate else 0
    d.bias = ptr(bias)
    return d


def gemm16_kk(Cm, A16, B16, K, M=None, N=None, lda=None, ldb=None, splitk=1, partials=None, accumulate=False, bias=None):
    d = _kk_desc(Cm, A16, B16, K, M, N, lda, ldb, splitk, partials, accumulate, bias)
    _check(load().t2amd_gemm16_kk(C.byref(d), _stream()), "t2amd_gemm16_kk")


def gemm16_kk_group(problems):
    if not 1 <= len(problems) <= 4:
        raise NativeError("gemm16_kk_group: 1..4 problems, got %d" % len(problems))
    arr = (Gemm16Desc * len(problems))(*[_kk_desc(**kw) for kw in problems])
    reads = [kw[k_] for kw in problems for k_ in ('A16', 'B16')]
    writes = [kw['partials'] if kw.get('partials') is not None else kw['Cm'] for kw in problems]
    if not _via_ops("wgrad_gemm16", [arr], reads, writes):
        _check(load().t2amd_gemm16_kk_group(arr, len(problems), _stream()), "t2amd_gemm16_kk_group")


def pack_conv_bf16(W, reversed=False):
    Co, Ci, k = W.shape
    rows, inner = (Ci, Co) if reversed else (Co, Ci)
    Kp = (k * inner + 63) // 64 * 64
    out = torch.empty(rows, Kp, dtype=torch.bfloat16, device=W.device)
    _check(load().t2amd_pack_conv_bf16(ptr(_fullc(W)), ptr(out, torch.bfloat16), Co, Ci, k, Kp, 1 if reversed else 0, _stream()),
           "t2amd_pack_conv_bf16")
    return out


def cast_halo_bf16(src, dst, T, pad):
    ps, lds, rows, Cc = _mat(src)
    if dst.dtype != torch.bfloat16 or dst.shape[1] != Cc or dst.shape[0] < (rows // T) * (T + 2 * pad) + 2 * pad:
        raise NativeError("cast_halo_bf16: shape mismatch src=%s dst=%s" % (tuple(src.shape), tuple(dst.shape)))
    _check(load().t2amd_cast_halo_bf16(ps, _i64(lds), ptr(_fullc(dst), torch.bfloat16), _i64(rows), Cc, T, pad, _stream()),
           "t2amd_cast_halo_bf16")


def transpose_cast_bf16(src, dst, rows_padded=None):
    lib = load()
    is16 = src.dtype == torch.bfloat16
    ps, lds, rows, cols = _mat(src, torch.bfloat16 if is16 else torch.float32)
    pd, ldd, c2, rp = _mat(dst, torch.bfloat16)
    rows_padded = rp if rows_padded is None else rows_padded
    if c2 != cols or rows_padded < rows or rows_padded > rp:
        raise NativeError("transpose_cast_bf16: shape mismatch src=%s dst=%s" % (tuple(src.shape), tuple(dst.shape)))
    _check(lib.t2amd_transpose_cast_bf16(ps, 1 if is16 else 0, _i64(lds), pd, _i64(ldd), rows, cols, rows_padded, _stream()),
           "t2amd_transpose_cast_bf16")


def splitk_reduce(partials, nsplit, out, accumulate=False, perm_taps=0, perm_ci=0):
    lib = load()
    n = out.numel()
    _fullc(out)
    _check(lib.t2amd_splitk_reduce_f32(ptr(partials), nsplit, _i64(n), ptr(out), _i64(n),
                                       1 if accumulate else 0, perm_taps, perm_ci, _stream()),
           "t2amd_splitk_reduce_f32")


def splitk_reduce2d(partials, nsplit, out, accumulate=False):
    po, ldo, rows, cols = _mat(out)
    _check(load().t2amd_splitk_reduce2d_f32(ptr(partials), nsplit, _i64(rows * cols), po, rows, cols, _i64(ldo),
                                            1 if accumulate else 0, _stream()), "t2amd_splitk_reduce2d_f32")


def bn_stats(x, ws, mean, invstd, running_mean=None, running_var=None, momentum=0.1, eps=1e-5):
    lib = load()
    px, ldx, M, N = _mat(x)
    _check(lib.t2amd_bn_stats_f32(px, _i64(ldx), M, N, ptr(ws, torch.float64), ptr(mean), ptr(invstd),
                                  ptr(running_mean), ptr(running_var), C.c_float(momentum), C.c_float(eps),
                                  _stream()), "t2amd_bn_stats_f32")


def bn_eval_invstd(running_var, invstd, eps=1e-5):
    lib = load()
    _check(lib.t2amd_bn_eval_invstd_f32(ptr(running_var), ptr(invstd), running_var.numel(), C.c_float(eps),
                                        _stream()), "t2amd_bn_eval_invstd_f32")


def bn_act_fwd(x, y, mean, invstd, gamma, beta, act, keep=None, keep_scale=1.0, lens=None, T=0):
    lib = load()
    px, ldx, M, N = _mat(x)
    py, ldy, M2, N2 = _mat(y)
    assert (M, N) == (M2, N2)
    pk, ldk = (None, 0)
    if keep is not None:
        assert tuple(keep.shape) == (M, N) and keep.stride(1) == 1
        pk, ldk = ptr(keep, torch.uint8), keep.stride(0)
    _check(lib.t2amd_bn_act_fwd_f32(px, _i64(ldx), py, _i64(ldy), M, N, ptr(mean), ptr(invstd), ptr(gamma),
                                    ptr(beta), act, pk, _i64(ldk), C.c_float(keep_scale),
                                    ptr(lens, torch.int32), T, _stream()), "t2amd_bn_act_fwd_f32")


def bn_act_fwd_img(x, y, mean, invstd, gamma, beta, act, keep, keep_scale, y_img, T, pad):
    lib = load()
    px, ldx, M, N = _mat(x)
    py, ldy, M2, N2 = _mat(y)
    assert (M, N) == (M2, N2)
    pk, ldk = (None, 0)
    if keep is not None:
        assert tuple(keep.shape) == (M, N) and keep.stride(1) == 1
        pk, ldk = ptr(keep, torch.uint8), keep.stride(0)
    assert y_img.is_contiguous() and y_img.dtype == torch.bfloat16 and tuple(y_img.shape) == ((M // T) * (T + 2 * pad) + 2 * pad, N)
    _check(lib.t2amd_bn_act_fwd_img_f32(px, _i64(ldx), py, _i64(ldy), M, N, ptr(mean), ptr(invstd), ptr(gamma), ptr(beta), act, pk,
                                        _i64(ldk), C.c_float(keep_scale), ptr(y_img, torch.bfloat16), int(T), int(pad), _stream()),
           "t2amd_bn_act_fwd_img_f32")


def bn_act_bwd(dy, y, x, mean, invstd, gamma, act, keep, keep_scale, ws, dgamma, dbeta):
    lib = load()
    pd, ldd, M, N = _mat(dy)
    py, ldy, _, _ = _mat(y)
    px, ldx, _, _ = _mat(x)
    pk, ldk = (None, 0)
    if keep is not None:
        assert tuple(keep.shape) == (M, N) and keep.stride(1) == 1
        pk, ldk = ptr(keep, torch.uint8), keep.stride(0)
    _check(lib.t2amd_bn_act_bwd_f32(pd, _i64(ldd), py, _i64(ldy), px, _i64(ldx), M, N, ptr(mean), ptr(invstd),
                                    ptr(gamma), act, pk, _i64(ldk), C.c_float(keep_scale),
                                    ptr(ws, torch.float64), ptr(dgamma), ptr(dbeta), _stream()),
           "t2amd_bn_act_bwd_f32")


def bn_act_bwd_img(dy, y, x, mean, invstd, gamma, act, keep, keep_scale, ws, dgamma, dbeta, dx_img, T, pad, dbias, keep_f32=False):
    lib = load()
    pd, ldd, M, N = _mat(dy)
    py, ldy, _, _ = _mat(y)
    px, ldx, _, _ = _mat(x)
    pk, ldk = (None, 0)
    if keep is not None:
        assert tuple(keep.shape) == (M, N) and keep.stride(1) == 1
        pk, ldk = ptr(keep, torch.uint8), keep.stride(0)
    assert dx_img.is_contiguous() and dx_img.dtype == torch.bfloat16 and tuple(dx_img.shape) == ((M // T) * (T + 2 * pad) + 2 * pad, N)
    assert dbias.numel() == N
    _check(lib.t2amd_bn_act_bwd_img_f32(pd, _i64(ldd), py, _i64(ldy), px, _i64(ldx), M, N, ptr(mean), ptr(invstd),
                                        ptr(gamma), act, pk, _i64(ldk), C.c_float(keep_scale),
                                        ptr(ws, torch.float64), ptr(dgamma), ptr(dbeta), ptr(dx_img, torch.bfloat16), int(T), int(pad),
                                        ptr(dbias), 1 if keep_f32 else 0, _stream()),
           "t2amd_bn_act_bwd_img_f32")


def colsum(x, ws, out, accumulate=False):
    lib = load()
    px, ldx, M, N = _mat(x)
    assert out.numel() == N
    _check(lib.t2amd_colsum_f32(px, _i64(ldx), M, N, ptr(ws, torch.float64), ptr(out), 1 if accumulate else 0,
                                _stream()), "t2amd_colsum_f32")


def colsum16(x16, ws, out, accumulate=False):
    lib = load()
    assert x16.dtype == torch.bfloat16 and x16.dim() == 2 and x16.stride(1) == 1 and out.numel() == x16.shape[1]
    _check(lib.t2amd_colsum_bf16(ptr(x16, torch.bfloat16), _i64(x16.stride(0)), x16.shape[0], x16.shape[1], ptr(ws, torch.float64),
                                 ptr(out), 1 if accumulate else 0, _stream()), "t2amd_colsum_bf16")


def embedding_fwd(ids, table, out):
    lib = load()
    rows = ids.numel()
    _check(lib.t2amd_embedding_fwd_f32(ptr(_fullc(ids), torch.int64), ptr(_fullc(table)), ptr(_fullc(out)),
                                       _i64(rows), table.shape[1], table.shape[0], _stream()),
           "t2amd_embedding_fwd_f32")


def embedding_bwd(ids, dout, dtable, ws=None):
    lib = load()
    rows = ids.numel()
    _check(lib.t2amd_embedding_bwd_f32(ptr(_fullc(ids), torch.int64), ptr(_fullc(dout)), ptr(_fullc(dtable)),
                                       None, _i64(rows), dtable.shape[1], dtable.shape[0], _stream()),
           "t2amd_embedding_bwd_f32")


def philox_keep_mask(out, p, seed, offset=0):
    lib = load()
    _check(lib.t2amd_philox_keep_mask(ptr(_fullc(out), torch.uint8), _i64(out.numel()), C.c_float(p),
                                      C.c_ulonglong(seed), C.c_ulonglong(offset), _stream()),
           "t2amd_philox_keep_mask")


def fill(t, v):
    lib = load()
    _check(lib.t2amd_fill_f32(ptr(_fullc(t)), _i64(t.numel()), C.c_float(v), _stream()), "t2amd_fill_f32")


def copy2d(dst, src, src2=None):
    lib = load()
    pd, ldd, R, Cc = _mat(dst)
    ps, lds, R1, C1 = _mat(src)
    assert (R, Cc) == (R1, C1), (dst.shape, src.shape)
    p2, ld2 = (None, 0)
    if src2 is not None:
        p2, ld2, R2, C2 = _mat(src2)
        assert (R, Cc) == (R2, C2)
    _check(lib.t2amd_copy2d_f32(ps, _i64(lds), p2, _i64(ld2), pd, _i64(ldd), R, Cc, _stream()), "t2amd_copy2d_f32")


def transpose(dst, src, batch=1, sstride=0, dstride=0):
    lib = load()
    ps, lds, R, Cc = _mat(src)
    pd, ldd, R1, C1 = _mat(dst)
    assert (R1, C1) == (Cc, R), (dst.shape, src.shape)
    _check(lib.t2amd_transpose_f32(ps, _i64(lds), pd, _i64(ldd), R, Cc, batch, _i64(sstride), _i64(dstride),
                                   _stream()), "t2amd_transpose_f32")


def frames_to_time_major(mels, x0):
    lib = load()
    B, Cm, To = mels.shape
    assert tuple(x0.shape) == (To, B, Cm)
    _check(lib.t2amd_frames_to_time_major_f32(ptr(_fullc(mels)), ptr(_fullc(x0)), B, Cm, To, _stream()),
           "t2amd_frames_to_time_major_f32")


def split_projection(pg, mel_cl, gate, out_lens):
    lib = load()
    B, To, Cm = mel_cl.shape
    assert pg.numel() == To * B * (Cm + 1)
    _check(lib.t2amd_split_projection_f32(ptr(_fullc(pg)), ptr(_fullc(mel_cl)), ptr(_fullc(gate)),
                                          ptr(out_lens, torch.int32), B, Cm, To, _stream()),
           "t2amd_split_projection_f32")


def finalize_outputs(mel_cl, post_cl, mel, mel_post, out_lens):
    lib = load()
    B, To, Cm = mel_cl.shape
    _check(lib.t2amd_finalize_outputs_f32(ptr(_fullc(mel_cl)), ptr(post_cl), ptr(_fullc(mel)), ptr(mel_post),
                                          ptr(out_lens, torch.int32), B, Cm, To, _stream()),
           "t2amd_finalize_outputs_f32")


def grads_to_channel_last(dmel, dmel_post, dmel_cl, dpost_cl):
    lib = load()
    B, To, Cm = dmel_cl.shape
    _check(lib.t2amd_grads_to_channel_last_f32(ptr(dmel), ptr(dmel_post), ptr(_fullc(dmel_cl)),
                                               ptr(_fullc(dpost_cl)), B, Cm, To, _stream()),
           "t2amd_grads_to_channel_last_f32")


def gather_dout(dmel_cl, dgate, dout):
    lib = load()
    B, To, Cm = dmel_cl.shape
    _check(lib.t2amd_gather_dout_f32(ptr(_fullc(dmel_cl)), ptr(dgate), ptr(_fullc(dout)), B, Cm, To, _stream()),
           "t2amd_gather_dout_f32")


def relu_dropout_bwd(dy, y, scale):
    lib = load()
    assert dy.shape == y.shape
    _check(lib.t2amd_relu_dropout_bwd_f32(ptr(_fullc(dy)), ptr(_fullc(y)), C.c_float(scale), _i64(dy.numel()),
                                          _stream()), "t2amd_relu_dropout_bwd_f32")


def _seg(t, width, dtype=torch.float32, x3=False):
    s = Seg()
    if t is None:
        s.p, s.ld, s.width = None, width, width
    else:
        p, ld, _, cols = _mat(t, dtype)
        if x3:
            if cols != 2 * width or ld % 2:
                raise NativeError("split-bf16 segment: expected %d columns (2 per k), got %d (ld %d)" % (2 * width, cols, ld))
            ld //= 2
        else:
            assert cols == width
        s.p, s.ld, s.width = p, ld, width
    return s


def lstm_step_fwd(xs, widths, W, H, B, gates_out, c_out, h_out, gin=None, bias=None, c_prev=None,
                  keep=None, keep_scale=1.0, lens=None, t=0, small=False, bf16=False, h16_out=None):
    lib = load()
    a = LstmStep()
    a.nseg = len(xs)
    x3 = bf16 == 3 and bf16 is not True
    odt = torch.bfloat16 if bf16 else torch.float32
    for i, (x, w) in enumerate(zip(xs, widths)):
        a.x[i] = _seg(x, w, odt, x3)
    a.W = ptr(_fullc(W), odt)
    a.bf16 = 3 if x3 else (1 if bf16 else 0)
    if h16_out is not None:
        a.h16_out, a.ld_h16 = _mat(h16_out, torch.bfloat16)[:2]
        if x3:
            a.ld_h16 //= 2
    a.Ktot, a.H, a.B = sum(widths), H, B
    if gin is not None:
        a.gin, a.ld_gin = _mat(gin)[:2]
    a.bias = ptr(bias)
    if c_prev is not None:
        a.c_prev, a.ld_cprev = _mat(c_prev)[:2]
    a.gates_out, a.ld_gates = _mat(gates_out)[:2]
    a.c_out, a.ld_c = _mat(c_out)[:2]
    a.h_out, a.ld_h = _mat(h_out)[:2]
    if keep is not None:
        a.keep, a.ld_keep, a.keep_scale = ptr(keep, torch.uint8), keep.stride(0), keep_scale
    a.lens = ptr(lens, torch.int32)
    a.t = t
    if small:
        _check(lib.t2amd_lstm_step_small_f32(C.byref(a), _stream()), "t2amd_lstm_step_small_f32")
    else:
        _check(lib.t2amd_lstm_step_fwd_f32(C.byref(a), _stream()), "t2amd_lstm_step_fwd_f32")


def linear_small(X, W, Y, bias=None, act=0, keep=None, keep_scale=1.0):
    lib = load()
    a = SmallLinear()
    a.X, a.ldx, Bx, K = _mat(X)
    a.W, a.ldw, N, Kw = _mat(W)
    a.Y, a.ldy, By, Ny = _mat(Y)
    if K != Kw or N != Ny or Bx != By:
        raise NativeError("linear_small: shape mismatch")
    a.B, a.N, a.K, a.act = Bx, N, K, act
    a.bias = ptr(bias)
    if keep is not None:
        a.keep, a.ldkeep, a.keep_scale = ptr(keep, torch.uint8), keep.stride(0), keep_scale
    _check(lib.t2amd_linear_small_f32(C.byref(a), _stream()), "t2amd_linear_small_f32")


def skinny_gemm(xs, widths, W, N, B, Y, nsplit=1, bf16=False, bias=None, act=0, keep=None, keep_scale=1.0):
    lib = load()
    a = SkinnyGemm()
    a.nseg = len(xs)
    x3 = bf16 == 3 and bf16 is not True
    odt = torch.bfloat16 if bf16 else torch.float32
    for i, (x, w) in enumerate(zip(xs, widths)):
        a.x[i] = _seg(x, w, odt, x3)
    a.W = ptr(_fullc(W), odt)
    a.bf16 = 3 if x3 else (1 if bf16 else 0)
    a.Ktot, a.N, a.B = sum(widths), N, B
    _fullc(Y)
    a.Y, a.ldy, a.nsplit, a.split_stride = ptr(Y), N, nsplit, B * N
    if bias is not None:
        a.bias = ptr(_fullc(bias))
    a.act = int(act)
    if keep is not None:
        a.keep, a.ld_keep, a.keep_scale = ptr(_fullc(keep), torch.uint8), keep.stride(0), keep_scale
    _check(lib.t2amd_skinny_gemm_f32(C.byref(a), _stream()), "t2amd_skinny_gemm_f32")


def _addend(t, nsplit=1, split_stride=0):
    a = Addend()
    if t is None:
        a.p, a.ld, a.nsplit, a.split_stride = None, 0, 1, 0
    else:
        p, ld, _, _ = _mat(t)
        a.p, a.ld, a.nsplit, a.split_stride = p, ld, nsplit, split_stride
    return a


def lstm_bwd_desc(B, H, dh_list, gates, c_prev, c, keep, keep_scale, dc, dgates, lens=None, t=0, dgates16=None, x3=False):
    a = LstmBwd()
    a.B, a.H = B, H
    for i in range(3):
        d = dh_list[i] if i < len(dh_list) else None
        a.dh[i] = _addend(*d) if isinstance(d, tuple) else _addend(d)
    a.gates, a.ld_gates = _mat(gates)[:2]
    if c_prev is not None:
        a.c_prev, a.ld_cprev = _mat(c_prev)[:2]
    a.c, a.ld_c = _mat(c)[:2]
    if keep is not None:
        a.keep, a.ld_keep, a.keep_scale = ptr(keep, torch.uint8), keep.stride(0), keep_scale
    a.dc, a.ld_dc = _mat(dc)[:2]
    a.dgates, a.ld_dgates = _mat(dgates)[:2]
    a.lens = ptr(lens, torch.int32)
    a.t = t
    if dgates16 is not None:
        a.dgates16, a.ld_dgates16 = ptr(dgates16, torch.bfloat16), dgates16.stride(0)
        if x3:
            a.ld_dgates16, a.dgates16_x3 = dgates16.stride(0) // 2, 1
    return a


def lstm_pointwise_bwd2(a, b=None):
    _check(load().t2amd_lstm_pointwise_bwd2_f32(C.byref(a), C.byref(b) if b is not None else None, _stream()),
           "t2amd_lstm_pointwise_bwd2_f32")


def lstm_pointwise_bwd(B, H, dh_list, gates, c_prev, c, keep, keep_scale, dc, dgates, lens=None, t=0):
    lib = load()
    a = LstmBwd()
    a.B, a.H = B, H
    for i in range(3):
        a.dh[i] = _addend(dh_list[i] if i < len(dh_list) else None)
    a.gates, a.ld_gates = _mat(gates)[:2]
    if c_prev is not None:
        a.c_prev, a.ld_cprev = _mat(c_prev)[:2]
    a.c, a.ld_c = _mat(c)[:2]
    if keep is not None:
        a.keep, a.ld_keep, a.keep_scale = ptr(keep, torch.uint8), keep.stride(0), keep_scale
    a.dc, a.ld_dc = _mat(dc)[:2]
    a.dgates, a.ld_dgates = _mat(dgates)[:2]
    a.lens = ptr(lens, torch.int32)
    a.t = t
    _check(lib.t2amd_lstm_pointwise_bwd_f32(C.byref(a), _stream()), "t2amd_lstm_pointwise_bwd_f32")

# ... 824 lines not shown
```

Before: 645,100 valid mel-frames/s.

## Route prenet and decoder projection GEMMs through bf16 MFMA with fused epilogues

Adds gemm16 epilogue extensions (ReLU, dropout keep-mask, a bf16 copy of C, row-limited stores and a split second destination). These let the prenet layers, the decoder mel/gate projection and its backward dgrad/wgrad run as bf16 MFMA GEMMs instead of the previous exact f32 paths. New kernels fuse the time-major transpose and the dout gather with emitting padded bf16 copies, so separate cast passes are not needed. This cuts f32 GEMM work and extra casts, at the cost of lower precision in the prenet and projection and more branching in the GEMM epilogue.

```diff
diff --git a/include/tacotron2_amd.h b/include/tacotron2_amd.h
--- a/include/tacotron2_amd.h
+++ b/include/tacotron2_amd.h
@@ -69,6 +69,17 @@
     int accumulate;
     const float* bias;
     int win_T, win_Tp;
+    int act;
+    const uint8_t* keep;
+    long long ldkeep;
+    float keep_scale;
+    void* C16;
+    long long ldc16;
+    int n16;
+    int m_store;
+    float* C2;
+    int c2_row;
+    long long ldc2;
 } t2amd_gemm16_desc;
 int t2amd_gemm16_tn(const t2amd_gemm16_desc* d, void* stream);
 int t2amd_gemm16_kk(const t2amd_gemm16_desc* d, void* stream);
@@ -118,6 +129,7 @@
 int t2amd_transpose_f32(const float* src, long long lds, float* dst, long long ldd, int rows,
                         int cols, int batch, long long sstride, long long dstride, void* stream);
 int t2amd_frames_to_time_major_f32(const float* mels, float* x0, int B, int C, int To, void* stream);
+int t2amd_frames_to_time_major_bf16(const float* mels, float* x0, void* x16, int ld16, int B, int C, int To, void* stream);
 int t2amd_split_projection_f32(const float* pg, float* mel_cl, float* gate, const int* out_lens,
                                int B, int C, int To, void* stream);
 int t2amd_finalize_outputs_f32(float* mel_cl, const float* post_cl, float* mel, float* mel_post,
@@ -126,6 +138,8 @@
                                     float* dpost_cl, int B, int C, int To, void* stream);
 int t2amd_gather_dout_f32(const float* dmel_cl, const float* dgate, float* dout, int B, int C,
                           int To, void* stream);
+int t2amd_gather_dout_bf16(const float* dmel_cl, const float* dgate, float* dout, void* dout16, int ld16, int B, int C,
+                           int To, void* stream);
 int t2amd_relu_dropout_bwd_f32(float* dy, const float* y, float scale, long long n, void* stream);
 
 typedef struct t2amd_seg {
diff --git a/tacotron2_amd/csrc/elementwise.hip b/tacotron2_amd/csrc/elementwise.hip
--- a/tacotron2_amd/csrc/elementwise.hip
+++ b/tacotron2_amd/csrc/elementwise.hip
@@ -945,6 +945,36 @@
     return T2AMD_OK;
 }
 
+__global__ void frames_to_tm16_kernel(const float* __restrict__ mels, float* __restrict__ x0, unsigned short* __restrict__ x16, int ld16,
+                                      int B, int C, int To) {
+    __shared__ float tile[32][33];
+    const int b = blockIdx.z;
+    const int t0 = blockIdx.x * 32, c0 = blockIdx.y * 32;
+    const int tx = threadIdx.x & 31, ty = threadIdx.x >> 5;
+    for (int j = ty; j < 32; j += 8) {
+        const int c = c0 + j, t = t0 + tx;
+        float v = 0.f;
+        if (c < C && t < To && t >= 1) v = mels[((long long)b * C + c) * To + (t - 1)];
+        tile[j][tx] = v;
+    }
+    __syncthreads();
+    for (int j = ty; j < 32; j += 8) {
+        const int t = t0 + j, c = c0 + tx;
+        if (t >= To) continue;
+        const long long row = (long long)t * B + b;
+        if (c < C) x0[row * C + c] = tile[tx][j];
+        if (c < ld16) x16[row * ld16 + c] = c < C ? t2_f32_to_bf16(tile[tx][j]) : (unsigned short)0;
+    }
+}
+extern "C" int t2amd_frames_to_time_major_bf16(const float* mels, float* x0, void* x16, int ld16, int B, int C, int To, void* stream) {
+    T2_REQUIRE(mels && x0 && x16 && B > 0 && C > 0 && To > 0 && ld16 >= C && ld16 % 8 == 0, "frames_to_tm16: bad args (ld16 >= C, a multiple of 8)");
+    dim3 grid(t2_cdiv(To, 32), t2_cdiv(ld16, 32), B);
+    T2_REQUIRE(grid.y <= 65535 && grid.z <= 65535, "frames_to_tm16: grid too large");
+    T2_LAUNCH(frames_to_tm16_kernel, grid, dim3(256), 0, (hipStream_t)stream, mels, x0, (unsigned short*)x16, ld16, B, C, To);
+    T2_LAUNCH_CHECK();
+    return T2AMD_OK;
+}
+
 __global__ void split_projection_kernel(const float* __restrict__ pg, float* __restrict__ mel_cl,
                                         float* __restrict__ gate, const int* __restrict__ out_lens, int B, int C,
                                         int To) {
@@ -1081,6 +1111,31 @@
     return T2AMD_OK;
 }
 
+__global__ void gather_dout16_kernel(const float* __restrict__ dmel_cl, const float* __restrict__ dgate, float* __restrict__ dout,
+                                     unsigned short* __restrict__ dout16, int ld16, int B, int C, int To) {
+    const long long total = (long long)To * B * ld16;
+    for (long long i = blockIdx.x * (long long)blockDim.x + threadIdx.x; i < total; i += (long long)gridDim.x * blockDim.x) {
+        const long long row = i / ld16;
+        const int c = (int)(i - row * ld16);
+        const int t = (int)(row / B), b = (int)(row - (long long)t * B);
+        float v = 0.f;
+        if (c < C) v = dmel_cl[((long long)b * To + t) * C + c];
+        else if (c == C) v = dgate ? dgate[(long long)b * To + t] : 0.f;
+        if (c <= C) dout[row * (C + 1) + c] = v;
+        dout16[i] = c <= C ? t2_f32_to_bf16(v) : (unsigned short)0;
+    }
+}
+extern "C" int t2amd_gather_dout_bf16(const float* dmel_cl, const float* dgate, float* dout, void* dout16, int ld16, int B, int C, int To,
+                                      void* stream) {
+    T2_REQUIRE(dmel_cl && dout && dout16 && B > 0 && C > 0 && To > 0 && ld16 >= C + 1 && ld16 % 8 == 0,
+               "gather_dout16: bad args (ld16 >= C + 1, a multiple of 8)");
+    int blocks = t2_cdiv((long long)To * B * ld16, 256);
+    if (blocks > 8192) blocks = 8192;
+    T2_LAUNCH(gather_dout16_kernel, dim3(blocks), dim3(256), 0, (hipStream_t)stream, dmel_cl, dgate, dout, (unsigned short*)dout16, ld16, B, C, To);
+    T2_LAUNCH_CHECK();
+    return T2AMD_OK;
+}
+
 __global__ void relu_dropout_bwd_kernel(float* __restrict__ dy, const float* __restrict__ y, float scale, long long n) {
     for (long long i = blockIdx.x * (long long)blockDim.x + threadIdx.x; i < n; i += (long long)gridDim.x * blockDim.x)
         dy[i] = (y[i] > 0.f) ? dy[i] * scale : 0.f;
diff --git a/tacotron2_amd/csrc/gemm16.hip b/tacotron2_amd/csrc/gemm16.hip
--- a/tacotron2_amd/csrc/gemm16.hip
+++ b/tacotron2_amd/csrc/gemm16.hip
@@ -159,6 +159,8 @@
 #undef G16_TILE
 
     float* __restrict__ C = d.C + (long long)split * d.strideSplitC;
+    unsigned short* __restrict__ c16 = reinterpret_cast<unsigned short*>(d.C16);
+    const int mst = d.m_store > 0 ? d.m_store : M;
 #pragma unroll
     for (int tm = 0; tm < 4; ++tm) {
 #pragma unroll
@@ -174,16 +176,36 @@
                     live = live && t_ < d.win_T;
                     crow = (long long)b_ * d.win_T + t_;
                 }
+                live = live && gm < mst;
                 if (live && gn < N) {
-                    float* cp = C + crow * d.ldc + gn;
+                    float* cp = (d.C2 && gm >= d.c2_row) ? d.C2 + (long long)(gm - d.c2_row) * d.ldc2 + gn : C + crow * d.ldc + gn;
                     float val = acc[tm][tn][r];
                     if (d.bias) val += d.bias[gn];
                     if (d.accumulate) val += *cp;
+                    if (d.act == 1) val = fmaxf(val, 0.f);
+                    if (d.keep) val = d.keep[(long long)gm * d.ldkeep + gn] ? val * d.keep_scale : 0.f;
                     *cp = val;
+                    if (c16) c16[(long long)gm * d.ldc16 + gn] = t2_f32_to_bf16(val);
+                } else if (live && c16 && gn < d.n16) {
+                    c16[(long long)gm * d.ldc16 + gn] = 0;
                 }
             }
         }
     }
+}
+
+static bool g16_check_epilogue(const t2amd_gemm16_desc& d, bool tn) {
+    const bool ext = d.act != 0 || d.keep || d.C16 || d.C2 || d.m_store != 0;
+    if (!ext) return true;
+    if (d.splitk != 1 || d.win_Tp != 0) return false;
+    if (d.act != 0 && d.act != 1) return false;
+    if (!tn && (d.act != 0 || d.keep || d.C16)) return false;
+    if (d.keep && d.ldkeep < d.N) return false;
+    if (d.C16 && (d.n16 < d.N || d.ldc16 < d.n16 || d.n16 > t2_cdiv(d.N, G16_T) * G16_T || d.C2 || d.m_store != 0)) return false;
+    if (d.m_store < 0 || d.m_store > d.M) return false;
+    const int rows = d.m_store > 0 ? d.m_store : d.M;
+    if (d.C2 && (d.c2_row <= 0 || d.c2_row >= rows || d.ldc2 < d.N)) return false;
+    return true;
 }
 
 extern "C" int t2amd_gemm16_tn(const t2amd_gemm16_desc* dp, void* stream) {
@@ -199,6 +221,8 @@
     T2_REQUIRE(d.win_Tp > 0 || d.lda >= d.K, "gemm16: lda must be >= K unless the rows are windows");
     if (d.splitk < 1) d.splitk = 1;
     T2_REQUIRE(d.splitk == 1 || (!d.bias && !d.accumulate), "gemm16: split-K needs a plain epilogue");
+    T2_REQUIRE(g16_check_epilogue(d, true), "gemm16: bad epilogue extension (act 0/1; keep / C16 / C2 / m_store need splitk 1 and no window; "
+               "ldc16 >= n16 >= N with n16 inside the last column tile; 0 < c2_row < rows stored; ldkeep, ldc2 >= N)");
     const int nkt = d.K / G16_BK;
     p.ktiles_per_split = t2_cdiv(nkt, d.splitk);
     dim3 grid(t2_cdiv(d.N, G16_T), t2_cdiv(d.M, G16_T), d.splitk);
@@ -232,10 +256,11 @@
         if (j + 1 < p.count && tile.bx >= p.coltile_end[j]) prob = j + 1;
     const int bx = tile.bx - (prob > 0 ? p.coltile_end[prob - 1] : 0);
     struct { const void* A; const void* B; float* C; int M, N, K; long long lda, ldb, ldc; long long strideSplitC; int accumulate;
-             const float* bias; int splitk; } d;
+             const float* bias; int splitk; int m_store; float* C2; int c2_row; long long ldc2; } d;
     d.A = p.d[prob].A; d.B = p.d[prob].B; d.C = p.d[prob].C; d.M = p.d[prob].M; d.N = p.d[prob].N; d.K = p.d[prob].K;
     d.lda = p.d[prob].lda; d.ldb = p.d[prob].ldb; d.ldc = p.d[prob].ldc; d.strideSplitC = p.d[prob].strideSplitC;
     d.accumulate = p.d[prob].accumulate; d.bias = p.d[prob].bias; d.splitk = p.d[prob].splitk;
+    d.m_store = p.d[prob].m_store; d.C2 = p.d[prob].C2; d.c2_row = p.d[prob].c2_row; d.ldc2 = p.d[prob].ldc2;
     const int row0 = tile.by * G16_T, col0 = bx * G16_T;
     const int M = d.M, N = d.N;
     const int nkt_all = (d.K + G16_BK - 1) / G16_BK;
@@ -375,6 +400,7 @@
 #undef KK_TILE
 
     float* __restrict__ C = d.C + (long long)split * d.strideSplitC;
+    const int mst = d.m_store > 0 ? d.m_store : M;
 #pragma unroll
     for (int tm = 0; tm < 4; ++tm) {
 #pragma unroll
@@ -383,8 +409,8 @@
 #pragma unroll
             for (int r = 0; r < 16; ++r) {
                 const int gm = row0 + wm * 128 + tm * 32 + (r & 3) + 8 * (r >> 2) + 4 * lhi;
-                if (gm < M && gn < N) {
-                    float* cp = C + (long long)gm * d.ldc + gn;
+                if (gm < mst && gn < N) {
+                    float* cp = (d.C2 && gm >= d.c2_row) ? d.C2 + (long long)(gm - d.c2_row) * d.ldc2 + gn : C + (long long)gm * d.ldc + gn;
                     float val = acc[tm][tn][r];
                     if (d.bias) val += d.bias[gn];
                     if (d.accumulate) val += *cp;
@@ -411,6 +437,8 @@
         T2_REQUIRE(d.win_Tp == 0 && d.win_T == 0, "gemm16_kk: no window epilogue (overlapping rows are expressed by lda / ldb < M / N)");
         if (d.splitk < 1) d.splitk = 1;
         T2_REQUIRE(d.splitk == 1 || (!d.bias && !d.accumulate), "gemm16_kk: split-K needs a plain epilogue");
+        T2_REQUIRE(g16_check_epilogue(d, false), "gemm16_kk: bad epilogue extension (no act / keep / C16 here; C2 / m_store need splitk 1; "
+                   "0 < c2_row < rows stored; ldc2 >= N)");
         T2_REQUIRE(d.M == p.d[0].M && d.splitk == p.d[0].splitk, "gemm16_kk: the products of one launch share M and the split count");
         coltiles += t2_cdiv(d.N, G16_T);
         p.coltile_end[j] = coltiles;
diff --git a/tacotron2_amd/engine.py b/tacotron2_amd/engine.py
--- a/tacotron2_amd/engine.py
+++ b/tacotron2_amd/engine.py
@@ -104,6 +104,34 @@
 
 
 WGRAD_KK = os.environ.get('T2AMD_WGRAD_KK', '1') != '0'
+
+DENSE16 = os.environ.get('T2AMD_DENSE16', '1') != '0'
+
+
+def _dense16(run):
+    return run.bf16 and DENSE16 and not nv.validate_only()
+
+
+def _pad_cols16(W, Kp, transpose=False):
+    W = W.t() if transpose else W
+    out = torch.zeros(W.shape[0], Kp, dtype=torch.bfloat16, device=W.device)
+    out[:, :W.shape[1]].copy_(W)
+    return out
+
+
+def _proj_wgrad16(run, dout16, rows_out, K, blocks, dW_main, dW_last):
+    Mp = (rows_out + 7) // 8 * 8
+    sk = _choose_splitk16(Mp, sum((w + 255) // 256 * 256 for _, _, w in blocks), K)
+    if sk == 1:
+        nv.gemm16_kk_group([dict(Cm=dW_main[:, o:o + w], A16=dout16, B16=X, K=K, M=Mp, N=w, m_store=rows_out,
+                                 C2=dW_last[:, o:o + w], c2_row=rows_out - 1) for X, o, w in blocks])
+        return
+    parts = [run.empty(sk, Mp * w) for _, _, w in blocks]
+    nv.gemm16_kk_group([dict(Cm=pt[0].view(Mp, w), A16=dout16, B16=X, K=K, M=Mp, N=w, splitk=sk, partials=pt)
+                        for (X, o, w), pt in zip(blocks, parts)])
+    for (X, o, w), pt in zip(blocks, parts):
+        nv.splitk_reduce2d(pt, sk, dW_main[:, o:o + w], stride=Mp * w)
+        nv.splitk_reduce2d(pt[0, (rows_out - 1) * w:], sk, dW_last[:, o:o + w], stride=Mp * w)
 
 
 def _kk_to(run, out, A16, B16, K, M, N, lda=None, ldb=None, perm=None):
@@ -1007,15 +1035,25 @@
 
     rowsD = To * B
     x0 = run.empty(To, B, Cm)
-    nv.frames_to_time_major(mels, x0)
+    pre16 = _dense16(run) and Pd % 64 == 0
+    x16 = run.empty16(rowsD, (Cm + 63) // 64 * 64) if pre16 else None
+    nv.frames_to_time_major(mels, x0, x16)
     W1 = P['decoder.prenet.layers.0.linear_layer.weight']
     W2 = P['decoder.prenet.layers.1.linear_layer.weight']
     k0 = ms.get('prenet', 0, (To, B, Pd), 0.5)
     k1 = ms.get('prenet', 1, (To, B, Pd), 0.5)
     p1 = run.empty(rowsD, Pd)
     p2 = run.empty(rowsD, Pd)
-    _fg(run, p1, x0.view(rowsD, Cm), W1, act=1, keep=k0.view(rowsD, Pd), keep_scale=2.0, exact=True)
-    _fg(run, p2, p1, W2, act=1, keep=k1.view(rowsD, Pd), keep_scale=2.0, exact=True)
+    p2_16 = None
+    if pre16:
+        W1_16 = run.cached('prenet_W1_16', [W1], lambda: _pad_cols16(W1, x16.shape[1]))
+        W2_16 = run.cached('prenet_W2_16', [W2], lambda: run.cast16(W2))
+        p1_16, p2_16 = run.empty16(rowsD, Pd), run.empty16(rowsD, Pd)
+        nv.gemm16_tn(p1, x16, W1_16, act=1, keep=k0.view(rowsD, Pd), keep_scale=2.0, C16=p1_16)
+        nv.gemm16_tn(p2, p1_16, W2_16, act=1, keep=k1.view(rowsD, Pd), keep_scale=2.0, C16=p2_16)
+    else:
+        _fg(run, p1, x0.view(rowsD, Cm), W1, act=1, keep=k0.view(rowsD, Pd), keep_scale=2.0, exact=True)
+        _fg(run, p2, p1, W2, act=1, keep=k1.view(rowsD, Pd), keep_scale=2.0, exact=True)
     Wmem = P['decoder.attention_layer.memory_layer.linear_layer.weight']
     pm = run.empty(B, Ti, A)
     _fg(run, pm.view(rowsE, A), memory.view(rowsE, E), Wmem)
@@ -1050,7 +1088,7 @@
     def project_ga():
         if run.bf16 and WGRAD16 and Pd % 64 == 0 and (Pd + E) % 8 == 0 and not nv.validate_only():
             Wih_a16 = run.cached('Wih_a16', [Wih_a], lambda: run.cast16(Wih_a))
-            nv.gemm16_tn(GA.view(rowsD, 4 * Ha), run.cast16(p2), Wih_a16[:, :Pd], bias=bias_a)
+            nv.gemm16_tn(GA.view(rowsD, 4 * Ha), p2_16 if p2_16 is not None else run.cast16(p2), Wih_a16[:, :Pd], bias=bias_a)
         else:
             _fg(run, GA.view(rowsD, 4 * Ha), p2, Wih_a[:, :Pd], bias=bias_a)
     project_ga()
@@ -1101,8 +1139,14 @@
 
     Wpg, bpg = _packed_projection(run, P, Cm, Hd, E)
     PG = run.empty(rowsD, Cm + 1)
-    _fg(run, PG, slabs['HD'].view(rowsD, Hd), Wpg[:, :Hd])
-    _fg(run, PG, slabs['CTX'].view(rowsD, E), Wpg[:, Hd:], accumulate=True, bias=bpg)
+    if _dense16(run) and Hd % 64 == 0 and E % 64 == 0:
+        Wpg16 = run.cached('Wpg16', [P['decoder.linear_projection.linear_layer.weight'], P['decoder.gate_layer.linear_layer.weight']],
+                           lambda: run.cast16(Wpg))
+        nv.gemm16_tn(PG, c.bf16['HD16'].view(rowsD, Hd), Wpg16[:, :Hd])
+        nv.gemm16_tn(PG, c.bf16['CTX16'].view(rowsD, E), Wpg16[:, Hd:], accumulate=True, bias=bpg)
+    else:
+        _fg(run, PG, slabs['HD'].view(rowsD, Hd), Wpg[:, :Hd])
+        _fg(run, PG, slabs['CTX'].view(rowsD, E), Wpg[:, Hd:], accumulate=True, bias=bpg)
     mel_cl = run.empty(B, To, Cm)
     gate = run.out_empty(B, To)
     nv.split_projection(PG, mel_cl, gate, olens32)
@@ -1122,7 +1166,7 @@
     c.dec = d
     c.keep = dict(att=keep_att, dec=keep_dec, k0=k0, k1=k1)
     c.slabs = slabs
-    c.tensors = dict(x0=x0, p1=p1, p2=p2, pm=pm, GA=GA, Wa_rec=Wa_rec, Wd_cat=Wd_cat, bias_d=bias_d,
+    c.tensors = dict(x0=x0, p1=p1, p2=p2, p2_16=p2_16, pm=pm, GA=GA, Wa_rec=Wa_rec, Wd_cat=Wd_cat, bias_d=bias_d,
                      Wq=Wq, U=U, Wpg=Wpg, mel_cl=mel_cl, vvec=vvec, lens32=lens32)
     return (mel, mel_post, gate, slabs['ALIGN']), c
 
@@ -1169,19 +1213,27 @@
     if sync is not None:
         sync.bucket_ready('postnet')
     dout = run.empty(rowsD, Cm + 1)
-    nv.gather_dout(dmel_cl, cont(d_gate), dout)
+    proj16 = _dense16(run) and Hd % 8 == 0 and E % 8 == 0
+    dout16 = run.empty16(rowsD, (Cm + 1 + 63) // 64 * 64) if proj16 else None
+    nv.gather_dout(dmel_cl, cont(d_gate), dout, dout16)
 
     Wpg = T['Wpg']
     DHC = run.empty(rowsD, Hd + E)
-    _ng(run, DHC, dout, Wpg, b_kn=True)
-    dWpg_h = run.empty(Cm + 1, Hd)
-    dWpg_c = run.empty(Cm + 1, E)
-    _rg(run, dWpg_h, dout, S['HD'].view(rowsD, Hd), a_km=True, b_kn=True)
-    _rg(run, dWpg_c, dout, S['CTX'].view(rowsD, E), a_km=True, b_kn=True)
     dWp = G('decoder.linear_projection.linear_layer.weight', Cm, Hd + E)
     dWg = G('decoder.gate_layer.linear_layer.weight', 1, Hd + E)
-    nv.copy2d(dWp[:, :Hd], dWpg_h[:Cm]); nv.copy2d(dWp[:, Hd:], dWpg_c[:Cm])
-    nv.copy2d(dWg[:, :Hd], dWpg_h[Cm:]); nv.copy2d(dWg[:, Hd:], dWpg_c[Cm:])
+    if proj16:
+        pdeps = [P['decoder.linear_projection.linear_layer.weight'], P['decoder.gate_layer.linear_layer.weight']]
+        WpgT16 = run.cached('WpgT16', pdeps, lambda: _pad_cols16(Wpg, dout16.shape[1], transpose=True))
+        nv.gemm16_tn(DHC, dout16, WpgT16)
+        _proj_wgrad16(run, dout16, Cm + 1, rowsD, [(c.bf16['HD16'].view(rowsD, Hd), 0, Hd), (c.bf16['CTX16'].view(rowsD, E), Hd, E)], dWp, dWg)
+    else:
+        _ng(run, DHC, dout, Wpg, b_kn=True)
+        dWpg_h = run.empty(Cm + 1, Hd)
+        dWpg_c = run.empty(Cm + 1, E)
+        _rg(run, dWpg_h, dout, S['HD'].view(rowsD, Hd), a_km=True, b_kn=True)
+        _rg(run, dWpg_c, dout, S['CTX'].view(rowsD, E), a_km=True, b_kn=True)
+        nv.copy2d(dWp[:, :Hd], dWpg_h[:Cm]); nv.copy2d(dWp[:, Hd:], dWpg_c[:Cm])
+        nv.copy2d(dWg[:, :Hd], dWpg_h[Cm:]); nv.copy2d(dWg[:, Hd:], dWpg_c[Cm:])
     dbpg = run.empty(Cm + 1)
     run.colsum(dout, dbpg)
     dbp = G('decoder.linear_projection.linear_layer.bias', Cm)
@@ -1258,7 +1310,10 @@
     g['decoder.attention_layer.location_layer.location_conv.conv.weight'] = dWconv
     g['decoder.attention_layer.v.linear_layer.weight'] = dv
     dWq = G('decoder.attention_layer.query_layer.linear_layer.weight', A, Ha)
-    _rg(run, dWq, DQ.view(rowsD, A), S['HA'].view(rowsD, Ha), a_km=True, b_kn=True)
+    if _dense16(run) and A % 8 == 0 and Ha % 8 == 0:
+        _kk_to(run, dWq, run.cast16(DQ.view(rowsD, A)), c.bf16['HA16'].view(rowsD, Ha), rowsD, A, Ha)
+    else:
+        _rg(run, dWq, DQ.view(rowsD, A), S['HA'].view(rowsD, Ha), a_km=True, b_kn=True)
     g['decoder.attention_layer.query_layer.linear_layer.weight'] = dWq
 
     dWih_a = G('decoder.attention_rnn.weight_ih', 4 * Ha, Pd + E)
@@ -1266,7 +1321,7 @@
     use16 = run.bf16 and WGRAD16 and B % 8 == 0 and not nv.validate_only()
     Z = c.bf16 if use16 else None
     if use16:
-        _lstm_wgrad16(run, b16['DGA16'].view(rowsD, 4 * Ha), B, [(T['p2'], False), (Z['CTX16'].view(rowsD, E), True), (Z['HA16'].view(rowsD, Ha), True)],
+        _lstm_wgrad16(run, b16['DGA16'].view(rowsD, 4 * Ha), B, [(T['p2_16'] if T.get('p2_16') is not None else T['p2'], False), (Z['CTX16'].view(rowsD, E), True), (Z['HA16'].view(rowsD, Ha), True)],
                       [(dWih_a, 0, 2), (dWhh_a, 2, 3)])
     elif To > 1:
         tmp = run.empty(4 * Ha, Pd)
diff --git a/tacotron2_amd/native.py b/tacotron2_amd/native.py
--- a/tacotron2_amd/native.py
+++ b/tacotron2_amd/native.py
@@ -43,6 +43,9 @@
         ("lda", _i64), ("ldb", _i64), ("ldc", _i64),
         ("splitk", C.c_int), ("strideSplitC", _i64), ("accumulate", C.c_int), ("bias", _f32p),
         ("win_T", C.c_int), ("win_Tp", C.c_int),
+        ("act", C.c_int), ("keep", C.c_void_p), ("ldkeep", _i64), ("keep_scale", C.c_float),
+        ("C16", C.c_void_p), ("ldc16", _i64), ("n16", C.c_int),
+        ("m_store", C.c_int), ("C2", _f32p), ("c2_row", C.c_int), ("ldc2", _i64),
     ]
 
 
@@ -257,7 +260,7 @@
     "t2amd_embedding_fwd_f32", "t2amd_embedding_bwd_f32", "t2amd_philox_keep_mask", "t2amd_fill_f32",
     "t2amd_copy2d_f32", "t2amd_cast_bf16_f32", "t2amd_split_bf16x3_f32", "t2amd_transpose_f32", "t2amd_frames_to_time_major_f32",
     "t2amd_split_projection_f32", "t2amd_finalize_outputs_f32", "t2amd_grads_to_channel_last_f32",
-    "t2amd_gather_dout_f32", "t2amd_relu_dropout_bwd_f32",
+    "t2amd_gather_dout_f32", "t2amd_gather_dout_bf16", "t2amd_frames_to_time_major_bf16", "t2amd_relu_dropout_bwd_f32",
     "t2amd_lstm_step_fwd_f32", "t2amd_skinny_gemm_f32", "t2amd_lstm_pointwise_bwd_f32",
     "t2amd_lstm_step_fwd2_f32", "t2amd_skinny_gemm2_f32", "t2amd_lstm_pointwise_bwd2_f32",
     "t2amd_fold_location_f32", "t2amd_unfold_location_grads_f32",
@@ -322,6 +325,8 @@
         "t2amd_finalize_outputs_f32": [_P, _P, _P, _P, _P, _I, _I, _I, _P],
         "t2amd_grads_to_channel_last_f32": [_P, _P, _P, _P, _I, _I, _I, _P],
         "t2amd_gather_dout_f32": [_P, _P, _P, _I, _I, _I, _P],
+        "t2amd_gather_dout_bf16": [_P, _P, _P, _P, _I, _I, _I, _I, _P],
+        "t2amd_frames_to_time_major_bf16": [_P, _P, _P, _I, _I, _I, _I, _P],
         "t2amd_relu_dropout_bwd_f32": [_P, _P, _F, _L, _P],
         "t2amd_lstm_step_fwd_f32": [pt(LstmStep), _P],
         "t2amd_skinny_gemm_f32": [pt(SkinnyGemm), _P],
@@ -708,7 +713,26 @@
     _check(lib.t2amd_gemm_f32(C.byref(d), _stream()), "t2amd_gemm_f32")
 
 
-def gemm16_tn(Cm, A16, B16, K=None, splitk=1, partials=None, accumulate=False, bias=None):
+def _epilogue16(d, M, N, act=0, keep=None, keep_scale=1.0, C16=None, m_store=None, C2=None, c2_row=0):
+    d.act = act
+    if keep is not None:
+        if keep.dim() != 2 or tuple(keep.shape) != (M, N) or keep.stride(1) != 1 or keep.dtype != torch.uint8:
+            raise NativeError("gemm16: keep mask must be a [M,N] uint8 view, got %s" % (tuple(keep.shape),))
+        d.keep, d.ldkeep, d.keep_scale = ptr(keep, torch.uint8), max(keep.stride(0), N), keep_scale
+    if C16 is not None:
+        if C16.dim() != 2 or C16.dtype != torch.bfloat16 or C16.shape[0] != M or C16.shape[1] < N or C16.stride(1) != 1:
+            raise NativeError("gemm16: the bf16 image of C must be a [M, >= N] bfloat16 view, got %s" % (tuple(C16.shape),))
+        d.C16, d.ldc16, d.n16 = ptr(C16, torch.bfloat16), max(C16.stride(0), C16.shape[1]), C16.shape[1]
+    if m_store is not None:
+        d.m_store = m_store
+    if C2 is not None:
+        rows = M if m_store is None else m_store
+        if C2.dim() != 2 or tuple(C2.shape) != (rows - c2_row, N) or C2.stride(1) != 1:
+            raise NativeError("gemm16: the second destination must be [rows stored - c2_row, N], got %s" % (tuple(C2.shape),))
+        d.C2, d.c2_row, d.ldc2 = ptr(C2), c2_row, max(C2.stride(0), N)
+
+
+def gemm16_tn(Cm, A16, B16, K=None, splitk=1, partials=None, accumulate=False, bias=None, act=0, keep=None, keep_scale=1.0, C16=None):
     lib = load()
     d = Gemm16Desc()
     pa, lda, M, Ka = _mat(A16, torch.bfloat16)
@@ -726,6 +750,7 @@
         d.C, d.ldc = _mat(Cm)[:2]
     d.accumulate = 1 if accumulate else 0
     d.bias = ptr(bias)
+    _epilogue16(d, M, N, act=act, keep=keep, keep_scale=keep_scale, C16=C16)
     _check(lib.t2amd_gemm16_tn(C.byref(d), _stream()), "t2amd_gemm16_tn")
 
 
@@ -747,7 +772,8 @@
     _check(lib.t2amd_gemm16_tn(C.byref(d), _stream()), "t2amd_gemm16_tn")
 
 
-def _kk_desc(Cm, A16, B16, K, M=None, N=None, lda=None, ldb=None, splitk=1, partials=None, accumulate=False, bias=None):
+def _kk_desc(Cm, A16, B16, K, M=None, N=None, lda=None, ldb=None, splitk=1, partials=None, accumulate=False, bias=None,
+             m_store=None, C2=None, c2_row=0):
     d = Gemm16Desc()
     pa, lda0, ra, wa = _mat(A16, torch.bfloat16)
     pb, ldb0, rb, wb = _mat(B16, torch.bfloat16)
@@ -757,7 +783,8 @@
     ldb = ldb0 if ldb is None else ldb
     span_a = (ra - 1) * lda0 + wa
     span_b = (rb - 1) * ldb0 + wb
-    if K < 1 or (K - 1) * lda + M > span_a or (K - 1) * ldb + N > span_b or Cm.shape[0] != M or Cm.shape[1] != N:
+    rows_c = M if (m_store is None or splitk > 1) else (c2_row if C2 is not None else m_store)
+    if K < 1 or (K - 1) * lda + M > span_a or (K - 1) * ldb + N > span_b or Cm.shape[0] != rows_c or Cm.shape[1] != N:
         raise NativeError("gemm16_kk: shape mismatch A=%s B=%s C=%s M=%d N=%d K=%d lda=%d ldb=%d"
                           % (tuple(A16.shape), tuple(B16.shape), tuple(Cm.shape), M, N, K, lda, ldb))
     d.A, d.B, d.M, d.N, d.K, d.lda, d.ldb = pa, pb, M, N, K, lda, ldb
@@ -770,11 +797,13 @@
         d.C, d.ldc = _mat(Cm)[:2]
     d.accumulate = 1 if accumulate else 0
     d.bias = ptr(bias)
+    _epilogue16(d, M, N, m_store=m_store, C2=C2, c2_row=c2_row)
     return d
 
 
-def gemm16_kk(Cm, A16, B16, K, M=None, N=None, lda=None, ldb=None, splitk=1, partials=None, accumulate=False, bias=None):
-    d = _kk_desc(Cm, A16, B16, K, M, N, lda, ldb, splitk, partials, accumulate, bias)
+def gemm16_kk(Cm, A16, B16, K, M=None, N=None, lda=None, ldb=None, splitk=1, partials=None, accumulate=False, bias=None,
+              m_store=None, C2=None, c2_row=0):
+    d = _kk_desc(Cm, A16, B16, K, M, N, lda, ldb, splitk, partials, accumulate, bias, m_store, C2, c2_row)
     _check(load().t2amd_gemm16_kk(C.byref(d), _stream()), "t2amd_gemm16_kk")
 
 
@@ -783,7 +812,8 @@
         raise NativeError("gemm16_kk_group: 1..4 problems, got %d" % len(problems))
     arr = (Gemm16Desc * len(problems))(*[_kk_desc(**kw) for kw in problems])
     reads = [kw[k_] for kw in problems for k_ in ('A16', 'B16')]
-    writes = [kw['partials'] if kw.get('partials') is not None else kw['Cm'] for kw in problems]
+    writes = [kw['partials'] if kw.get('partials') is not None else kw['Cm'] for kw in problems] \
+        + [kw['C2'] for kw in problems if kw.get('C2') is not None]
     if not _via_ops("wgrad_gemm16", [arr], reads, writes):
         _check(load().t2amd_gemm16_kk_group(arr, len(problems), _stream()), "t2amd_gemm16_kk_group")
 
@@ -827,9 +857,12 @@
            "t2amd_splitk_reduce_f32")
 
 
-def splitk_reduce2d(partials, nsplit, out, accumulate=False):
+def splitk_reduce2d(partials, nsplit, out, accumulate=False, stride=None):
     po, ldo, rows, cols = _mat(out)
-    _check(load().t2amd_splitk_reduce2d_f32(ptr(partials), nsplit, _i64(rows * cols), po, rows, cols, _i64(ldo),
+    stride = rows * cols if stride is None else stride
+    if stride < rows * cols:
+        raise NativeError("splitk_reduce2d: slab stride %d < rows * cols = %d" % (stride, rows * cols))
+    _check(load().t2amd_splitk_reduce2d_f32(ptr(partials), nsplit, _i64(stride), po, rows, cols, _i64(ldo),
                                             1 if accumulate else 0, _stream()), "t2amd_splitk_reduce2d_f32")
 
 
@@ -973,10 +1006,16 @@
                                    _stream()), "t2amd_transpose_f32")
 
 
-def frames_to_time_major(mels, x0):
+def frames_to_time_major(mels, x0, x16=None):
     lib = load()
     B, Cm, To = mels.shape
     assert tuple(x0.shape) == (To, B, Cm)
+    if x16 is not None:
+        if x16.dtype != torch.bfloat16 or x16.dim() != 2 or x16.shape[0] != To * B or not x16.is_contiguous():
+            raise NativeError("frames_to_time_major: x16 must be a contiguous [To.B, ld16] bfloat16 matrix, got %s" % (tuple(x16.shape),))
+        _check(lib.t2amd_frames_to_time_major_bf16(ptr(_fullc(mels)), ptr(_fullc(x0)), ptr(x16, torch.bfloat16), x16.shape[1], B, Cm, To,
+                                                   _stream()), "t2amd_frames_to_time_major_bf16")
+        return
     _check(lib.t2amd_frames_to_time_major_f32(ptr(_fullc(mels)), ptr(_fullc(x0)), B, Cm, To, _stream()),
            "t2amd_frames_to_time_major_f32")
 
@@ -1006,9 +1045,15 @@
            "t2amd_grads_to_channel_last_f32")
 
 
-def gather_dout(dmel_cl, dgate, dout):
+def gather_dout(dmel_cl, dgate, dout, dout16=None):
     lib = load()
     B, To, Cm = dmel_cl.shape
+    if dout16 is not None:
+        if dout16.dtype != torch.bfloat16 or dout16.dim() != 2 or dout16.shape[0] != To * B or not dout16.is_contiguous():
+            raise NativeError("gather_dout: dout16 must be a contiguous [To.B, ld16] bfloat16 matrix, got %s" % (tuple(dout16.shape),))
+        _check(lib.t2amd_gather_dout_bf16(ptr(_fullc(dmel_cl)), ptr(dgate), ptr(_fullc(dout)), ptr(dout16, torch.bfloat16), dout16.shape[1],
+                                          B, Cm, To, _stream()), "t2amd_gather_dout_bf16")
+        return
     _check(lib.t2amd_gather_dout_f32(ptr(_fullc(dmel_cl)), ptr(dgate), ptr(_fullc(dout)), B, Cm, To, _stream()),
            "t2amd_gather_dout_f32")
 
```

New measurement: 621,800 valid mel-frames/s. 3.6% lower.
